# XJTU-Power-AI/charginghub-env

Hardware: AMD Instinct MI355X
Metric: env-steps/sec at 65 536 parallel envs (higher is better)
Workload: dtype f64; 1 GPU; 65536 envs x hub [20 fast, 25 slow] (BASELINE.json configs[3]), fcev_permeate 0.01, random policy resident in HBM, reset every 96 steps, Philox streams; envs_per_gpu=65536, obs_dim=13, act_dim=47, work_order=XCD-aware (tiles, tail and level workgroups in contiguous eighths per XCD), graph=on, collective=none

## Files before the change

### charginghub-env_amd/_lib.py

```python
import ctypes as C
import os

os.environ.setdefault("HIP_FORCE_DEV_KERNARG", "1")

_HERE = os.path.dirname(os.path.abspath(__file__))
DATA_DIR = os.path.join(_HERE, "data")

CHUB_FAST, CHUB_SLOW = 0, 1
RNG_COMPAT, RNG_PHILOX, RNG_PHILOX_CURVES = 0, 1, 2
RNG_MODES = {"compat": RNG_COMPAT, "philox": RNG_PHILOX, "philox_curves": RNG_PHILOX_CURVES}
T_COUNT = 38
TELEMETRY_NAMES = ["hy_act", "hy_flow_speed", "all_power_second", "Store_SOC", "capacity", "total_mass_need", "hy_use",
                   "not_meet", "fc_power", "hy_to_use", "re_used_renew", "re_ev_power_0", "re_ev_power_1",
                   "re_hydrogen_power", "income", "reward", "re_pv_power", "re_wd_power", "price_next",
                   "fcev_arrive_number", "fcev_line", "fcev_queue_len", "pv_day", "wd_day",
                   "ev_power_0_net", "ev_power_1_net", "ev_power_sum_net", "price_now",
                   "min_power_0", "charge_power_0", "max_power_0", "line_0", "flow_in_0",
                   "min_power_1", "charge_power_1", "max_power_1", "line_1", "flow_in_1"]
T = {name: i for i, name in enumerate(TELEMETRY_NAMES)}
EPISODE_NAMES = ["return", "income", "draw_ele", "length", "deviation", "test_penalty", "end_soc"]
EP_COUNT = len(EPISODE_NAMES)
EP = {name: i for i, name in enumerate(EPISODE_NAMES)}
PILE_NAMES = ("car", "charge", "emergency", "power", "soc", "init_soc", "target_soc", "stay_time", "already_stay_time")
PILE_COUNT = len(PILE_NAMES)
# ... 305 lines not shown
                ("price_fluctuate", C.c_double), ("hydro_loss", C.c_double)]


ENV_PARAM_FIELDS = ("hydro_prod_rate", "hydro_store_vlt", "init_soc", "fc_max_power", "fcev_permeate", "renew_fluctuate", "price_fluctuate",
                    "hydro_loss")


class ChubEnvParams(C.Structure):
    _fields_ = [(name, C.c_double) for name in ENV_PARAM_FIELDS]


def lib_path():
    return os.environ.get("CHUB_LIB") or os.path.join(_HERE, "libchub.so")


def source_hash():
    import hashlib

    h = hashlib.sha256()
    csrc = os.path.join(_HERE, "csrc")
    for name in ("chub_kernels.hip", "chub_policy.hip", "chub_critic.hip", "chub_runtime.cpp", "chub_comm.cpp", "chub_device.h", "chub_curves.h", "chub_plan.h",
                 "chub_policy.h", "chub_critic.h"):
        h.update(open(os.path.join(csrc, name), "rb").read())
    h.update(open(os.path.join(os.path.dirname(_HERE), "include", "chub.h"), "rb").read())
    return h.hexdigest()[:16]


_lib = None


def load_library():
    global _lib
    if _lib is not None:
        return _lib
    path = lib_path()
    if not os.path.exists(path):
        raise ChubError("libchub.so is not built (%s): run `python -c 'import __graft_entry__ as g; g.build()'` "
                        "or `make -C charginghub-env_amd/csrc`; there is no CPU fallback" % path)
    lib = C.CDLL(path)
    if not os.environ.get("CHUB_LIB"):
        lib.chub_build_id.restype = C.c_char_p
        have, want = lib.chub_build_id().decode(), source_hash()
        if have != want:
            raise ChubError("libchub.so (build id %s) is older than its sources (%s): rebuild with "
                            "`make -C charginghub-env_amd/csrc`" % (have, want))
    P, I, L = C.c_void_p, C.c_int, C.c_int64
    sig = {
        "chub_create": (I, [C.POINTER(ChubConfig), C.c_char_p, L, L, I, C.c_uint64, I, C.POINTER(P)]),
        "chub_create_ex": (I, [C.POINTER(ChubConfig), C.c_char_p, L, L, I, C.c_uint64, I, C.POINTER(ChubOptions), C.POINTER(P)]),
        "chub_destroy": (I, [P]),
        "chub_obs_dim": (I, [P]), "chub_act_dim": (I, [P]), "chub_num_envs": (L, [P]), "chub_clock": (I, [P]), "chub_uses_packed_kernel": (I, [P]), "chub_uses_fused_step": (I, [P]), "chub_uses_xcd_order": (I, [P]),
        "chub_launch_plan": (I, [C.POINTER(ChubConfig), L, I, C.POINTER(ChubOptions), P]),
        "chub_launch_plan_params": (I, [C.POINTER(ChubConfig), L, I, C.POINTER(ChubOptions), P]),
        "chub_create_params": (I, [C.POINTER(ChubConfig), C.c_char_p, L, L, I, C.c_uint64, I, C.POINTER(ChubOptions), P, C.POINTER(P)]),
        "chub_set_env_params": (I, [P, P, P]), "chub_get_env_params": (I, [P, P]), "chub_has_env_params": (I, [P]),
        "chub_reset": (I, [P, P, P, P]),
        "chub_step": (I, [P, P, P, P, P, P]), "chub_host_actions": (I, [P, C.POINTER(P)]),
        "chub_step_bits": (I, [P, P, P, P, P, P, P]), "chub_host_bits": (I, [P, C.POINTER(P), C.POINTER(P)]),
        "chub_step_bits_device": (I, [P, P, P, P, P, P, P, P]), "chub_step_bits_device_packed": (I, [P, P, P, P, P, P]),
        "chub_reset_device": (I, [P, P, P, P, P]),
        "chub_step_device": (I, [P, P, P, P, P, P, P]),
        "chub_step_device_packed": (I, [P, P, P, P, P]),
        "chub_reset_envs": (I, [P, P, P, P, P]), "chub_step_envs": (I, [P, P, P, P, P, P, P]), "chub_reset_envs_device": (I, [P, P, P, P, P, P]),
        "chub_step_envs_device": (I, [P, P, P, P, P, P, P, P]), "chub_env_clocks": (I, [P, P, P]), "chub_clock_groups": (I, [P]),
        "chub_dmask_reset_envs_device": (I, [P, P, P, P, P, P]), "chub_dmask_step_envs_device": (I, [P, P, P, P, P, P, P, P]),
        "chub_autoreset_step_device": (I, [P, P, P, P, P, P, P, P]),
        "chub_call_plan": (I, [C.POINTER(ChubConfig), L, I, C.POINTER(ChubOptions), I, C.c_uint32, P]),
        "chub_step_load": (I, [P, P, P, P, P, P]), "chub_step_load_device": (I, [P, P, P, P, P, P, P]),
        "chub_step_load_envs": (I, [P, P, P, P, P, P, P]), "chub_step_load_envs_device": (I, [P, P, P, P, P, P, P, P]),
        "chub_random_actions_device": (I, [P, C.c_uint64, C.c_uint32, P, P]),
        "chub_sync": (I, [P]),
        "chub_profile_begin": (I, [P, I, I]), "chub_profile_end": (I, [P, P, P, P]),
        "chub_get_slots": (I, [P, P]), "chub_get_station_scalars": (I, [P, P]), "chub_get_telemetry": (I, [P, P]),
        "chub_get_obs_f64": (I, [P, P]), "chub_get_reward_f64": (I, [P, P]), "chub_set_telemetry": (I, [P, I]), "chub_fcev_stuck_count": (I, [P, P]),
        "chub_telemetry_host": (I, [P, C.POINTER(P), C.POINTER(P), C.POINTER(P)]),
        "chub_set_episode_stats": (I, [P, I]), "chub_has_episode_stats": (I, [P]), "chub_get_episode_stats": (I, [P, I, P]),
        "chub_get_episode_counts": (I, [P, P]), "chub_episode_stats_device": (I, [P, I, P, P, P]),
        "chub_episode_summary_device": (I, [P, P, I, P]), "chub_episode_summary": (I, [P, P, I]),
        "chub_pile_obs_columns": (I, [C.c_uint32]), "chub_pile_obs_device": (I, [P, C.c_uint32, P, P, P]),
        "chub_station_profile_size": (I, [C.c_uint32, C.c_int32]), "chub_station_profile_device": (I, [P, C.c_uint32, C.c_int32, P, P, P]),
        "chub_load_dispatch_device": (I, [P, I, P, P, P, P, P, P]), "chub_load_dispatch": (I, [P, I, P, P, P, P]),
        "chub_forecast_size": (I, [C.c_uint32, C.c_int32]), "chub_forecast_device": (I, [P, C.c_uint32, C.c_int32, P, P, P]),
        "chub_forecast": (I, [P, C.c_uint32, C.c_int32, P]),
        "chub_get_step_terms_size": (I, [C.c_uint32]), "chub_get_step_terms_device": (I, [P, C.c_uint32, P, P, P]),
        "chub_get_step_terms": (I, [P, C.c_uint32, P]), "chub_set_step_terms": (I, [P, C.c_uint32, P]), "chub_get_step_terms_attached": (I, [P]),
        "chub_set_rng_compat_seeds": (I, [P, P]), "chub_set_rng_compat_state": (I, [P, P]),
        "chub_get_rng_compat_state": (I, [P, P]), "chub_compat_replay_constructor": (I, [P]), "chub_set_ou_state": (I, [P, P]),
        "chub_copy_envs": (I, [P, P, P, P, L]), "chub_copy_envs_device": (I, [P, P, P, P, L, P]),
        "chub_state_size": (L, [P]), "chub_get_state": (I, [P, P, L]), "chub_set_state": (I, [P, P, L]),
        "chub_get_hy_table": (I, [P, P]), "chub_get_hy_table_env": (I, [P, L, P]), "chub_set_hy_table": (I, [P, P]),
        "chub_last_error": (C.c_char_p, []), "chub_device_count": (I, []), "chub_build_id": (C.c_char_p, []),
        "chub_comm_unique_id": (I, [P]), "chub_comm_create": (I, [P, I, I, I, C.POINTER(P)]), "chub_comm_destroy": (I, [P]),
        "chub_comm_world": (I, [P]), "chub_comm_rank": (I, [P]), "chub_comm_gather": (I, [P, P, P, L, P]),
        "chub_comm_gather_timed": (I, [P, P, P, L, P, I, C.POINTER(C.c_double)]),
        "chub_comm_max_f64": (I, [P, C.POINTER(C.c_double), P]), "chub_comm_barrier": (I, [P, P]),
        "chub_comm_ranks_seen": (I, [P, C.POINTER(C.c_int), P]),
        "chub_comm_set_overlap": (I, [P, I]), "chub_comm_gather_begin": (I, [P, P, P]), "chub_comm_join": (I, [P, P]), "chub_device_info": (I, [I, P]),
        "chub_step_gather": (I, [P, P, P, P, P, P]), "chub_run_steps": (I, [P, P, P, I, P, P, P, L, L, P]),
        "chub_tape_register_soc": (I, [P, P, C.c_int32, P]), "chub_set_slots": (I, [P, P]), "chub_set_station_queue": (I, [P, P]),
        "chub_step_tape": (I, [P, P, P, P, P, P, P]), "chub_reset_tape": (I, [P, P, P, P]), "chub_tape_clear_soc": (I, [P]),
        "chub_step_tape_env": (I, [P, P, P, P, P, P, C.c_int32, P, P, P]), "chub_reset_tape_env": (I, [P, P, P, P, P, P]),
        "chub_graph_begin": (I, [P, P]), "chub_graph_end": (I, [P, P, C.POINTER(P)]), "chub_graph_launch": (I, [P, P]),
        "chub_graph_destroy": (I, [P]),
        "chub_malloc_device": (I, [I, L, C.POINTER(P)]), "chub_free_device": (I, [I, P]), "chub_copy_to_host": (I, [I, P, P, L, P]),
        "chub_copy_to_device": (I, [I, P, P, L, P]), "chub_alloc_host": (I, [I, L, C.POINTER(P)]), "chub_free_host": (I, [I, P]), "chub_stream_create": (I, [I, C.POINTER(P)]), "chub_stream_destroy": (I, [I, P]),
        "chub_stream_sync": (I, [I, P]),
# ... 2 lines not shown
        "chub_policy_set_weights": (I, [P, C.c_int32, P, P]), "chub_policy_set_weights_device": (I, [P, C.c_int32, P, P, P]),
        "chub_policy_act_device": (I, [P, P, P, L, P, P, P, P, P]), "chub_policy_act": (I, [P, P, P, P]),
        "chub_policy_run_steps": (I, [P, P, I, P, P, P, L, L, P]),
        "chub_next_tick": (I, [P, C.POINTER(C.c_uint32)]), "chub_policy_set_exploration": (I, [P, C.c_uint64, P]),
        "chub_policy_set_log_std_device": (I, [P, P, P]),
        "chub_policy_sample_device": (I, [P, P, P, L, P, C.POINTER(ChubPolicySampleOut), P]),
        "chub_policy_collect": (I, [P, P, I, C.POINTER(ChubRollout), P, L, P]),
        "chub_pile_set_device": (I, [P, I, P, P, P]),
        "chub_policy_sample_set_device": (I, [P, P, P, L, P, I, P, C.POINTER(ChubPolicySampleOut), P]),
        "chub_policy_collect_set": (I, [P, P, I, I, C.POINTER(ChubRollout), P, P, L, P]),
        "chub_rollout_gae_device": (I, [P, C.POINTER(ChubGae), P]),
        "chub_moments_create": (I, [P, C.c_int32, C.POINTER(P)]), "chub_moments_destroy": (I, [P]),
        "chub_moments_update_device": (I, [P, P, L, L, P, P]), "chub_moments_reset_device": (I, [P, P]),
        "chub_moments_get": (I, [P, C.POINTER(C.c_double), P, P]), "chub_moments_set": (I, [P, C.c_double, P, P]),
        "chub_moments_state_device": (I, [P, C.POINTER(P)]),
        "chub_policy_set_normalizer": (I, [P, P, P]), "chub_policy_set_normalizer_device": (I, [P, P, P, P]),
        "chub_policy_get_normalizer_device": (I, [P, P, P, P]), "chub_policy_normalizer_from_moments_device": (I, [P, P, C.c_double, P]),
        "chub_population_param_count": (I, [C.POINTER(ChubConfig), C.POINTER(ChubPolicySpec), C.POINTER(L)]),
        "chub_population_create": (I, [P, C.c_int32, C.c_uint64, C.POINTER(P)]), "chub_population_destroy": (I, [P]),
        "chub_population_perturb_device": (I, [P, P, P, C.c_float, C.c_uint32, P]),
        "chub_population_set_member_device": (I, [P, C.c_int32, C.c_int32, P, P, P]),
        "chub_population_get_member_device": (I, [P, C.c_int32, C.c_int32, P, P, P]),
        "chub_population_set_member": (I, [P, C.c_int32, C.c_int32, P, P]), "chub_population_get_member": (I, [P, C.c_int32, C.c_int32, P, P]),
        "chub_population_copy_members_device": (I, [P, P, P, C.c_int32, P]),
        "chub_population_act_device": (I, [P, P, P, L, P, P, P, P, P]), "chub_population_run_steps": (I, [P, P, I, P, P, P, L, L, P]),
        "chub_population_es_gradient_device": (I, [P, P, C.c_uint32, P, P, P]),
        "chub_policy_grad_plan": (I, [C.POINTER(ChubConfig), C.POINTER(ChubPolicySpec), L, C.POINTER(ChubPolicyGradPlanOut)]),
        "chub_policy_grad_create": (I, [P, L, C.POINTER(P)]), "chub_policy_grad_destroy": (I, [P]),
        "chub_policy_grad_device": (I, [P, C.POINTER(ChubPolicyGradIn), C.POINTER(ChubPolicyGradOut), P]),
        "chub_critic_plan": (I, [C.POINTER(ChubCriticSpec), L, C.POINTER(ChubCriticPlanOut)]),
        "chub_critic_create": (I, [P, C.POINTER(ChubCriticSpec), P, P, P, P, L, C.POINTER(P)]), "chub_critic_destroy": (I, [P]),
        "chub_critic_set_weights": (I, [P, C.c_int32, P, P]), "chub_critic_set_weights_device": (I, [P, C.c_int32, P, P, P]),
        "chub_critic_set_normalizer": (I, [P, P, P]), "chub_critic_set_normalizer_device": (I, [P, P, P, P]),
        "chub_critic_normalizer_from_moments_device": (I, [P, P, C.c_double, P]),
        "chub_critic_values_device": (I, [P, P, L, L, P, L, P, P]),
        "chub_critic_grad_device": (I, [P, C.POINTER(ChubCriticGradIn), C.POINTER(ChubCriticGradOut), P]),
    }
    for name, (res, args) in sig.items():
        try:
            fn = getattr(lib, name)
        except AttributeError:
            if os.environ.get("CHUB_LIB"):
                def missing(*_a, _name=name, _path=path):
                    raise ChubError("%s is not exported by the library CHUB_LIB names (%s): an older build" % (_name, _path))
                setattr(lib, name, missing)
                continue
            raise
        fn.restype = res
        fn.argtypes = args
    _lib = lib
    return lib


EXPORTED = ["chub_create", "chub_create_ex", "chub_destroy", "chub_obs_dim", "chub_act_dim", "chub_num_envs", "chub_clock", "chub_uses_packed_kernel", "chub_uses_fused_step", "chub_uses_xcd_order", "chub_launch_plan", "chub_launch_plan_params",
            "chub_create_params", "chub_set_env_params", "chub_get_env_params", "chub_has_env_params", "chub_reset",
            "chub_step", "chub_host_actions", "chub_step_bits", "chub_host_bits", "chub_step_bits_device", "chub_step_bits_device_packed", "chub_reset_device", "chub_step_device", "chub_step_device_packed", "chub_step_load", "chub_step_load_device", "chub_step_load_envs", "chub_step_load_envs_device", "chub_reset_envs", "chub_step_envs", "chub_reset_envs_device", "chub_step_envs_device",
            "chub_env_clocks", "chub_clock_groups", "chub_dmask_reset_envs_device", "chub_dmask_step_envs_device", "chub_autoreset_step_device", "chub_call_plan", "chub_random_actions_device", "chub_sync", "chub_profile_begin", "chub_profile_end",
            "chub_get_slots", "chub_get_station_scalars", "chub_get_telemetry", "chub_get_obs_f64",
            "chub_get_reward_f64", "chub_set_telemetry", "chub_fcev_stuck_count", "chub_set_rng_compat_seeds", "chub_set_rng_compat_state", "chub_get_rng_compat_state", "chub_compat_replay_constructor", "chub_set_ou_state",
            "chub_copy_envs", "chub_copy_envs_device", "chub_state_size", "chub_get_state", "chub_set_state", "chub_get_hy_table", "chub_get_hy_table_env", "chub_set_hy_table", "chub_last_error", "chub_device_count", "chub_build_id",
            "chub_comm_unique_id", "chub_comm_create", "chub_comm_destroy", "chub_comm_world", "chub_comm_rank", "chub_comm_gather", "chub_comm_gather_timed",
            "chub_comm_max_f64", "chub_comm_barrier", "chub_comm_ranks_seen", "chub_comm_set_overlap", "chub_comm_gather_begin", "chub_comm_join", "chub_device_info", "chub_step_gather", "chub_run_steps", "chub_tape_register_soc", "chub_set_slots",
            "chub_set_station_queue", "chub_step_tape", "chub_reset_tape", "chub_tape_clear_soc", "chub_step_tape_env", "chub_reset_tape_env", "chub_telemetry_host", "chub_graph_begin", "chub_graph_end", "chub_graph_launch", "chub_graph_destroy",
            "chub_malloc_device", "chub_free_device", "chub_copy_to_host", "chub_copy_to_device", "chub_alloc_host", "chub_free_host", "chub_stream_create",
            "chub_stream_destroy", "chub_stream_sync",
            "chub_set_episode_stats", "chub_has_episode_stats", "chub_get_episode_stats", "chub_get_episode_counts", "chub_episode_stats_device",
            "chub_episode_summary_device", "chub_episode_summary", "chub_pile_obs_columns", "chub_pile_obs_device",
            "chub_station_profile_size", "chub_station_profile_device", "chub_load_dispatch_device", "chub_load_dispatch",
            "chub_forecast_size", "chub_forecast_device", "chub_forecast",
            "chub_get_step_terms_size", "chub_get_step_terms_device", "chub_get_step_terms", "chub_set_step_terms", "chub_get_step_terms_attached",
            "chub_policy_input_width", "chub_policy_create", "chub_policy_destroy", "chub_policy_set_weights", "chub_policy_set_weights_device",
            "chub_policy_act_device", "chub_policy_act", "chub_policy_run_steps",
            "chub_next_tick", "chub_policy_set_exploration", "chub_policy_set_log_std_device", "chub_policy_sample_device", "chub_policy_collect",
            "chub_pile_set_device", "chub_policy_sample_set_device", "chub_policy_collect_set", "chub_rollout_gae_device",
            "chub_moments_create", "chub_moments_destroy", "chub_moments_update_device", "chub_moments_reset_device", "chub_moments_get", "chub_moments_set",
            "chub_moments_state_device", "chub_policy_set_normalizer", "chub_policy_set_normalizer_device", "chub_policy_get_normalizer_device",
            "chub_policy_normalizer_from_moments_device",
            "chub_population_param_count", "chub_population_create", "chub_population_destroy", "chub_population_perturb_device",
            "chub_population_set_member_device", "chub_population_get_member_device", "chub_population_set_member", "chub_population_get_member",
            "chub_population_copy_members_device", "chub_population_act_device", "chub_population_run_steps", "chub_population_es_gradient_device",
            "chub_policy_grad_plan", "chub_policy_grad_create", "chub_policy_grad_destroy", "chub_policy_grad_device",
            "chub_critic_plan", "chub_critic_create", "chub_critic_destroy", "chub_critic_set_weights", "chub_critic_set_weights_device",
            "chub_critic_set_normalizer", "chub_critic_set_normalizer_device", "chub_critic_normalizer_from_moments_device",
            "chub_critic_values_device", "chub_critic_grad_device"]


def check(rc):
    if rc != 0:
        msg = load_library().chub_last_error()
        raise ChubError("libchub error %d: %s" % (rc, msg.decode() if msg else "?"))
```

### charginghub-env_amd/csrc/chub_device.h

```cpp
#pragma once

#include <stdint.h>

#include "chub_curves.h"

#if defined(__HIP_DEVICE_COMPILE__)
#define CHUB_G(T) T __attribute__((address_space(1))) *
#else
#define CHUB_G(T) T *
#endif

namespace chub {

constexpr int kMaxLine = 10;
constexpr int kLevels = 1000;
constexpr int kBalkTab = 1024;
constexpr int kMaxPiles = 4096;
constexpr int kSocLevels = 2048;
constexpr int kSocLevelShift = 21;
constexpr int kPolarMaxTrials = 32;
#ifndef CHUB_TRACE
#define CHUB_TRACE 0
#endif
#ifndef CHUB_SLOTS_PER_LANE
// ... 175 lines not shown
struct EpisodeArrays {
    int32_t on;
    int32_t pad_;
    CHUB_G(double) live;
    CHUB_G(double) fin;
    CHUB_G(uint32_t) episodes;
    CHUB_G(uint8_t) pending;
};

enum FcField : uint32_t { FC_SLOT = 0, FC_VALID, FC_SIN, FC_COS, FC_PRICE, FC_PV, FC_WIND, FC_ARRIVALS0, FC_ARRIVALS1, FC_FCEV };
constexpr int kFcCount = 10;
constexpr int kFcHist = 301;
struct ForecastTabs {
    const float *mean;
    const uint32_t *hist;
    const uint16_t *hist_len;
};

struct DevCtx {
    HubParams hp;
    SlotArrays sl;
    StationArrays st;
    EnvArrays ev;
    CompatRng cr;
    Tables tb;
    EnvParamArrays ep;
    EpisodeArrays es;
};

struct CopyArgs {
    const DevCtx *src;
    const DevCtx *dst;
    CHUB_G(const int64_t) src_idx;
    CHUB_G(const int64_t) dst_idx;
    int64_t count;
    CHUB_G(const uint16_t) src_clk;
    CHUB_G(uint16_t) dst_clk;
    uint32_t src_clk_value;
    int32_t src_rng, dst_rng;
    CHUB_G(const double) src_rows;
    CHUB_G(double) dst_rows;
};

struct PackedPtrs {
    const EnvArrays *ev;
    const StationArrays *st;
    uint32_t *hot, *rec;
    uint8_t *stay8;
    uint32_t *pk[2];
    const float *cls[2], *ttab[2], *ttab2;
    uint32_t late8[8];
    const Tables *tb;
    const double *sin96;
};

struct StepArgs {
    int32_t t;
    uint32_t tick;
    int32_t draw_price;
    int32_t station_filter;
    double price_last;
    double price_prev;
    const float *actions;
    const uint64_t *act_bits;
    const float *act_tail;
    const double *exo_z;
    const int32_t *exo_days;
    float *obs;
    float *reward;
    uint8_t *done;
    float *done_f32;
    int32_t obs_stride, reward_stride;
    int32_t load_mode;
    const uint64_t *pk_tape;
    const uint32_t *car_tape;
    const uint32_t *hv_tape;
    int32_t hv_w;
    int32_t tail_tape;
    uint16_t *env_clk;
    const uint8_t *env_mask;
    int32_t env_lo, env_hi;
    int32_t fresh;
    int32_t empt_fresh;
    int32_t commit_rng;
    int32_t rng_cur;
    int32_t walked;
    int32_t walk_far, walk_short;
    uint32_t *tick_note;
    uint8_t *done_mask;
    uint32_t *done_count;
    const uint32_t *skip_count;
    float *final_obs;
#if CHUB_TRACE
    unsigned long long *stamps_slot, *stamps_env;
#endif
};

}
```

### charginghub-env_amd/csrc/chub_kernels.hip

```cpp
#include <hip/hip_runtime.h>
#include <hip/hip_ext.h>
#include <stdint.h>

#include "chub_device.h"
#include "chub_plan.h"

namespace chub {

typedef uint32_t u32x4 __attribute__((ext_vector_type(4)));
typedef uint32_t u32x2 __attribute__((ext_vector_type(2)));

__device__ __forceinline__ bool in_group(const StepArgs &sa, int64_t env) { return !sa.env_mask || sa.env_mask[env] != 0; }
__device__ __forceinline__ uint32_t env_clk(const StepArgs &sa, int64_t n_envs, int64_t env) {
    return sa.env_clk[(int64_t) (sa.tick & 1u) * n_envs + env];
}
__device__ __forceinline__ int64_t range_len(const StepArgs &sa) { return (int64_t) sa.env_hi - sa.env_lo + 1; }
__device__ __forceinline__ bool range_unit(const StepArgs &sa, int64_t i, int segments, int &seg, int64_t &env) {
    const int64_t R = range_len(sa);
    if (i >= (int64_t) segments * R) return false;
    seg = (i >= R ? 1 : 0) + (i >= 2 * R ? 1 : 0);
    env = sa.env_lo + (i - (int64_t) seg * R);
    return true;
}

// ... 218 lines not shown
}

__device__ __forceinline__ float normal_from_word(const float *tz, const float *tl, uint32_t w) {
    const uint32_t cell = w >> 20;
    const bool hi = cell >= 4096u - 16u, lo = cell < 16u;
    const uint32_t m = hi ? ~w : w;
    const bool tail = hi || lo;
    const float *tab = tail ? tl : tz;
    const uint32_t idx = tail ? (m >> 12) : cell;
    const float frac = tail ? (float) (m & 0xFFFu) * (1.0f / 4096.0f) : (float) (w & 0xFFFFFu) * (1.0f / 1048576.0f);
    const float a = tab[idx], b = tab[idx + 1];
    const float z = __fadd_rn(a, __fmul_rn(__fsub_rn(b, a), frac));
    return hi ? -z : z;
}

__device__ __forceinline__ uint32_t dk_make(uint64_t pk, int line, bool fast) {
    line = __popc((uint32_t) pk & ((1u << line) - 1u));
    const int n_in = (int) (pk >> 10) & 15;
    const int flow = fast ? n_in : (int) ((pk >> (14 + 4 * line)) & 15);
    return (uint32_t) (line + flow) | ((uint32_t) flow << 8);
}
__device__ __forceinline__ uint32_t draw_decoded_levels(const HubParams &hp, const Tables &tb, uint32_t tick, int t, int k, int64_t env,
                                                        int line, bool fast) {
    PhiloxCtx px{hp.key[0], hp.key[1], tick, (uint32_t) (hp.env_id0 + env)};
    const U4 a0 = px.block(SITE_ARRIVE, (uint32_t) k, 0);
    const U4 r0 = px.block(SITE_RENEGE, (uint32_t) k, 0);
    int n_in = (int) tb.cnt[k][t * kLevels + (int) (a0.v[0] % 1000u)];
    n_in = n_in > 9 ? 9 : n_in;
    uint32_t rw[10] = {r0.v[0], r0.v[1], r0.v[2], r0.v[3], 0u, 0u, 0u, 0u, 0u, 0u};
    if (__any(line > 4)) {
        const U4 r1 = px.block(SITE_RENEGE, (uint32_t) k, 1), r2 = px.block(SITE_RENEGE, (uint32_t) k, 2);
        rw[4] = r1.v[0]; rw[5] = r1.v[1]; rw[6] = r1.v[2]; rw[7] = r1.v[3]; rw[8] = r2.v[0]; rw[9] = r2.v[1];
    }
    int stay_q = 0;
#pragma unroll
    for (int w = 0; w < kMaxLine; w++) stay_q += (w < line && (int) (rw[w] % 1000u) >= (int) tb.thr_renege[w]) ? 1 : 0;
    int flow = n_in;
    if (!fast && __any(n_in > 0)) {
        uint32_t bw[9] = {a0.v[1], a0.v[2], a0.v[3], 0u, 0u, 0u, 0u, 0u, 0u};
        if (__any(n_in > 3)) {
            const U4 a1 = px.block(SITE_ARRIVE, (uint32_t) k, 1), a2 = px.block(SITE_ARRIVE, (uint32_t) k, 2);
            bw[3] = a1.v[0]; bw[4] = a1.v[1]; bw[5] = a1.v[2]; bw[6] = a1.v[3]; bw[7] = a2.v[0]; bw[8] = a2.v[1];
        }
        const int S = hp.S[k];
        flow = 0;
#pragma unroll
        for (int j = 0; j < 9; j++) {
            if (j >= 3 && !__any(n_in > j)) break;
            const int top = (int) tb.inv_balk[bw[j] % 1000u] - j;
            flow += (j < n_in && j <= S && stay_q <= top) ? 1 : 0;
        }
    }
    return (uint32_t) (stay_q + flow) | ((uint32_t) flow << 8);
}
__device__ __forceinline__ int dk_want(uint32_t dk) { return (int) (dk & 255u); }
__device__ __forceinline__ int dk_flow(uint32_t dk) { return (int) ((dk >> 8) & 255u); }


template <int TYPE>
__device__ __forceinline__ void car_step_curves(float tt, bool cp, const CurveConsts &cc, float &soc, float &power) {
    if (cp) {
        soc = time_to_soc<TYPE>(tt, cp, cc);
        power = time_to_power<TYPE>(tt, cp);
        return;
    }
    if (TYPE == 0) {
        const float xf = tt * 15.0f;
        const double x = xf, t = tt;
        const bool p1 = tt >= 0 && t < (28.7 / 15), p2 = tt >= 0 && t < (51.2 / 15);
        const bool s0 = tt <= 0, s1 = t <= 28.7 / 15, s2 = t <= 51.2 / 15;
        float pw = 0.0f, sc = 100.0f;
        if (__any(p1 || (!s0 && s1))) {
            const double e = exp(0.053 * x);
            if (p1) pw = (float) (0.7194 * e + 47.78);
            if (!s0 && s1) sc = (float) ((0.7194 / 0.053) * e + 50.15 * x - (double) cc.fast_aa1_c) * cc.fast_soc_scale;
        }
        if (__any((!p1 && p2) || (!s0 && !s1 && s2))) {
            const double x2 = x * x, x3 = x2 * x, x4 = x2 * x2, x5 = x4 * x;
            if (!p1 && p2) pw = (float) (0.0002253 * x4 - 0.03572 * x3 + 2.016 * x2 - 48.76 * x + 457.7);
            if (!s0 && !s1 && s2)
                sc = (float) ((0.0002253 / 5) * x5 - (0.03572 / 4) * x4 + (2.016 / 3) * x3 - (48.76 / 2) * x2 + 457.7 * x +
                              (double) cc.fast_aa2_c) * cc.fast_soc_scale;
        }
        if (s0) sc = 0.0f;
        soc = sc;
        power = pw;
    } else {
        const float xf = tt / 4.0f;
        const double x = xf, t = tt;
        const bool p1 = t < 2.33 * 4, p2 = t < 3.67 * 4;
        const bool c0 = tt <= 0, c1 = t <= 2.33 * 4, c2 = t <= 3.67 * 4;
        float pw = 0.0f, ch = cc.slow_c2_end;
        if (__any(p1 || (!c0 && c1))) {
            const double x2 = x * x, x3 = x2 * x, x4 = x2 * x2, x5 = x4 * x;
            if (p1) pw = (float) (-0.002056 * x4 + 0.00921 * x3 + 0.03562 * x2 + 0.02379 * x + 6.007);
            if (!c0 && c1)
                ch = (float) (-0.0004112 * x5 + 0.0023025 * x4 + (0.03562 / 3) * x3 + 0.011895 * x2 + 6.007 * x);
        }
        if (__any((!p1 && p2) || (!c0 && !c1 && c2))) {
            if (!p1 && p2) pw = (float) ((-4.041 * x + 21.1) / (x - 0.485));
            if (!c0 && !c1 && c2) ch = (float) (-4.041 * x + 19.140115 * log(fabs(x - 0.485)) + 11.943306312699628);
        }
        if (c0) ch = 0.0f;
        soc = (float) CHUB_DIV_K64((double) (100.0f * ch), 19.285746346634653);
        power = pw;
    }
// ... 1100 lines not shown
            car = tl > 0;
        }
        const bool urgent = car && must_charge(t_target, t_soc, tl);
        const uint64_t bc = __ballot(car);
        if (lane == 0) s_ball[4 + wave] = bc;
        if (MODE == MODE_COMPAT) {
            s_a[tid] = urgent ? power : 0.0f;
            s_b[tid] = charge ? power : 0.0f;
            s_c[tid] = car ? power : 0.0f;
        } else {
            const int q = kw_to_fixed(power);
            s_u[tid] = (uint32_t) (urgent ? q : 0);
            s_v[tid] = (uint32_t) (charge ? q : 0);
            s_w[tid] = (uint32_t) (car ? q : 0);
        }
        __syncthreads();
        cars += __popcll(s_ball[4]) + __popcll(s_ball[5]) + __popcll(s_ball[6]) + __popcll(s_ball[7]);
        if (tid == 0) {
            const int n = S - (c << 8) < 256 ? S - (c << 8) : 256;
            if (MODE == MODE_COMPAT) rf.add(s_a, s_b, s_c, n);
            else ri.add(s_u, s_v, s_w, n);
        }
        base += chunk_empties;
        __syncthreads();
    }
    if (tid == 0) {
        if (MODE == MODE_COMPAT) {
            rs.store(ctx->cr, sa.rng_cur, env);
            rec_store(st.rec, sidx, rf.mn, rf.chg, rf.mx, pkd_make(s_hdr[2], s_hdr[1], cars));
        } else {
            rec_store(st.rec, sidx, fixed64_to_kw(ri.mn), fixed64_to_kw(ri.chg), fixed64_to_kw(ri.mx), pkd_make(s_hdr[2], s_hdr[1], cars));
        }
    }
}

struct PackedArgs {
    uint32_t S[2], type[2];
    uint32_t n_envs, epb, magic, cls_delta;
    CHUB_G(uint32_t) state;
    CHUB_G(uint32_t) rec;
    CHUB_G(const uint32_t) pk;
    CHUB_G(const float) actions;
    CHUB_G(const float) cls0;
    CHUB_G(const float) ttab2;
    CHUB_G(const uint32_t) car_tape;
    uint32_t key[2], gid0, tick;
    const uint32_t *tick_base;
    uint32_t late[8];
    CHUB_G(const uint8_t) env_mask;
    uint32_t blk0;
    uint32_t xcd;
    CHUB_G(float) tail_act;
    CHUB_G(uint8_t) stay8;
};

typedef const uint32_t __attribute__((address_space(4))) *chub_sptr;
__device__ __forceinline__ uint32_t sload_u32(const void *p, int i) { return ((chub_sptr) (uintptr_t) p)[i]; }
__device__ __forceinline__ bool mask_is_empty(const StepArgs &sa) { return sa.skip_count != nullptr && sload_u32(sa.skip_count, 0) == 0u; }

#ifndef CHUB_ACT_NT
#define CHUB_ACT_NT 0
#endif
#if CHUB_ACT_NT
#define CHUB_ACT_LOAD(p) __builtin_nontemporal_load(p)
#else
#define CHUB_ACT_LOAD(p) (*(p))
#endif
#ifndef CHUB_ACC_COPIES
#define CHUB_ACC_COPIES 2
#endif
constexpr int kAccCopies = CHUB_ACC_COPIES;
#ifndef CHUB_TAIL_PRE
#define CHUB_TAIL_PRE 1
#endif
#ifndef CHUB_UNIT_DRAWS
#define CHUB_UNIT_DRAWS 1
#endif
#ifndef CHUB_EPI_ALL
#define CHUB_EPI_ALL 1
#endif
#define CHUB_AT(T_, base, byte_off) (*(CHUB_G(T_)) ((CHUB_G(char)) (base) + (uint32_t) (byte_off)))
template <int BLOCK, int T, bool RESET, bool BIG, bool MASKED, bool FUSED, bool BITS>
__device__ __forceinline__ void packed_records(const PackedArgs &pa, const uint32_t block_local, int *s_acc, const uint32_t *s_unit, u32x4 *s_rec,
                                               const float *tail_pre = nullptr) {
    const int lane = threadIdx.x & 63;
    const int S0 = (int) pa.S[0], S1 = (int) pa.S[1], St = S0 + S1;
    const int epb = (int) pa.epb, N = (int) pa.n_envs;
    const int env_first = (int) block_local * epb;
    const long long *s_acc64 = (const long long *) s_acc;
    __builtin_amdgcn_fence(__ATOMIC_RELEASE, "wavefront");
    __builtin_amdgcn_wave_barrier();
    __builtin_amdgcn_fence(__ATOMIC_ACQUIRE, "wavefront");
    for (int i = lane; i < 2 * epb; i += 64) {
        const int e = i >> 1, k = i & 1;
        const int env = env_first + e;
        if (env >= N) continue;
        if (MASKED && pa.env_mask[env] == 0) continue;
        const uint32_t su = (uint32_t) (k ? N : 0) + (uint32_t) env;
        if (!RESET && !FUSED && !BITS && k == 0) {
            typedef float f32x2_ __attribute__((ext_vector_type(2)));
            const uint32_t ai = ((uint32_t) env * (uint32_t) (St + 2) + (uint32_t) St) << 2;
            f32x2_ tv;
            if (CHUB_TAIL_PRE && i < 64) tv = f32x2_{tail_pre[0], tail_pre[1]};
            else tv = f32x2_{CHUB_AT(const float, pa.actions, ai), CHUB_AT(const float, pa.actions, ai + 4u)};
            CHUB_AT(f32x2_, pa.tail_act, (uint32_t) env << 3) = tv;
        }
        uint32_t lf = s_unit[i];
        if ((k ? S1 : S0) == 0) {
            const uint32_t pk = CHUB_AT(const uint32_t, pa.pk, su << 2);
            const bool fast = (k ? pa.type[1] : pa.type[0]) == 0;
            int want, fl;
            if (RESET) {
                fl = fast ? (int) (int16_t) (pk & 0xFFFFu) : (int) ((pk >> 16) & 0xFFFFu);
                want = fl;
            } else {
                want = dk_want(pk);
                fl = dk_flow(pk);
            }
            const int as = want < 0 ? want : 0;
            int ln = want - as;
            ln = ln < kMaxLine ? ln : kMaxLine;
            lf = pkd_make(ln, fl, 0);
        }
        u32x4 rv;
        if (!BIG) {
            int a0 = 0, a1 = 0, a2 = 0, a3 = 0;
#pragma unroll
            for (int c = 0; c < kAccCopies; c++) {
                const int *acc = s_acc + 4 * i + c * 8 * epb;
                a0 += acc[0]; a1 += acc[1]; a2 += acc[2]; a3 += acc[3];
            }
            rv = u32x4{__float_as_uint(fixed_to_kw(a0)), __float_as_uint(fixed_to_kw(a1)), __float_as_uint(fixed_to_kw(a2)),
                       lf | ((uint32_t) a3 << 16)};
        } else {
            const long long *a64 = s_acc64 + 4 * i;
            rv = u32x4{__float_as_uint((float) a64[0] * (1.0f / 524288.0f)), __float_as_uint((float) a64[1] * (1.0f / 524288.0f)),
                       __float_as_uint((float) a64[2] * (1.0f / 524288.0f)), lf | ((uint32_t) a64[3] << 16)};
        }
        CHUB_AT(u32x4, pa.rec, su << 4) = rv;
        if (FUSED) s_rec[i] = rv;
    }
}
#undef CHUB_AT

struct NoHook {
    __device__ __forceinline__ void prefetch() {}
    __device__ __forceinline__ void park() {}
};
template <int BLOCK, int T, bool TAPE, bool RESET, bool BIG, bool MASKED, bool FUSED, typename Hook, bool BITS = false, bool PIPED = false>
__device__ __forceinline__ int slot_body_packed(const HubParams &hp, const StepArgs &sa, PackedArgs &pa, const Tables &tb,
                                                const uint32_t block_local, uint32_t *q_cnt, uint32_t *q_new,
                                                uint64_t *s_ball, int *s_acc, uint32_t *s_unit, Hook &hook, u32x4 *s_rec, uint32_t *s_uinfo) {
    typedef float f32x4 __attribute__((ext_vector_type(4)));
    typedef float f32x2 __attribute__((ext_vector_type(2)));
    constexpr int WAVES = BLOCK / 64;
    const int tid = threadIdx.x;
    const int lane = tid & 63, wave = tid >> 6;
    const int S0 = (int) pa.S[0], S1 = (int) pa.S[1], St = S0 + S1;
    const int epb = (int) pa.epb, N = (int) pa.n_envs;
    const int env_first = (int) block_local * epb;
    const uint32_t idx0 = (uint32_t) env_first * (uint32_t) St;
    CHUB_STAMP_DECL(16);
    CHUB_STAMP_REAL(12);
    CHUB_STAMP(0);
#define CHUB_AT(T_, base, byte_off) (*(CHUB_G(T_)) ((CHUB_G(char)) (base) + (uint32_t) (byte_off)))

    constexpr bool STATE_FIRST = !RESET && !FUSED && BLOCK <= 256;
    constexpr bool UNIT_DRAWS = CHUB_UNIT_DRAWS && STATE_FIRST && !BIG && T <= 2;
    int e_[T], k_[T], slot[T];
    bool valid[T];
    uint32_t sidx[T];
    uint32_t s2[T];
    float act[T];
    u32x2 actw[T];
    int hs_[T];
    uint32_t pk_in[T];
    uint32_t served[T];
    constexpr bool HOIST_TAIL = CHUB_TAIL_PRE && !RESET && !FUSED && !BITS;
    float tail_pre[2];
#pragma unroll
    for (int j = 0; j < T; j++) {
        const int v = tid + j * BLOCK;
        e_[j] = (int) (__umul24((uint32_t) v, pa.magic) >> 20);
        const int hs = v - (int) __umul24((uint32_t) e_[j], (uint32_t) St);
        k_[j] = hs >= S0 ? 1 : 0;
        hs_[j] = hs;
        slot[j] = hs - (k_[j] ? S0 : 0);
        const int env = env_first + e_[j];
        valid[j] = e_[j] < epb && env < N;
        served[j] = 1u;
        sidx[j] = (uint32_t) (k_[j] ? N : 0) + (uint32_t) env;
        asm volatile("" : "=v"(s2[j]), "=v"(act[j]), "=v"(pk_in[j]), "=v"(actw[j]));
        if (!STATE_FIRST) {
            if (RESET) {
                s2[j] = 0u;
                act[j] = 0.0f;
            }
            if (MASKED && valid[j]) served[j] = pa.env_mask[env];
            if (valid[j]) {
                if (!RESET) {
                    s2[j] = CHUB_AT(uint32_t, pa.state, (idx0 + (uint32_t) v) << 2);
                    if (BITS) actw[j] = CHUB_AT(const u32x2, pa.actions, ((uint32_t) env * (((uint32_t) St + 63u) >> 6) + ((uint32_t) hs >> 6)) << 3);
                    else act[j] = CHUB_ACT_LOAD((CHUB_G(const float)) ((CHUB_G(const char)) pa.actions + (uint32_t) ((idx0 + (uint32_t) v + 2u * (uint32_t) env) << 2)));
                }
                pk_in[j] = CHUB_AT(const uint32_t, pa.pk, sidx[j] << 2);
            }
        }
    }
    if (STATE_FIRST) {
        uint32_t vc[T], envc[T];
#pragma unroll
        for (int j = 0; j < T; j++) {
            vc[j] = valid[j] ? (uint32_t) (tid + j * BLOCK) : 0u;
            envc[j] = valid[j] ? (uint32_t) (env_first + e_[j]) : (uint32_t) env_first;
        }
#pragma unroll
        for (int j = 0; j < T; j++) s2[j] = CHUB_AT(uint32_t, pa.state, (idx0 + vc[j]) << 2);
        asm volatile("" ::: "memory");
        if (MASKED) {
#pragma unroll
            for (int j = 0; j < T; j++) served[j] = CHUB_AT(const uint8_t, pa.env_mask, envc[j]);
            asm volatile("" ::: "memory");
        }
        if (!UNIT_DRAWS) {
#pragma unroll
            for (int j = 0; j < T; j++) pk_in[j] = CHUB_AT(const uint32_t, pa.pk, (valid[j] ? sidx[j] : (uint32_t) env_first) << 2);
            asm volatile("" ::: "memory");
        }
#pragma unroll
        for (int j = 0; j < T; j++) {
            if (BITS) actw[j] = CHUB_AT(const u32x2, pa.actions, (envc[j] * (((uint32_t) St + 63u) >> 6) + (valid[j] ? (uint32_t) hs_[j] >> 6 : 0u)) << 3);
            else act[j] = CHUB_ACT_LOAD((CHUB_G(const float)) ((CHUB_G(const char)) pa.actions + (uint32_t) ((idx0 + vc[j] + 2u * envc[j]) << 2)));
        }
    }
    uint32_t upk = 0u;
    if (UNIT_DRAWS) asm volatile("" : "=v"(upk));
    if (UNIT_DRAWS && (tid & ~63) < 2 * epb) {
        asm volatile("" ::: "memory");
        const int ue = tid >> 1, uenv = env_first + ue;
        upk = CHUB_AT(const uint32_t, pa.pk, (ue < epb && uenv < N ? (uint32_t) ((tid & 1) ? N : 0) + (uint32_t) uenv : (uint32_t) env_first) << 2);
    }
    if (HOIST_TAIL) asm volatile("" : "=v"(tail_pre[0]), "=v"(tail_pre[1]));
    if (HOIST_TAIL && wave == WAVES - 1) {
        asm volatile("" ::: "memory");
        const int te = env_first + (lane >> 1);
        const uint32_t tenv = (uint32_t) ((lane >> 1) < epb && te < N ? te : env_first);
        const uint32_t ai = (tenv * (uint32_t) (St + 2) + (uint32_t) St) << 2;
        tail_pre[0] = CHUB_AT(const float, pa.actions, ai);
        tail_pre[1] = CHUB_AT(const float, pa.actions, ai + 4u);
    }
    if (!TAPE) {
        pa.tick += sload_u32(pa.tick_base, 0);
        asm volatile("" : "+s"(pa.key[0]), "+s"(pa.key[1]), "+s"(pa.gid0), "+s"(pa.tick), "+s"(pa.late[0]), "+s"(pa.late[1]), "+s"(pa.late[2]),
                          "+s"(pa.late[3]), "+s"(pa.late[4]), "+s"(pa.late[5]), "+s"(pa.late[6]), "+s"(pa.late[7]));
    }
    CHUB_STAMP(1);
    if (FUSED) hook.prefetch();
    if (tid == 0) q_cnt[0] = 0;
    for (int i = tid; i < (BIG ? 16 : 8 * kAccCopies) * epb; i += BLOCK) s_acc[i] = 0;
    long long *s_acc64 = (long long *) s_acc;

    uint32_t w0[T];
    int tl[T];
    bool stays[T];
    f32x4 row[T];
    float ttg[T];
    if (!FUSED) {
#pragma unroll
        for (int j = 0; j < T; j++) asm volatile("" : "+v"(s2[j]));
    }
    if (MASKED) {
#pragma unroll
        for (int j = 0; j < T; j++) {
            asm volatile("" : "+v"(served[j]));
            valid[j] = valid[j] && served[j] != 0u;
        }
    }
#pragma unroll
    for (int j = 0; j < T; j++) {
        if (FUSED) asm volatile("" : "+v"(s2[j]));
        w0[j] = valid[j] ? s2[j] : 0u;
        tl[j] = ps_tl(w0[j]);
        stays[j] = tl[j] > 1;
        asm volatile("" : "=v"(row[j]), "=v"(ttg[j]));
        if (stays[j]) {
            row[j] = CHUB_AT(const f32x4, pa.cls0, (k_[j] ? pa.cls_delta : 0u) + (ps_cls(w0[j]) << 8) + (ps_n(w0[j]) << 3));
            ttg[j] = CHUB_AT(const float, pa.ttab2, (k_[j] ? 4096u : 0u) + (ps_lev(w0[j]) << 2));
        }
    }

    CHUB_STAMP(2);
    bool empty[T];
    uint64_t be[T];
#pragma unroll
    for (int j = 0; j < T; j++) {
        empty[j] = valid[j] && !stays[j];
        be[j] = __ballot(empty[j]);
        if (lane == 0) s_ball[wave + j * WAVES] = be[j];
    }
    if (FUSED) hook.park();
    CHUB_STAMP(3);
    __syncthreads();
    CHUB_STAMP(4);
    if (!BIG) {
        for (int u = tid; u < 2 * epb; u += BLOCK) {
            const int e = u >> 1, k = u & 1;
            const int Sk = k ? S1 : S0;
            const int U0 = e * St + (k ? S0 : 0), U1 = U0 + Sk;
            const int wv = U0 >> 6, lo = U0 & 63;
            const int hi0 = (U1 - (wv << 6)) < 64 ? (U1 - (wv << 6)) : 64;
            uint32_t info = (uint32_t) wv << 24;
            int all = 0;
            if (Sk > 0) {
                const uint64_t b0 = s_ball[wv];
                const uint64_t below_lo = lo ? (~0ull >> (64 - lo)) : 0ull, below_hi = ~0ull >> (64 - hi0);
                const int start_e = __popcll(b0 & below_lo), cnt0 = __popcll(b0 & below_hi & ~below_lo);
                const int over = U1 - ((wv + 1) << 6);
                const int cnt1 = over > 0 ? __popcll(s_ball[wv + 1] & (~0ull >> (64 - over))) : 0;
                all = cnt0 + cnt1;
                info |= (uint32_t) start_e | ((uint32_t) cnt0 << 8) | (UNIT_DRAWS ? 0u : (uint32_t) (cnt0 + cnt1) << 16);
            }
            if (UNIT_DRAWS) {
                asm volatile("" : "+v"(upk));
                const int want = dk_want(upk);
                const int assign = want < all ? want : all;
                const int ln = want - assign;
                s_unit[u] = pkd_make(ln < kMaxLine ? ln : kMaxLine, dk_flow(upk), 0);
                info |= (uint32_t) assign << 16;
            }
            s_uinfo[u] = info;
        }
    }

    uint32_t w0n[T];
#pragma unroll
    for (int j = 0; j < T; j++) {
        if (BITS) asm volatile("" : "+v"(row[j]), "+v"(ttg[j]), "+v"(actw[j]));
        else asm volatile("" : "+v"(row[j]), "+v"(ttg[j]), "+v"(act[j]));
        const int u = 2 * e_[j] + k_[j];
        int *acc = s_acc + 4 * u + (BIG ? 0 : (lane & (kAccCopies - 1)) * 8 * epb);
        w0n[j] = 0u;
        if (stays[j]) {
            const float t_target = ttg[j];
            const bool bit_on = BITS && ((((hs_[j] & 32) ? actw[j].y : actw[j].x) >> (hs_[j] & 31)) & 1u) != 0u;
            const bool on = (BITS ? bit_on : act[j] >= kActOnThreshold) || must_charge(t_target, row[j].y, tl[j]);
            const float power = on ? row[j].z : row[j].x, t_soc = on ? row[j].w : row[j].y;
            const int q = kw_to_fixed(power);
            const bool urgent = must_charge(t_target, t_soc, tl[j] - 1);
            w0n[j] = (w0[j] & ~kPsChg) - 1u + (on ? (kPsStep | kPsChg) : 0u);
            if (!BIG) {
                atomicAdd((unsigned long long *) (acc + 2), (unsigned long long) (uint32_t) q | (1ull << 32));
                if (on || urgent)
                    atomicAdd((unsigned long long *) acc,
                              (unsigned long long) (urgent ? (uint32_t) q : 0u) | ((unsigned long long) (on ? (uint32_t) q : 0u) << 32));
            } else {
                unsigned long long *a64 = (unsigned long long *) (s_acc64 + 4 * u);
                atomicAdd(a64 + 2, (unsigned long long) q);
                atomicAdd(a64 + 3, 1ull);
                if (urgent) atomicAdd(a64 + 0, (unsigned long long) q);
                if (on) atomicAdd(a64 + 1, (unsigned long long) q);
            }
        }
    }
    CHUB_STAMP(5);
    if (!BIG) __syncthreads();
    CHUB_STAMP(6);

    int line[T], flow[T];
    bool adm[T];
    uint64_t ba[T];
    uint32_t n_push = 0;
#pragma unroll
    for (int j = 0; j < T; j++) {
        const int vw = wave + j * WAVES;
        int empties, rank;
        if (!BIG) {
// ... 77 lines not shown
            const u32x2 tp = CHUB_AT(const u32x2, pa.car_tape, (idx0 + (uint32_t) src) << 3);
            c = tp.x;
            lev = tp.y & 0xFFFFu;
            late = (int) (tp.y >> 16);
        } else {
            PhiloxCtx p2{pa.key[0], pa.key[1], pa.tick, pa.gid0 + (uint32_t) (env_first + s_e)};
            const U4 o = p2.block(SITE_SOC, (uint32_t) s_hs, 0);
            c = o.v[0] >> kSocLevelShift;
            lev = o.v[1] % 1000u;
            late = 0;
#pragma unroll
            for (int j = 0; j < 8; j++) late += (o.v[2] >= pa.late[j]) ? 1 : 0;
            if (__any(o.v[2] >= pa.late[7])) {
#pragma unroll
                for (int j = 8; j < 16; j++) late += (o.v[2] >= tb.late_thr[j]) ? 1 : 0;
            }
        }
        f32x2 e0 = CHUB_AT(const f32x2, pa.cls0, (s_k ? pa.cls_delta : 0u) + (c << 8));
        float tt_ = CHUB_AT(const float, pa.ttab2, (s_k ? 4096u : 0u) + (lev << 2));
        asm volatile("" : "+v"(e0), "+v"(tt_));
        int st_ = (int) ceilf(__fsub_rn(tt_, e0.y)) + late;
        st_ = st_ > kMaxStay ? kMaxStay : st_;
        CHUB_AT(uint32_t, pa.state, (idx0 + (uint32_t) src) << 2) = st_ > 0 ? ps_make(st_, c, lev) : 0u;
        CHUB_AT(uint8_t, pa.stay8, idx0 + (uint32_t) src) = (uint8_t) st_;
        if (st_ > 0) {
            const int q = kw_to_fixed(e0.x);
            if (!BIG) {
                int *ac = s_acc + 4 * (2 * s_e + s_k) + (lane & (kAccCopies - 1)) * 8 * epb;
                atomicAdd((unsigned long long *) (ac + 2), (unsigned long long) (uint32_t) q | (1ull << 32));
                if (must_charge(tt_, e0.y, st_)) atomicAdd(ac, q);
            } else {
                unsigned long long *a64 = (unsigned long long *) (s_acc64 + 4 * (2 * s_e + s_k));
                atomicAdd(a64 + 2, (unsigned long long) q);
                atomicAdd(a64 + 3, 1ull);
                if (must_charge(tt_, e0.y, st_)) atomicAdd(a64 + 0, (unsigned long long) q);
            }
        }
    }
    CHUB_STAMP(9);
    if (FUSED) return wave == WAVES - 1 ? WAVES : wave + 1;
    if (ALL) {
        __syncthreads();
        CHUB_STAMP(10);
        CHUB_STAMP_REAL(13);
#if CHUB_TRACE
        if (sa.stamps_slot && tid == 0) {
            for (int i = 0; i <= 10; i++) sa.stamps_slot[(size_t) block_local * 16 + i] = stamp_[i];
            sa.stamps_slot[(size_t) block_local * 16 + 12] = stamp_[12];
            sa.stamps_slot[(size_t) block_local * 16 + 13] = stamp_[13];
        }
#endif
        if (wave != WAVES - 1) return 0;
    }
    packed_records<BLOCK, T, RESET, BIG, MASKED, false, BITS>(pa, block_local, s_acc, s_unit, nullptr, tail_pre);
#if CHUB_TRACE
    asm volatile("s_waitcnt vmcnt(0)" ::: "memory");
    CHUB_STAMP(11);
    if (sa.stamps_slot && lane == 0) sa.stamps_slot[(size_t) block_local * 16 + 11] = stamp_[11];
#endif
    return 0;
#undef CHUB_AT
}

template <int BLOCK, int T, bool TAPE, bool RESET, bool BIG, bool MASKED, bool BITS = false>
__global__ __launch_bounds__(BLOCK, (BLOCK <= 256 ? 8 : 2048 / BLOCK)) void k_slot_packed(const DevCtx *__restrict__ ctx, StepArgs sa, PackedArgs pa_in) {
    __shared__ uint32_t q_new[BLOCK * T];
    __shared__ uint32_t q_cnt[2];
    __shared__ uint64_t s_ball[BLOCK * T / 64 + 2];
    __shared__ __attribute__((aligned(16))) int s_acc[2 * BLOCK * T * kAccCopies];
    __shared__ uint32_t s_unit[BLOCK * T / 2];
    __shared__ uint32_t s_uinfo[BLOCK * T / 2];
    if (RESET && MASKED && mask_is_empty(sa)) return;
    PackedArgs pa = pa_in;
    asm volatile("" : "+s"(pa.S[0]), "+s"(pa.S[1]), "+s"(pa.type[0]), "+s"(pa.type[1]), "+s"(pa.n_envs), "+s"(pa.epb), "+s"(pa.magic),
                      "+s"(pa.cls_delta), "+s"(pa.state), "+s"(pa.rec), "+s"(pa.pk), "+s"(pa.actions), "+s"(pa.cls0), "+s"(pa.ttab2));
    NoHook hook;
    (void) slot_body_packed<BLOCK, T, TAPE, RESET, BIG, MASKED, false, NoHook, BITS>(ctx->hp, sa, pa, ctx->tb, xcd_order(blockIdx.x, pa.xcd, MASKED ? 0u : pa.xcd) + (MASKED ? pa.blk0 : 0u), q_cnt, q_new,
                                                                                     s_ball + 1, s_acc, s_unit, hook, nullptr, s_uinfo);
}

struct TailArgs {
    CHUB_G(const double) ou;
    CHUB_G(const double) price_noise;
    CHUB_G(const double) cap;
    CHUB_G(const int16_t) pv_day;
    CHUB_G(const int16_t) wd_day;
    CHUB_G(const uint8_t) q_len;
    CHUB_G(const uint8_t) hv_line;
    CHUB_G(const uint32_t) drw;
    CHUB_G(const uint8_t) drw_cnt;
    CHUB_G(uint32_t) rec;
    CHUB_G(const float) actions;
    uint32_t n_envs, act_dim, s_tot, xcd;
    CHUB_G(const float) tail_act;
    CHUB_G(const double) pv_row;
    CHUB_G(const double) wd_row;
    CHUB_G(const double) pv_row_now;
    CHUB_G(const double) wd_row_now;
    CHUB_G(const double) hy_table;
    const uint32_t *tick_base;
    double sin_t;
    uint32_t key[2], gid0, pad2;
};
inline TailArgs make_tail_args(const EnvArrays &ev, const StationArrays &st, const HubParams &hp, const StepArgs &sa, const PackedPtrs &pp,
                               bool reset) {
    TailArgs ta;
    const int t_next = reset ? 0 : (sa.t + 1) % 96;
    ta.tail_act = (hp.rng_mode == MODE_PHILOX && hp.packed && !sa.load_mode && !reset) ? (CHUB_G(const float)) st.tail_act : nullptr;
    if (sa.act_bits && !reset) ta.tail_act = (CHUB_G(const float)) sa.act_tail;
    ta.pv_row = (CHUB_G(const double)) (pp.tb->pvT + t_next * 100);
    ta.wd_row = (CHUB_G(const double)) (pp.tb->wdT + t_next * 150);
    ta.pv_row_now = (CHUB_G(const double)) (pp.tb->pvT + (reset ? 0 : sa.t) * 100);
    ta.wd_row_now = (CHUB_G(const double)) (pp.tb->wdT + (reset ? 0 : sa.t) * 150);
    ta.hy_table = (CHUB_G(const double)) pp.tb->hy_table;
    ta.tick_base = hp.tick_base;
    ta.sin_t = pp.sin96[t_next];
    ta.key[0] = hp.key[0];
    ta.key[1] = hp.key[1];
    ta.gid0 = (uint32_t) hp.env_id0;
    ta.pad2 = 0;
    ta.ou = (CHUB_G(const double)) ev.ou;
    ta.price_noise = (CHUB_G(const double)) ev.price_noise;
    ta.cap = (CHUB_G(const double)) ev.cap;
    ta.pv_day = (CHUB_G(const int16_t)) ev.pv_day;
    ta.wd_day = (CHUB_G(const int16_t)) ev.wd_day;
    ta.q_len = (CHUB_G(const uint8_t)) ev.q_len;
    ta.hv_line = (CHUB_G(const uint8_t)) ev.hv_line;
    ta.drw = (CHUB_G(const uint32_t)) ev.drw[sa.tick & 1u];
    ta.drw_cnt = (CHUB_G(const uint8_t)) ev.drw_cnt[sa.tick & 1u];
    ta.rec = (CHUB_G(uint32_t)) st.rec;
// ... 491 lines not shown
    double soc = (double) socf;
    if (soc < 0.5) soc = 0.5;
    const double p0 = (soc * 0.01) * 70;
    j2601_time_mass(p0, tn, mn);
}

__device__ __forceinline__ double ou_sample(double &state, double theta, double sigma, double z) {
    const double dx = theta * (0.0 - state) + sigma * z;
    state += dx;
    return state;
}

#define CHUB_TEL(i, v)                                        \
    do {                                                      \
        if (tel_on) ev.telem[(size_t) (i) * (size_t) N + (size_t) env] = (v); \
    } while (0)

constexpr int kEnvBlock = 256;

struct TailIn {
    double ou_pv, ou_wd, ou_price, price_noise, cap;
    float a_el, a_fc;
    int pv_day, wd_day, q_len, hv_line;
    u32x4 drw;
    uint32_t drw_n;
};
__device__ __forceinline__ void tail_prefetch(TailIn &in, const TailArgs &ta, const uint32_t e32, const bool predrawn) {
    const uint32_t n32 = ta.n_envs;
    in.ou_pv = ta.ou[e32];
    in.ou_wd = ta.ou[n32 + e32];
    in.ou_price = ta.ou[2u * n32 + e32];
    in.price_noise = ta.price_noise[e32];
    if (ta.tail_act) {
        typedef float f32x2_ __attribute__((ext_vector_type(2)));
        const f32x2_ tv = ((CHUB_G(const f32x2_)) ta.tail_act)[e32];
        in.a_el = tv.x;
        in.a_fc = tv.y;
    } else {
        const uint32_t ai = e32 * ta.act_dim + ta.s_tot;
        in.a_el = ta.actions[ai];
        in.a_fc = ta.actions[ai + 1u];
    }
    in.cap = ta.cap[e32];
    in.pv_day = ta.pv_day[e32];
    in.wd_day = ta.wd_day[e32];
    in.q_len = ta.q_len[e32];
    in.hv_line = ta.hv_line[e32];
    if (predrawn) {
        in.drw = ((CHUB_G(const u32x4)) ta.drw)[e32];
        in.drw_n = ta.drw_cnt[e32];
    }
}

struct NoMid {
    __device__ __forceinline__ void operator()() {}
    __device__ __forceinline__ void at1() {}
    __device__ __forceinline__ void at2() {}
    __device__ __forceinline__ void at3() {}
};
__device__ __forceinline__ uint32_t hv_count_rate(float rate, uint32_t n) {
    const int c = (int) roundf(rate * (float) n);
    return (uint32_t) (c < 0 ? 0 : (c > 255 ? 255 : c));
}
__device__ __forceinline__ uint32_t hv_count_env(const EnvParamArrays &ep, uint32_t e, int t, uint32_t lev) {
    return hv_count_rate(ep.hv_rate[e], (uint32_t) ep.hv_idx[(uint32_t) t * (uint32_t) kLevels + lev]);
}

template <bool RESET, int MODE, bool MULTI, bool FUSED = false, typename Mid = NoMid, int EB = kEnvBlock, bool TAPE = false, bool EP = false>
__device__ __forceinline__ void env_tail(const DevCtx *__restrict__ ctx, const StepArgs &sa, const int env, const bool live,
                                         const double *s_pv, const double *s_wd, const double *s_pv_now, const double *s_wd_now,
                                         const double *s_hy, const uint8_t *s_hv, float *s_out, const int env_block, const TailArgs &ta,
                                         const u32x4 *s_rec, const int local_env, const int env0_fused, const int rows_fused,
                                         const TailIn &pre, const bool use_pre, Mid &mid) {
    const HubParams &hp = ctx->hp;
    const EnvArrays &ev = ctx->ev;
    const CompatRng &cr = ctx->cr;
    const Tables &tb = ctx->tb;
    const int64_t N = hp.n_envs;
    constexpr bool multi = MULTI;
    const uint32_t my_clk = (multi && env < (int) N) ? env_clk(sa, N, env) : 0u;
    if (multi && env < (int) N)
        sa.env_clk[(int64_t) ((sa.tick + 1u) & 1u) * N + env] = (uint16_t) (!live ? my_clk : (RESET ? 0u : clk_next(my_clk)));
    const int t_now = multi ? clk_t(my_clk) : sa.t;
    const int t_next = RESET ? 0 : (t_now + 1) % 96;
    const bool draw_price = multi ? ((my_clk >> 8) & 3u) == 0u : sa.draw_price != 0;
    const double price_last = multi ? tb.price[RESET ? 95 : t_now] : sa.price_last;
    const double price_prev = multi ? tb.price[(t_now + 95) % 96] : sa.price_prev;
#define TAB_PV(d) (multi ? tb.pvT[t_next * 100 + (d)] : s_pv[d])
#define TAB_WD(d) (multi ? tb.wdT[t_next * 150 + (d)] : s_wd[d])
#define TAB_PV_NOW(d) (multi ? tb.pvT[t_now * 100 + (d)] : s_pv_now[d])
#define TAB_WD_NOW(d) (multi ? tb.wdT[t_now * 150 + (d)] : s_wd_now[d])
#define TAB_HY(i) ((MODE == MODE_COMPAT || EP) ? hy_env[i] : s_hy[i])
#define HP_E(field, own) (EP ? (own) : hp.field)
#define TAB_HV(l) (EP ? hv_count_env(ctx->ep, e32, t_now, (uint32_t) (l)) : multi ? tb.cnt_hv[(uint32_t) t_now * (uint32_t) kLevels + (uint32_t) (l)] : s_hv[l])
    const uint32_t e32 = (uint32_t) env, n32 = ta.n_envs;
    CHUB_STAMP_DECL(16);
    CHUB_STAMP_REAL(8);
    CHUB_STAMP(0);
#if CHUB_TRACE
    {
        uint32_t n_ = n32;
        asm volatile("" : "+s"(n_));
        CHUB_STAMP(1);
    }
#endif
    double st_pv = 0.0, st_wd = 0.0, st_hy = 0.0, st_pv_now = 0.0, st_wd_now = 0.0;
    uint32_t st_hv = 0;
    const double sin_t = multi ? tb.sin96[t_next] : ta.sin_t;
    const int32_t tel_word = hp.telemetry;
    const bool tel_on = (tel_word & 1) != 0;
    const bool ep_on = (tel_word & 2) != 0;
    if (!FUSED) {
        const int i = threadIdx.x;
        if (!multi) {
            if (i < 100) st_pv = ta.pv_row[i];
            if (i < 150) st_wd = ta.wd_row[i];
            if (!RESET) {
                if (i < 100) st_pv_now = ta.pv_row_now[i];
                if (i < 150) st_wd_now = ta.wd_row_now[i];
            }
        }
        if (!RESET) {
            if (!EP && i < 102) st_hy = ta.hy_table[i];
            if (MODE == MODE_COMPAT && !EP && !multi && !sa.hv_tape && i < kLevels / 4) st_hv = ((CHUB_G(const uint32_t)) tb.cnt_hv)[sa.t * (kLevels / 4) + i];
        }
    }
    constexpr bool tick_late = MODE == MODE_PHILOX && !RESET && !TAPE;
    const bool tick_now = MODE == MODE_PHILOX && (!tick_late || sa.fresh != 0);
    PhiloxCtx px{ta.key[0], ta.key[1], tick_now ? sa.tick + sload_u32(ta.tick_base, 0) : sa.tick, ta.gid0 + (uint32_t) env};
    double cap = 0.0, in_price_noise = 0.0;
    double ou_pv = 0.0, ou_wd = 0.0, ou_price = 0.0, z_pv = 0.0, z_wd = 0.0, z_pr = 0.0;
    float a_el_f = 0.0f, a_fc_f = 0.0f, P0f = 0.0f, P1f = 0.0f, mn0 = 0.0f, mx0 = 0.0f, mn1 = 0.0f, mx1 = 0.0f;
    int pv_day = 0, wd_day = 0, q_len = 0, hv_line = 0, F0i = 0, F1i = 0, ln0 = 0, ln1 = 0, hv_lev = 0, hv_arrive = 0;
    u32x4 drw_raw = {0u, 0u, 0u, 0u};
    uint32_t drw_n = 0u, hvw0 = 0u, hvw1 = 0u;
    const bool have_pre = FUSED && use_pre;
    double p_v_h_max = 0.0, p_cells = 0.0, p_rc_cells = 0.0, p_cap_mass = 0.0, p_rc_cap_mass = 0.0, p_init_soc = 0.0, p_hydro_loss = 0.0;
    double p_fc_max_power = 0.0, p_renew_fluct1 = 0.0, p_price_fluct1 = 0.0;
    if (live) {
        if (EP) {
            CHUB_G(const double) pr = ctx->ep.prm;
            p_cap_mass = pr[PRM_CAP_MASS * n32 + e32];
            p_renew_fluct1 = pr[PRM_RENEW_FLUCT1 * n32 + e32];
            p_price_fluct1 = pr[PRM_PRICE_FLUCT1 * n32 + e32];
            if (RESET) {
                p_init_soc = pr[PRM_INIT_SOC * n32 + e32];
            } else {
                p_v_h_max = pr[PRM_V_H_MAX * n32 + e32];
                p_cells = pr[PRM_CELLS * n32 + e32];
                p_rc_cells = pr[PRM_RC_CELLS * n32 + e32];
                p_rc_cap_mass = pr[PRM_RC_CAP_MASS * n32 + e32];
                p_hydro_loss = pr[PRM_HYDRO_LOSS * n32 + e32];
                p_fc_max_power = pr[PRM_FC_MAX_POWER * n32 + e32];
            }
        }
        if (have_pre) {
            ou_pv = pre.ou_pv; ou_wd = pre.ou_wd; ou_price = pre.ou_price; in_price_noise = pre.price_noise;
        } else {
            ou_pv = ta.ou[e32];
            ou_wd = ta.ou[n32 + e32];
            ou_price = ta.ou[2u * n32 + e32];
            in_price_noise = ta.price_noise[e32];
        }
        if (!FUSED) {
            const StationRec r0 = rec_load(ta.rec, e32), r1 = rec_load(ta.rec, n32 + e32);
            mn0 = r0.mn; P0f = r0.chg; mx0 = r0.mx; ln0 = pkd_line(r0.pkd); F0i = pkd_flow(r0.pkd);
            mn1 = r1.mn; P1f = r1.chg; mx1 = r1.mx; ln1 = pkd_line(r1.pkd); F1i = pkd_flow(r1.pkd);
        }
        if (!RESET && have_pre) {
            a_el_f = pre.a_el; a_fc_f = pre.a_fc; cap = pre.cap;
            pv_day = pre.pv_day; wd_day = pre.wd_day; q_len = pre.q_len; hv_line = pre.hv_line;
        } else if (!RESET) {
            if (ta.tail_act) {
                typedef float f32x2_ __attribute__((ext_vector_type(2)));
                const f32x2_ tv = ((CHUB_G(const f32x2_)) ta.tail_act)[e32];
                a_el_f = tv.x;
                a_fc_f = tv.y;
            } else {
                const uint32_t ai = e32 * ta.act_dim + ta.s_tot;
                a_el_f = ta.actions[ai];
                a_fc_f = ta.actions[ai + 1u];
            }
            cap = ta.cap[e32];
            pv_day = ta.pv_day[e32];
            wd_day = ta.wd_day[e32];
            q_len = ta.q_len[e32];
            hv_line = ta.hv_line[e32];
        }
        if (MODE == MODE_COMPAT && !RESET && sa.hv_tape) {
            hvw0 = sa.hv_tape[e32 * (uint32_t) sa.hv_w];
            if (sa.hv_w > 1) hvw1 = sa.hv_tape[e32 * (uint32_t) sa.hv_w + 1u];
        }
        if (TAPE) {
            z_pv = sa.exo_z[e32 * 3u + 0u];
            z_wd = sa.exo_z[e32 * 3u + 1u];
            z_pr = sa.exo_z[e32 * 3u + 2u];
            if (!RESET) hv_arrive = (int) sa.hv_tape[e32 * (uint32_t) sa.hv_w];
        } else if (MODE == MODE_PHILOX && !RESET && !sa.fresh) {
            if (have_pre) {
                drw_raw = pre.drw;
                drw_n = pre.drw_n;
            } else {
                drw_raw = ((CHUB_G(const u32x4)) ta.drw)[e32];
                drw_n = ta.drw_cnt[e32];
            }
        } else if (MODE == MODE_PHILOX) {
            const U4 ow = px.block(SITE_OU, 0, 0);
            z_pv = (double) normal_from_word(tb.normal_icdf, tb.normal_tail, ow.v[0]);
            z_wd = (double) normal_from_word(tb.normal_icdf, tb.normal_tail, ow.v[1]);
            z_pr = (double) normal_from_word(tb.normal_icdf, tb.normal_tail, ow.v[2]);
            if (!RESET) {
                hv_lev = (int) (px.block(SITE_HV, 0, 0).v[0] % 1000u);
                hv_arrive = EP ? (int) hv_count_env(ctx->ep, e32, t_now, (uint32_t) hv_lev)
                               : (int) tb.cnt_hv[(uint32_t) t_now * (uint32_t) kLevels + (uint32_t) hv_lev];
            }
        } else {
            z_pv = sa.exo_z[e32 * 3u + 0u];
            z_wd = sa.exo_z[e32 * 3u + 1u];
            z_pr = sa.exo_z[e32 * 3u + 2u];
        }
    }


    if (tick_late && !tick_now) {
        const uint32_t *tbp = ta.tick_base;
        asm volatile("" : "+s"(tbp) : : "memory");
        px.tick += sload_u32(tbp, 0);
    }
    if (!FUSED) {
        static_assert(EB >= 150, "one table element per lane");
        CHUB_STAMP(2);
        const int i = threadIdx.x;
        if (i < 100) ((double *) s_pv)[i] = st_pv;
        if (i < 150) ((double *) s_wd)[i] = st_wd;
        if (!RESET) {
            if (i < 100) ((double *) s_pv_now)[i] = st_pv_now;
            if (i < 150) ((double *) s_wd_now)[i] = st_wd_now;
            if (!EP && i < 102) ((double *) s_hy)[i] = st_hy;
            if (MODE == MODE_COMPAT && !EP && i < kLevels / 4) ((uint32_t *) s_hv)[i] = st_hv;
        }
        __syncthreads();
    }
    CHUB_STAMP(3);
    if (!TAPE && MODE == MODE_PHILOX && !RESET && !sa.fresh) {
        z_pv = (double) __uint_as_float(drw_raw.x);
        z_wd = (double) __uint_as_float(drw_raw.y);
        z_pr = (double) __uint_as_float(drw_raw.z);
        hv_arrive = (int) drw_n;
    }
    const int row_w = sa.obs_stride;
    auto flush_rows = [&]() {
        if (FUSED) {
            __builtin_amdgcn_fence(__ATOMIC_RELEASE, "wavefront");
            __builtin_amdgcn_wave_barrier();
            __builtin_amdgcn_fence(__ATOMIC_ACQUIRE, "wavefront");
            float *dst = sa.obs + (size_t) env0_fused * (size_t) row_w;
            const int total = rows_fused * row_w;
            if ((((uintptr_t) dst) & 15u) == 0) {
                typedef float f32x4 __attribute__((ext_vector_type(4)));
                const int quads = total >> 2;
                for (int i = (int) (threadIdx.x & 63u); i < quads; i += 64) ((f32x4 *) dst)[i] = ((const f32x4 *) s_out)[i];
                for (int i = (quads << 2) + (int) (threadIdx.x & 63u); i < total; i += 64) dst[i] = s_out[i];
            } else {
                for (int i = (int) (threadIdx.x & 63u); i < total; i += 64) dst[i] = s_out[i];
            }
            __builtin_amdgcn_fence(__ATOMIC_RELEASE, "wavefront");
            __builtin_amdgcn_wave_barrier();
            return;
        }
        __syncthreads();
        const int env0 = env_block * EB;
        const int rows = (int) N - env0 < EB ? (int) N - env0 : EB;
        float *dst = sa.obs + (size_t) env0 * (size_t) row_w;
        const int total = rows * row_w;
        if (MULTI && sa.env_mask && !__syncthreads_and((live || env >= (int) N) ? 1 : 0)) {
            for (int i = threadIdx.x; i < total; i += EB)
                if (in_group(sa, env0 + i / row_w)) dst[i] = s_out[i];
        } else if ((((uintptr_t) dst) & 15u) == 0) {
            typedef float f32x4 __attribute__((ext_vector_type(4)));
            const int quads = total >> 2;
            for (int i = threadIdx.x; i < quads; i += EB) ((f32x4 *) dst)[i] = ((const f32x4 *) s_out)[i];
            for (int i = (quads << 2) + threadIdx.x; i < total; i += EB) dst[i] = s_out[i];
        } else {
            for (int i = threadIdx.x; i < total; i += EB) dst[i] = s_out[i];
        }
    };
    const double *hy_env = (MODE == MODE_COMPAT || EP) ? (const double *) ev.hy_env + (size_t) e32 * 102u : nullptr;
    (void) hy_env;
// ... 88 lines not shown
                }
                if (stuck) {
                    fold_n++;
                } else if (q_len < qcap) {
                    qt[q_len] = tn;
                    qm[q_len] = mn;
                    q_len++;
                }
                total_time += tn;
                total_mass += mn;
            }
            int hv_num = 0;
            if (total_time > 15.0) {
                bool found = false;
                if (!stuck) {
                    for (int i = 1; i <= arrive - 1; i++) {
                        int keep = q_len - i;
                        keep = keep < 0 ? 0 : keep;
                        double part = 0.0;
                        for (int j = 0; j < keep; j++) part += qt[j];
                        if (part <= 15.0) {
                            hv_line = i;
                            hv_num = keep;
                            found = true;
                            break;
                        }
                    }
                }
                if (found) {
                    for (int j = hv_num; j < q_len; j++) {
                        qt[j - hv_num] = qt[j];
                        qm[j - hv_num] = qm[j];
                    }
                    q_len -= hv_num;
                } else {
                    fold_n += (uint32_t) q_len;
                    q_len = 0;
                    stuck = true;
                    ev.q_fold[2u * e32] = total_time;
                    ev.q_fold[2u * e32 + 1u] = total_mass;
                    ev.q_fold_cnt[e32] = fold_n;
                }
            } else {
                hv_line = 0;
                q_len = 0;
            }
            ev.q_len[e32] = (uint8_t) q_len;
            ev.hv_line[e32] = (uint8_t) (hv_line | (stuck ? 128 : 0));
        } else if (hv_line != 0) {
            ev.hv_line[e32] = 0;
            hv_line = 0;
        }
        total_mass_need = total_mass;
    }
    mid.at1();

    {
        double temp = TAB_PV(pv_day);
        if (temp > 0 && (pv_day % 2) == 0) {
            temp += ou_sample(ou_pv, .01, 1., z_pv) * HP_E(renew_fluct1, p_renew_fluct1);
            ev.ou[e32] = ou_pv;
        }
        re_pv = (temp > 0 ? temp : 0.0) * 5;
        temp = TAB_WD(wd_day);
        temp += ou_sample(ou_wd, .01, 1.5, z_wd) * HP_E(renew_fluct1, p_renew_fluct1);
        ev.ou[n32 + e32] = ou_wd;
        re_wd = (temp > 0 ? temp : 0.0) * 1;
        if (draw_price) {
            price_next = ou_sample(ou_price, .1, 0.005, z_pr) * HP_E(price_fluct1, p_price_fluct1);
            ev.ou[2u * n32 + e32] = ou_price;
            ev.price_noise[e32] = price_next;
            price_next += price_last;
        } else {
            price_next = price_last + in_price_noise;
        }
    }
    if (MODE == MODE_COMPAT && !RESET && !hv_walked) rs.store(cr, sa.rng_cur, env);
    } while (0);

    CHUB_STAMP(4);
    mid();
    if (FUSED && live) {
        const u32x4 v0 = s_rec[2 * local_env], v1 = s_rec[2 * local_env + 1];
        mn0 = __uint_as_float(v0.x); P0f = __uint_as_float(v0.y); mx0 = __uint_as_float(v0.z); ln0 = pkd_line(v0.w); F0i = pkd_flow(v0.w);
        mn1 = __uint_as_float(v1.x); P1f = __uint_as_float(v1.y); mx1 = __uint_as_float(v1.z); ln1 = pkd_line(v1.w); F1i = pkd_flow(v1.w);
    }

    do {
    if (!live) break;
    if (!RESET) {
        const double a_el = ((double) a_el_f + 1) / 2;
        const double a_fc = ((double) a_fc_f + 1) / 2;
        const double P0 = (double) P0f, P1 = (double) P1f;
        const double F0 = (double) F0i, F1 = (double) F1i;
        double re_new_power = in_re_wd + in_re_pv;
        const double charging_power = 0.0 + P0 + P1;
        double hy_power_limit = 2000 + re_new_power - charging_power;
        hy_power_limit = hy_power_limit > 0 ? hy_power_limit : 0.0;
        double act_el = a_el;
        int req = (int) ceil(a_el * 100);
        req = req < 0 ? 0 : (req > 101 ? 101 : req);
        if (((MODE == MODE_COMPAT || EP) ? hy_req_pre : TAB_HY(req)) > hy_power_limit) {
            int ind = 0;
            while (ind < 102 && !(TAB_HY(ind) >= hy_power_limit)) ind++;
            act_el = (ind >= 102 || ind == 0) ? 0.01 * 100 : 0.01 * (ind - 1);
        }
        {
        double must_chg = cap_mass * 0.1 - cap;
        must_chg = must_chg > 0 ? must_chg : 0.0;
        double upper_charge = cap_mass - cap;
        upper_charge = upper_charge > 0 ? upper_charge : 0.0;
        const double v_h_max = HP_E(v_h_max, p_v_h_max), cells = HP_E(cells, p_cells);
        double charge_temp = act_el * v_h_max * (15 * 60);
        charge_temp = charge_temp < upper_charge ? charge_temp : upper_charge;
        charge_temp = charge_temp > must_chg ? charge_temp : must_chg;
        double flow = DIV_K(charge_temp, 15 * 60);
        flow = flow < v_h_max ? flow : v_h_max;
        double ele_power = 0.0;
        if (cells != 0.0) {
            const double v_H_mass = div_c(flow, cells, HP_E(rc_cells, p_rc_cells));
            const double v_H_mol = DIV_K(v_H_mass, 2.02);
            const double v_H_L = v_H_mol * hp.v_M;
            const double v_H = v_H_L * 1000 * 60;
            const double temp = div_c(v_H * 2 * 96487, hp.v_M * 1000 * 60, hp.rc_vm60k);
            double power = temp * temp * 0.326 + temp * 1.476;
            ele_power = DIV_K(cells * power, 1000);
        }
// ... 46 lines not shown
        {
            const double sl_ = 0.0 + e0 + e1;
            if (sl_ > 0) {
                const double rate_ = ev_power_sum / sl_;
                e0 = rate_ * e0;
                e1 = rate_ * e1;
            }
        }
        const double hy_loss = -6 / 1000.0 * hy_to_use;
        const double real_price_dollar = in_price_next / 4;
        const double income_evs_fast = 0.42 / 4 * P0 - real_price_dollar * e0;
        const double income_evs_slow = 0.21 / 4 * P1 - real_price_dollar * e1;
        const double income_evs = income_evs_fast + income_evs_slow;
        const double income_evs_serve = 0.8 * (0.0 + F0 + F1);
        const double income_hys = 6 / 1000.0 * hy_use;
        const double not_meet_loss = -10 / 1000.0 * not_meet;
        const double hy_cost = -real_price_dollar * hydrogen_power;
        reward = DIV_K(income_hys + income_evs + income_evs_serve + hy_cost + 1 * hy_loss + not_meet_loss, 50);
        if (tel_on) {
            CHUB_TEL(0, act_el); CHUB_TEL(1, flow); CHUB_TEL(2, all_power_second); CHUB_TEL(4, cap);
            CHUB_TEL(5, total_mass_need); CHUB_TEL(6, hy_use); CHUB_TEL(7, not_meet); CHUB_TEL(8, fc_power);
            CHUB_TEL(9, hy_to_use); CHUB_TEL(10, used_renew); CHUB_TEL(13, hydrogen_power);
            CHUB_TEL(14, income_hys + income_evs + income_evs_serve + hy_cost); CHUB_TEL(15, reward);
            CHUB_TEL(19, (double) arrive); CHUB_TEL(20, (double) hv_line); CHUB_TEL(21, (double) q_len + (double) fold_n);
            CHUB_TEL(24, e0); CHUB_TEL(25, e1); CHUB_TEL(26, ev_power_sum);
            CHUB_TEL(27, in_price_next);
        }
        if (ep_on) {
            CHUB_G(double) lv = ctx->es.live;
            const size_t nn = n32, ee = e32;
            const double init_soc = EP ? ctx->ep.prm[PRM_INIT_SOC * n32 + e32] : hp.init_soc;
            double col[kEpCount];
            col[EPC_RETURN] = lv[EPC_RETURN * nn + ee] + reward;
            col[EPC_INCOME] = lv[EPC_INCOME * nn + ee] + (income_hys + income_evs + income_evs_serve + hy_cost);
            col[EPC_DRAW_ELE] = lv[EPC_DRAW_ELE * nn + ee] + ((e0 + e1) + hydrogen_power);
            col[EPC_LENGTH] = lv[EPC_LENGTH * nn + ee] + 1.0;
            col[EPC_DEVIATION] = fabs(store_soc - init_soc);
            col[EPC_TEST_PENALTY] = fabs(col[EPC_DEVIATION] * cap_mass / 1000 / 0.2);
            col[EPC_END_SOC] = store_soc;
#pragma unroll
            for (int c = 0; c < kEpCount; c++) lv[c * nn + ee] = col[c];
            if ((t_now + 1) >= 96) {
                CHUB_G(double) fin = ctx->es.fin;
#pragma unroll
                for (int c = 0; c < kEpCount; c++) fin[c * nn + ee] = col[c];
                ctx->es.episodes[ee] += 1u;
                ctx->es.pending[ee] = 1;
            }
        }
        }
    }

    ev.cap[e32] = cap;

    float *obs = s_out + (FUSED ? (int) (threadIdx.x & 63u) : (int) threadIdx.x) * row_w;
    double *o64 = tel_on ? (double *) ev.obs64 + (size_t) e32 * hp.obs_dim : nullptr;
    int n = 0;
#define CHUB_OBS(v)                    \
    do {                               \
        const double v_ = (v);         \
        obs[n] = (float) v_;           \
        if (o64) o64[n] = v_;          \
        n++;                           \
    } while (0)
    CHUB_OBS(sin_t);
    CHUB_OBS(div_c(price_next - hp.price_mean, hp.price_std, hp.rc_price_std));
    if (hp.S[0] > 0) {
        const double half_range = (double) hp.transformer_limit[0] / 2, rc_hr = hp.rc_half_range[0];
        CHUB_OBS(div_c((double) mn0 - half_range, half_range, rc_hr));
        CHUB_OBS(div_c((double) P0f - half_range, half_range, rc_hr));
        CHUB_OBS(div_c((double) mx0 - half_range, half_range, rc_hr));
        CHUB_OBS(DIV_K((double) ln0, 5));
    }
    if (hp.S[1] > 0) {
        const double half_range = (double) hp.transformer_limit[1] / 2, rc_hr = hp.rc_half_range[1];
        CHUB_OBS(div_c((double) mn1 - half_range, half_range, rc_hr));
        CHUB_OBS(div_c((double) P1f - half_range, half_range, rc_hr));
        CHUB_OBS(div_c((double) mx1 - half_range, half_range, rc_hr));
        CHUB_OBS(DIV_K((double) ln1, 5));
    }
    CHUB_OBS(store_soc);
    CHUB_OBS(DIV_K(re_pv, 42 * 5));
    CHUB_OBS(DIV_K(re_wd, 92 * 1));
#undef CHUB_OBS
    if (!RESET) {
        const bool dn = (t_now + 1) >= 96;
        if (sa.done_f32) {
            obs[n] = (float) reward;
            obs[n + 1] = dn ? 1.0f : 0.0f;
        } else {
            sa.reward[(size_t) e32 * sa.reward_stride] = (float) reward;
            if (sa.done) sa.done[e32] = (uint8_t) (dn ? 1 : 0);
            if (sa.done_f32) sa.done_f32[(size_t) e32 * sa.reward_stride] = dn ? 1.0f : 0.0f;
        }
    } else if (MULTI && sa.done_f32) {
        obs[n] = sa.reward[(size_t) e32 * sa.reward_stride];
        obs[n + 1] = sa.done_f32[(size_t) e32 * sa.reward_stride];
    }
    if (tel_on) {
        ev.reward64[e32] = reward;
        CHUB_TEL(3, store_soc); CHUB_TEL(16, re_pv); CHUB_TEL(17, re_wd); CHUB_TEL(18, price_next);
        CHUB_TEL(22, (double) pv_day); CHUB_TEL(23, (double) wd_day);
        CHUB_TEL(28, (double) mn0); CHUB_TEL(29, (double) P0f); CHUB_TEL(30, (double) mx0); CHUB_TEL(31, (double) ln0); CHUB_TEL(32, (double) F0i);
        CHUB_TEL(33, (double) mn1); CHUB_TEL(34, (double) P1f); CHUB_TEL(35, (double) mx1); CHUB_TEL(36, (double) ln1); CHUB_TEL(37, (double) F1i);
    }
    } while (0);
// ... 50 lines not shown
        const U4 ow = px.block(SITE_OU, 0, 0);
        const uint32_t hv_lev = px.block(SITE_HV, 0, 0).v[0] % 1000u;
        u32x4 d;
        d.x = __float_as_uint(normal_from_word(tb.normal_icdf, tb.normal_tail, ow.v[0]));
        d.y = __float_as_uint(normal_from_word(tb.normal_icdf, tb.normal_tail, ow.v[1]));
        d.z = __float_as_uint(normal_from_word(tb.normal_icdf, tb.normal_tail, ow.v[2]));
        const uint32_t cnt = EP ? hv_count_env(ctx->ep, e, t_next, hv_lev) : (uint32_t) tb.cnt_hv[(uint32_t) t_next * (uint32_t) kLevels + hv_lev];
        d.w = cnt != 0u ? __float_as_uint(soc_from_word(tb.soc_d_icdf, px.block(SITE_HVSOC, 0, 0).v[0])) : 0u;
        ((CHUB_G(u32x4)) ctx->ev.drw[(sa.tick + 1u) & 1u])[e] = d;
        ctx->ev.drw_cnt[(sa.tick + 1u) & 1u][e] = (uint8_t) cnt;
    }
}

template <bool RESET, int MODE, bool MULTI, bool TAPE = false, bool EP = false>
__global__ __launch_bounds__(kEnvBlock) void k_env(const DevCtx *__restrict__ ctx, StepArgs sa, TailArgs ta, int nb_env) {
    __shared__ double s_pv[100], s_wd[150], s_pv_now[100], s_wd_now[150], s_hy[102];
    __shared__ __attribute__((aligned(16))) uint8_t s_hv[kLevels];
    __shared__ __attribute__((aligned(16))) float s_out[kEnvBlock * 16];
    if (RESET && MULTI && mask_is_empty(sa)) return;
    if (MODE == MODE_PHILOX && (int) blockIdx.x >= nb_env) {
        int seg = 0;
        int64_t env_ = 0;
#if CHUB_TRACE
        CHUB_STAMP_DECL(16);
        CHUB_STAMP_REAL(8);
#endif
        const uint32_t jb = blockIdx.x - (uint32_t) nb_env, n32 = (uint32_t) ctx->hp.n_envs, per = n32 >> 3;
        bool have;
        if (!MULTI && ta.xcd && (n32 & 2047u) == 0u && ((uint32_t) nb_env & 7u) == 0u) {
            const uint32_t x = jb & 7u, i = jb >> 3, wpx = per / kEnvBlock;
            seg = (int) (i / wpx);
            env_ = (int64_t) (x * per + (i - (uint32_t) seg * wpx) * kEnvBlock + threadIdx.x);
            have = seg < 3;
        } else {
            have = range_unit(sa, (int64_t) jb * kEnvBlock + threadIdx.x, 3, seg, env_);
        }
        if (have) level_block<RESET, MULTI, EP>(ctx, sa, (int64_t) seg * ctx->hp.n_envs + env_);
#if CHUB_TRACE
        asm volatile("s_waitcnt vmcnt(0)" ::: "memory");
        CHUB_STAMP_REAL(9);
        if (sa.stamps_env && threadIdx.x == 0) {
            sa.stamps_env[(size_t) blockIdx.x * 16 + 8] = stamp_[8];
            sa.stamps_env[(size_t) blockIdx.x * 16 + 9] = stamp_[9];
        }
#endif
        return;
    }
    const int blk = (int) xcd_order(blockIdx.x, (uint32_t) nb_env, MULTI ? 0u : ta.xcd) + (MULTI ? sa.env_lo / kEnvBlock : 0);
    const int env = blk * kEnvBlock + (int) threadIdx.x;
    TailIn none;
    NoMid nomid;
    env_tail<RESET, MODE, MULTI, false, NoMid, kEnvBlock, TAPE, EP>(ctx, sa, env, env < (int) ta.n_envs && (!MULTI || in_group(sa, env)), s_pv, s_wd, s_pv_now,
                                                                s_wd_now, s_hy, s_hv, s_out, blk, ta, nullptr, 0, 0, 0, none, false, nomid);
}

__global__ __launch_bounds__(256) void k_env_walk(const DevCtx *__restrict__ ctx, StepArgs sa, TailArgs ta, StepArgs sw, int nb_env) {
    __shared__ __attribute__((aligned(16))) uint32_t lds[32 * 256 + 4 * kWalkStageWords];
    if ((int) blockIdx.x >= nb_env) {
        __builtin_amdgcn_s_setprio(3);
        compat_walk_block<false>(ctx, sw, blockIdx.x - (uint32_t) nb_env, lds, lds + 32 * 256);
        return;
    }
    double *s_pv = (double *) lds, *s_wd = s_pv + 100, *s_pv_now = s_wd + 150, *s_wd_now = s_pv_now + 100, *s_hy = s_wd_now + 150;
    uint8_t *s_hv = (uint8_t *) (s_hy + 102 + 2);
    float *s_out = (float *) (s_hv + 1008);
    static_assert((602 + 2) * 8 + 1008 + kEnvBlock * 16 * 4 <= 32 * 256 * 4 && kLevels <= 1008, "the tail's LDS inside the walk's");
    const int env = (int) blockIdx.x * kEnvBlock + (int) threadIdx.x;
    TailIn none;
    NoMid nomid;
    env_tail<false, MODE_COMPAT, false>(ctx, sa, env, env < (int) ta.n_envs, s_pv, s_wd, s_pv_now, s_wd_now, s_hy, s_hv, s_out, (int) blockIdx.x, ta, nullptr, 0, 0,
                                        0, none, false, nomid);
}

static_assert(64 * (1 + kCompatSmallWaves0 + kCompatSmallWaves1) == kCompatSmallBlock, "wave roles of k_compat_small");
struct SmallMid {
    __device__ __forceinline__ void operator()() {
        __builtin_amdgcn_fence(__ATOMIC_RELEASE, "agent");
        __syncthreads();
        __builtin_amdgcn_fence(__ATOMIC_ACQUIRE, "agent");
    }
};
template <bool RESET>
__global__ __launch_bounds__(kCompatSmallBlock) void k_compat_small(const DevCtx *__restrict__ ctx, StepArgs sa, TailArgs ta) {
    constexpr int BLOCK = kCompatSmallBlock;
    __shared__ float lds_f[BLOCK];
    __shared__ uint32_t lds_u[2 * BLOCK];
    __shared__ double s_pv[100], s_wd[150], s_pv_now[100], s_wd_now[150], s_hy[102];
    __shared__ __attribute__((aligned(16))) uint8_t s_hv[kLevels];
    __shared__ __attribute__((aligned(16))) float s_out[kEnvBlock * 16];
    const HubParams &hp = ctx->hp;
    const int wave = (int) (threadIdx.x >> 6);
    const int k = wave <= kCompatSmallWaves0 ? 0 : 1, wave0 = k ? 1 + kCompatSmallWaves0 : 1;
    SmallMid mid;
    if (!RESET && sa.empt_fresh) {
        if (wave >= 1) {
            const int lane = (int) (threadIdx.x & 63u), U = hp.U[k], S = hp.S[k];
            const int upw = 64 / U, uiw = lane / U, slot = lane - uiw * U;
            const int env = (wave - wave0) * upw + uiw;
            const bool unit_ok = uiw < upw && env < (int) hp.n_envs;
            const bool valid = unit_ok && slot < S;
            const uint64_t unit_mask = (U == 64) ? ~0ull : (uiw < upw ? (((1ull << U) - 1ull) << (uiw * U)) : 0ull);
            uint32_t w = 0u;
            if (valid) w = ctx->sl.hot[4 * ((size_t) hp.base[k] + (size_t) env * (size_t) S + (size_t) slot) + 3];
            const uint64_t be = __ballot(valid && hot_tl(w) <= 1) & unit_mask;
            if (unit_ok && slot == 0) ctx->st.empt[(uint32_t) k * (uint32_t) hp.n_envs + (uint32_t) env] = (uint8_t) __popcll(be);
        }
// ... 1391 lines not shown
template void launch_slot<true>(const CallPlan &, const HubParams &, const LaunchPlan &, const DevCtx *, const StepArgs &, hipStream_t, const PackedPtrs &,
                                hipEvent_t, hipEvent_t);
template void launch_slot<false>(const CallPlan &, const HubParams &, const LaunchPlan &, const DevCtx *, const StepArgs &, hipStream_t, const PackedPtrs &,
                                 hipEvent_t, hipEvent_t);

void launch_slot_walk2(const LaunchPlan &lp, const HubParams &hp, const DevCtx *ctx, const StepArgs &sa, const StepArgs &sw, hipStream_t stream,
                       hipEvent_t ev0, hipEvent_t ev1) {
    constexpr int BLOCK = 256;
    ev0 = launch_split_front(hp, ctx, sa, stream, ev0);
    const int64_t sb0 = blocks_for_split2(hp.n_envs, hp.U[0], BLOCK), sb1 = blocks_for_split2(hp.n_envs, hp.U[1], BLOCK);
    switch ((CompatForm) lp.compat) {
    case COMPAT_WALK2_32: {
        const int nwalk = (int) ((hp.n_envs + 31) / 32);
        CHUB_LAUNCH((k_slot_walk2<BLOCK, 32>), dim3((unsigned) (nwalk + sb0 + sb1)), dim3(BLOCK), stream, ev0, ev1, ctx, sa, sw, sb0, nwalk);
        break;
    }
    case COMPAT_WALK2_64: {
        const int nwalk = (int) ((hp.n_envs + 63) / 64);
        CHUB_LAUNCH((k_slot_walk2<BLOCK, 64>), dim3((unsigned) (nwalk + sb0 + sb1)), dim3(BLOCK), stream, ev0, ev1, ctx, sa, sw, sb0, nwalk);
        break;
    }
    default: break;
    }
}

static PackedArgs make_packed_args(const HubParams &hp, const StepArgs &sa, const PackedPtrs &pp) {
    PackedArgs pa;
    for (int k = 0; k < 2; k++) {
        pa.S[k] = (uint32_t) hp.S[k];
        pa.type[k] = (uint32_t) hp.type[k];
    }
    pa.n_envs = (uint32_t) hp.n_envs;
    pa.epb = (uint32_t) hp.epb;
    pa.magic = (1u << 20) / (uint32_t) (hp.S[0] + hp.S[1]) + 1u;
    pa.cls_delta = (uint32_t) ((const char *) pp.cls[1] - (const char *) pp.cls[0]);
    pa.state = (CHUB_G(uint32_t)) pp.hot;
    pa.rec = (CHUB_G(uint32_t)) pp.rec;
    pa.pk = (CHUB_G(const uint32_t)) pp.pk[sa.tick & 1u];
    pa.actions = sa.act_bits ? (CHUB_G(const float)) (const void *) sa.act_bits : (CHUB_G(const float)) sa.actions;
    pa.cls0 = (CHUB_G(const float)) pp.cls[0];
    pa.ttab2 = (CHUB_G(const float)) pp.ttab2;
    pa.car_tape = (CHUB_G(const uint32_t)) sa.car_tape;
    pa.key[0] = hp.key[0];
    pa.key[1] = hp.key[1];
    pa.gid0 = (uint32_t) hp.env_id0;
    pa.tick = sa.tick;
    pa.tick_base = hp.tick_base;
    for (int j = 0; j < 8; j++) pa.late[j] = pp.late8[j];
    pa.env_mask = (CHUB_G(const uint8_t)) sa.env_mask;
    pa.blk0 = sa.env_mask ? (uint32_t) (sa.env_lo / hp.epb) : 0u;
    pa.xcd = hp.xcd ? (uint32_t) ((hp.n_envs + hp.epb - 1) / hp.epb) : 0u;
    pa.tail_act = (CHUB_G(float)) pp.st->tail_act;
    pa.stay8 = (CHUB_G(uint8_t)) pp.stay8;
    return pa;
}

void launch_step_fused(const CallPlan &cp, const HubParams &hp, const DevCtx *ctx, const StepArgs &sa, hipStream_t stream, const PackedPtrs &pp,
                       hipEvent_t ev0, hipEvent_t ev1) {
    launch_levels(cp.levels, ctx, sa, stream);
    const PackedArgs pa = make_packed_args(hp, sa, pp);
    TailArgs ta = make_tail_args(*pp.ev, *pp.st, hp, sa, pp, false);
    ta.tail_act = (cp.one == ONE_FUSED_BITS || cp.one == ONE_TAILWAVE_BITS) ? (CHUB_G(const float)) sa.act_tail : nullptr;
    const uint32_t nb = (uint32_t) ((hp.n_envs + hp.epb - 1) / hp.epb);
    switch (cp.one) {
    case ONE_FUSED: CHUB_LAUNCH((k_step_fused<kPackedBlock, kSlotsPerLane>), dim3(nb), dim3(kPackedBlock), stream, ev0, ev1, ctx, sa, pa, ta); break;
    case ONE_TAILWAVE: CHUB_LAUNCH((k_step_tailwave<kPackedBlock, kSlotsPerLane>), dim3(nb), dim3(kPackedBlock + 64), stream, ev0, ev1, ctx, sa, pa, ta); break;
    case ONE_FUSED_BITS: CHUB_LAUNCH((k_step_fused<kPackedBlock, kSlotsPerLane, true>), dim3(nb), dim3(kPackedBlock), stream, ev0, ev1, ctx, sa, pa, ta); break;
    case ONE_TAILWAVE_BITS:
        CHUB_LAUNCH((k_step_tailwave<kPackedBlock, kSlotsPerLane, true>), dim3(nb), dim3(kPackedBlock + 64), stream, ev0, ev1, ctx, sa, pa, ta);
        break;
    case ONE_FUSED_TAPE:
        CHUB_LAUNCH((k_step_fused<kPackedBlock, kSlotsPerLane, false, true>), dim3(nb), dim3(kPackedBlock), stream, ev0, ev1, ctx, sa, pa, ta);
        break;
    case ONE_NONE: break;
    }
}

void launch_steps_fused(const HubParams &hp, const LaunchPlan &lp, const DevCtx *ctx, const StepArgs &sa, hipStream_t stream, const PackedPtrs &pp,
                        int n_steps, int pc0, int64_t first, const float *const *batches, int n_batches, float *const *packed2) {
    launch_levels(sa.fresh ? LEVELS_DRAW : LEVELS_NONE, ctx, sa, stream);
    const PackedArgs pa = make_packed_args(hp, sa, pp);
    TailArgs ta = make_tail_args(*pp.ev, *pp.st, hp, sa, pp, false);
    ta.tail_act = nullptr;
    SpanArgs sp = {};
    sp.n_steps = n_steps;
    sp.pc0 = pc0;
    sp.first = (uint32_t) (first % (2 * n_batches));
    sp.n_batches = n_batches;
    sp.D = hp.obs_dim;
    for (int j = 0; j < 8; j++) sp.actions[j] = batches[j < n_batches ? j : 0];
    sp.packed[0] = packed2[0];
    sp.packed[1] = packed2[1];
    for (int q = 0; q < 2; q++) {
        sp.pk[q] = (CHUB_G(const uint32_t)) pp.pk[q];
        sp.drw[q] = (CHUB_G(const uint32_t)) pp.ev->drw[q];
        sp.drw_cnt[q] = (CHUB_G(const uint8_t)) pp.ev->drw_cnt[q];
    }
    sp.price = (CHUB_G(const double)) pp.tb->price;
    sp.pvT = (CHUB_G(const double)) pp.tb->pvT;
    sp.wdT = (CHUB_G(const double)) pp.tb->wdT;
    sp.sin96 = (CHUB_G(const double)) pp.tb->sin96;
    const uint32_t nb = (uint32_t) ((hp.n_envs + hp.epb - 1) / hp.epb);
    if (lp.span_piped)
        hipLaunchKernelGGL((k_steps_piped<kPackedBlock, kSlotsPerLane>), dim3(nb), dim3(kPackedBlock + 64), 0, stream, ctx, sa, pa, ta, sp);
    else
        hipLaunchKernelGGL((k_steps_fused<kPackedBlock, kSlotsPerLane>), dim3(nb), dim3(kPackedBlock), 0, stream, ctx, sa, pa, ta, sp);
// ... 1 lines not shown

template <bool RESET>
void launch_compat_small(const HubParams &hp, const DevCtx *ctx, const StepArgs &sa, hipStream_t stream, const PackedPtrs &pp) {
    const TailArgs ta = make_tail_args(*pp.ev, *pp.st, hp, sa, pp, RESET);
    hipLaunchKernelGGL(k_compat_small<RESET>, dim3(1), dim3(kCompatSmallBlock), 0, stream, ctx, sa, ta);
}
template void launch_compat_small<true>(const HubParams &, const DevCtx *, const StepArgs &, hipStream_t, const PackedPtrs &);
template void launch_compat_small<false>(const HubParams &, const DevCtx *, const StepArgs &, hipStream_t, const PackedPtrs &);

template <bool RESET>
void launch_env(EnvForm f, const HubParams &hp, const DevCtx *ctx, const StepArgs &sa, hipStream_t stream, hipEvent_t ev0, hipEvent_t ev1,
                const PackedPtrs &pp) {
    const TailArgs ta = make_tail_args(*pp.ev, *pp.st, hp, sa, pp, RESET);
    const int nb_env = sa.env_clk ? sa.env_hi / kEnvBlock - sa.env_lo / kEnvBlock + 1 : (int) ((hp.n_envs + kEnvBlock - 1) / kEnvBlock);
    if (sa.env_clk && sa.env_mask) {
        const int64_t N = hp.n_envs;
        hipLaunchKernelGGL(k_keep_clocks, dim3((unsigned) ((N + 255) / 256)), dim3(256), 0, stream, sa.env_clk + (int64_t) ((sa.tick + 1u) & 1u) * N,
                           (const uint16_t *) sa.env_clk + (int64_t) (sa.tick & 1u) * N, N);
    }
    const unsigned nb = (unsigned) nb_env + (unsigned) ((3 * ((int64_t) sa.env_hi - sa.env_lo + 1) + kEnvBlock - 1) / kEnvBlock);
    switch (f) {
    case ENV_PHILOX: CHUB_LAUNCH((k_env<RESET, MODE_PHILOX, false>), dim3(nb), dim3(kEnvBlock), stream, ev0, ev1, ctx, sa, ta, nb_env); break;
    case ENV_PHILOX_CLOCKS: CHUB_LAUNCH((k_env<RESET, MODE_PHILOX, true>), dim3(nb), dim3(kEnvBlock), stream, ev0, ev1, ctx, sa, ta, nb_env); break;
    case ENV_PHILOX_TAPE:
        CHUB_LAUNCH((k_env<RESET, MODE_PHILOX, false, true>), dim3(nb), dim3(kEnvBlock), stream, ev0, ev1, ctx, sa, ta, nb_env);
        break;
    case ENV_COMPAT: CHUB_LAUNCH((k_env<RESET, MODE_COMPAT, false>), dim3((unsigned) nb_env), dim3(kEnvBlock), stream, ev0, ev1, ctx, sa, ta, nb_env); break;
    case ENV_COMPAT_CLOCKS: CHUB_LAUNCH((k_env<RESET, MODE_COMPAT, true>), dim3((unsigned) nb_env), dim3(kEnvBlock), stream, ev0, ev1, ctx, sa, ta, nb_env); break;
    case ENV_PHILOX_PARAMS:
        CHUB_LAUNCH((k_env<RESET, MODE_PHILOX, false, false, true>), dim3(nb), dim3(kEnvBlock), stream, ev0, ev1, ctx, sa, ta, nb_env);
        break;
    case ENV_PHILOX_PARAMS_CLOCKS:
        CHUB_LAUNCH((k_env<RESET, MODE_PHILOX, true, false, true>), dim3(nb), dim3(kEnvBlock), stream, ev0, ev1, ctx, sa, ta, nb_env);
        break;
    case ENV_COMPAT_PARAMS:
        CHUB_LAUNCH((k_env<RESET, MODE_COMPAT, false, false, true>), dim3((unsigned) nb_env), dim3(kEnvBlock), stream, ev0, ev1, ctx, sa, ta, nb_env);
        break;
    case ENV_COMPAT_PARAMS_CLOCKS:
        CHUB_LAUNCH((k_env<RESET, MODE_COMPAT, true, false, true>), dim3((unsigned) nb_env), dim3(kEnvBlock), stream, ev0, ev1, ctx, sa, ta, nb_env);
        break;
    }
}
template void launch_env<true>(EnvForm, const HubParams &, const DevCtx *, const StepArgs &, hipStream_t, hipEvent_t, hipEvent_t, const PackedPtrs &);
template void launch_env<false>(EnvForm, const HubParams &, const DevCtx *, const StepArgs &, hipStream_t, hipEvent_t, hipEvent_t, const PackedPtrs &);

void launch_env_walk(const HubParams &hp, const DevCtx *ctx, const StepArgs &sa, const StepArgs &sw, hipStream_t stream, hipEvent_t ev0, hipEvent_t ev1,
                     const PackedPtrs &pp) {
    const TailArgs ta = make_tail_args(*pp.ev, *pp.st, hp, sa, pp, false);
    const int nb_env = (int) ((hp.n_envs + kEnvBlock - 1) / kEnvBlock);
    const unsigned nb = (unsigned) nb_env + (unsigned) ((hp.n_envs + 255) / 256);
    CHUB_LAUNCH(k_env_walk, dim3(nb), dim3(kEnvBlock), stream, ev0, ev1, ctx, sa, ta, sw, nb_env);
}

__global__ void k_tick_advance(uint32_t *tick_base, uint32_t by) { *tick_base += by; }


__global__ void k_expand_bits(int64_t n_envs, int S, int W, const uint64_t *__restrict__ bits, const float *__restrict__ tail,
                              float *__restrict__ actions) {
    const uint32_t A = (uint32_t) S + 2u;
    const uint32_t total = (uint32_t) n_envs * A;
    for (uint32_t i = blockIdx.x * blockDim.x + threadIdx.x; i < total; i += gridDim.x * blockDim.x) {
        const uint32_t env = i / A;
        const uint32_t j = i - env * A;
        float v;
        if (j < (uint32_t) S) v = ((bits[(size_t) env * (size_t) W + (j >> 6)] >> (j & 63u)) & 1ull) ? 1.0f : -1.0f;
        else v = tail[env * 2u + (j - (uint32_t) S)];
        actions[i] = v;
    }
}
void launch_expand_bits(const HubParams &hp, const uint64_t *d_bits, const float *d_tail, float *d_actions, hipStream_t stream) {
    const int S = hp.S[0] + hp.S[1];
    const int64_t total = hp.n_envs * (int64_t) (S + 2);
    int64_t nb = (total + 255) / 256;
    if (nb > 16384) nb = 16384;
    hipLaunchKernelGGL(k_expand_bits, dim3((unsigned) nb), dim3(256), 0, stream, hp.n_envs, S, (S + 63) / 64, d_bits, d_tail, d_actions);
}

__global__ void k_fill_clocks(uint16_t *dst, int64_t n, uint16_t value) {
    const int64_t i = (int64_t) blockIdx.x * blockDim.x + threadIdx.x;
    if (i < n) dst[i] = value;
}
void launch_fill_clocks(uint16_t *dst, int64_t n, uint16_t value, hipStream_t stream) {
    hipLaunchKernelGGL(k_fill_clocks, dim3((unsigned) ((n + 255) / 256)), dim3(256), 0, stream, dst, n, value);
}
void launch_keep_clocks(uint16_t *dst, const uint16_t *src, int64_t n, hipStream_t stream) {
    hipLaunchKernelGGL(k_keep_clocks, dim3((unsigned) ((n + 255) / 256)), dim3(256), 0, stream, dst, src, n);
}
void launch_tick_advance(uint32_t *tick_base, uint32_t by, hipStream_t stream) {
    hipLaunchKernelGGL(k_tick_advance, dim3(1), dim3(1), 0, stream, tick_base, by);
}

__device__ __forceinline__ void copy_span(CHUB_G(uint8_t) d, CHUB_G(const uint8_t) s, uint32_t n, uint32_t lane) {
    const uint32_t al = (uint32_t) (uintptr_t) d | (uint32_t) (uintptr_t) s;
    uint32_t done = 0u;
    if ((al & 15u) == 0u) {
        const uint32_t nv = n >> 4;
        for (uint32_t i = lane; i < nv; i += 64u) ((CHUB_G(u32x4)) d)[i] = ((CHUB_G(const u32x4)) s)[i];
        done = nv << 4;
    }
    if ((al & 3u) == 0u) {
        const uint32_t nw = (n - done) >> 2;
        for (uint32_t i = lane; i < nw; i += 64u) ((CHUB_G(uint32_t)) (d + done))[i] = ((CHUB_G(const uint32_t)) (s + done))[i];
        done += nw << 2;
    }
    for (uint32_t i = done + lane; i < n; i += 64u) d[i] = s[i];
}
// ... 211 lines not shown
```

### charginghub-env_amd/csrc/chub_plan.h

```cpp
#pragma once

#include <stdint.h>

#include <algorithm>

#include "../../include/chub.h"
#include "chub_device.h"

namespace chub {

#ifndef CHUB_XCD_ANY_TILE
#define CHUB_XCD_ANY_TILE 0
#endif
#ifndef CHUB_SPLIT2
#define CHUB_SPLIT2 1
#endif
constexpr int64_t kBigTileSlots = (int64_t) 10 << 20;
constexpr int64_t kXcdOrderSlots = (int64_t) 6 << 20;
constexpr int kPipedMaxBlocks = 256;
constexpr int kFusedMaxBlocksTailWave = 768;
constexpr int kSpanMaxBlocks = 384;
constexpr int kFusedMaxBlocks = 384;
constexpr int64_t kWalk2HalfMaxEnvs = 40000;

enum PackedForm : int32_t {
    PACKED_NONE = 0, PACKED_SMALL = 1, PACKED_SMALL_WIDE = 2, PACKED_LARGE = 3, PACKED_LARGE_WIDE = 4
};
enum OneLaunch : int32_t {
    ONE_NONE = 0, ONE_FUSED = 1, ONE_TAILWAVE = 2, ONE_FUSED_BITS = 3, ONE_TAILWAVE_BITS = 4, ONE_FUSED_TAPE = 5
};
enum CompatForm : int32_t {
    COMPAT_NONE = 0,
    COMPAT_STATIONS = 1,
    COMPAT_SPLIT = 2,
    COMPAT_WALK2_32 = 3,
    COMPAT_WALK2_64 = 4
};
enum StationKernel : int32_t {
    STATION_WAVE = 0,
    STATION_UNIT = 1,
    STATION_UNIT_ANY = 2,
    STATION_CURVES = 3
};

struct LaunchPlan {
    int32_t packed;
    int32_t big_tile;
    int32_t pblock, pslots;
    int32_t epb;
    int32_t xcd;
    int32_t one_launch;
    int32_t span_size_ok;
    int32_t span_piped;
    int32_t span_steps;
    int32_t compat_small;
    int32_t compat;
    int32_t split2;
    int32_t walk_ahead;
    int32_t station[2];
};
static_assert(sizeof(LaunchPlan) == CHUB_PLAN_COUNT * sizeof(int32_t), "LaunchPlan mirrors the CHUB_PLAN_* list");

inline int plan_handle(const chub_config *cfg, int64_t n_envs, int rng_mode, const chub_options &opt, LaunchPlan &p, const char **msg) {
    auto refuse = [&](int code, const char *m) {
        *msg = m;
        return code;
    };
    if (opt.slot_kernel < 0 || opt.slot_kernel > 2) return refuse(CHUB_ERR_ARG, "chub_options.slot_kernel must be 0, 1 or 2");
    if (opt.fused_step < 0 || opt.fused_step > 2) return refuse(CHUB_ERR_ARG, "chub_options.fused_step must be 0, 1 or 2");
    if (opt.tile < 0 || opt.tile > 2) return refuse(CHUB_ERR_ARG, "chub_options.tile must be 0, 1 or 2");
    if (opt.walk_ahead < 0 || opt.walk_ahead > 1) return refuse(CHUB_ERR_ARG, "chub_options.walk_ahead must be 0 or 1");
    if (opt.work_order < 0 || opt.work_order > 1) return refuse(CHUB_ERR_ARG, "chub_options.work_order must be 0 or 1");
    if (opt.span_steps < 0 || opt.span_steps > 96) return refuse(CHUB_ERR_ARG, "chub_options.span_steps must be 0 .. 96");
    if (opt.span_tails < 0 || opt.span_tails > 2)
        return refuse(CHUB_ERR_ARG, "chub_options.span_tails must be 0 (by size), 1 (on the last slot wave) or 2 (on a wave of their own)");
// ... 26 lines not shown
    const int pb = p.pblock * p.pslots;
    p.epb = pb / St > 0 ? pb / St : 1;
    if (p.epb > pb / 4) p.epb = pb / 4;
    bool magic_ok = true;
    for (int l = 0; l < pb && magic_ok; l++)
        if ((((uint32_t) l * ((1u << 20) / (uint32_t) St + 1u)) >> 20) != (uint32_t) (l / St)) magic_ok = false;
    const bool packed = rng_mode == CHUB_RNG_PHILOX && St <= pb && magic_ok &&
                        (uint64_t) n_envs * (uint64_t) (St + 2) * 16u < ((uint64_t) 1 << 32) &&
                        opt.slot_kernel != 1;
    const bool large = p.pblock == kBigBlock;
    p.packed = !packed ? PACKED_NONE : large ? (small_units ? PACKED_LARGE : PACKED_LARGE_WIDE) : (small_units ? PACKED_SMALL : PACKED_SMALL_WIDE);

    const int64_t nb = (n_envs + p.epb - 1) / p.epb;
    const bool can = packed && small_units && p.pblock == kPackedBlock;
    const bool fused = can && (opt.fused_step == 2 || (opt.fused_step == 0 && nb <= (p.epb <= 64 ? kFusedMaxBlocksTailWave : kFusedMaxBlocks)));
    p.one_launch = !fused ? ONE_NONE : p.epb <= 64 ? ONE_TAILWAVE : ONE_FUSED;
    p.span_size_ok = (nb <= kSpanMaxBlocks || opt.fused_step == 2) ? 1 : 0;
    const bool can_pipe = p.one_launch == ONE_TAILWAVE;
    p.span_piped = (can_pipe && (opt.span_tails == 2 || (opt.span_tails == 0 && nb <= kPipedMaxBlocks))) ? 1 : 0;
    p.span_steps = opt.span_steps;

    const int U0 = S0 > 0 ? (S0 < 64 ? S0 : 64) : 1, U1 = S1 > 0 ? (S1 < 64 ? S1 : 64) : 1;
    const int64_t fit = std::min<int64_t>(64, std::min<int64_t>(kCompatSmallWaves0 * (64 / U0), kCompatSmallWaves1 * (64 / U1)));
    p.compat_small = (compat && opt.fused_step != 1 && small_units && n_envs <= fit) ? 1 : 0;
    const bool split = compat && small_units && opt.slot_kernel != 1;
    p.split2 = (split && CHUB_SPLIT2 && U0 >= 8 && U1 >= 8) ? 1 : 0;
    p.walk_ahead = (split && opt.walk_ahead == 0) ? 1 : 0;
    const bool walk2 = p.walk_ahead && p.split2 && !p.compat_small;
    p.compat = !compat ? COMPAT_NONE : !split ? COMPAT_STATIONS : !walk2 ? COMPAT_SPLIT : n_envs <= kWalk2HalfMaxEnvs ? COMPAT_WALK2_32 : COMPAT_WALK2_64;

    if (opt.fused_step == 2 && !can)
        return refuse(CHUB_ERR_UNSUPPORTED, "fused_step = 2: the single-launch step covers PHILOX handles on the packed slot kernel with "
                                            "stations of at most 64 piles");
    if (opt.span_tails == 2 && !can_pipe)
        return refuse(CHUB_ERR_UNSUPPORTED, "span_tails = 2: the tail wave of a span covers handles on the one-launch step (fused_step) with at most 64 envs "
                                            "per workgroup (hubs of 8 piles and more)");
    return CHUB_OK;
}

inline int plan_params(LaunchPlan &p, int rng_mode, const char **msg) {
    (void) msg;
    if (rng_mode == CHUB_RNG_COMPAT) {
        p.compat = COMPAT_STATIONS;
        p.compat_small = 0;
        p.split2 = 0;
        p.walk_ahead = 0;
    }
    p.one_launch = ONE_NONE;
    p.span_size_ok = 0;
    p.span_piped = 0;
    return CHUB_OK;
}

enum CallForm : int32_t {
    CALL_COMPAT_SMALL,
    CALL_ONE_LAUNCH,
    CALL_SLOT_WALK2,
    CALL_SLOT_ENV_WALK,
    CALL_SLOT_ENV
};
enum SlotForm : int32_t {
    SLOT_PACKED, SLOT_PACKED_MASKED, SLOT_PACKED_TAPE, SLOT_PACKED_BITS,
    SLOT_CURVES,
    SLOT_WAVE,
    SLOT_STATIONS,
    SLOT_SPLIT,
    SLOT_SPLIT2,
    SLOT_COMPAT_STATIONS
};
enum LevelsForm : int32_t { LEVELS_NONE, LEVELS_DRAW, LEVELS_RESET };
enum EnvForm : int32_t { ENV_PHILOX, ENV_PHILOX_CLOCKS, ENV_PHILOX_TAPE, ENV_COMPAT, ENV_COMPAT_CLOCKS,
                         ENV_PHILOX_PARAMS, ENV_PHILOX_PARAMS_CLOCKS, ENV_COMPAT_PARAMS, ENV_COMPAT_PARAMS_CLOCKS };

struct CallState {
    bool reset, load_mode;
    bool per_env;
    bool all_served;
    bool capturing;
    bool car_tape, pk_tape, tail_tape;
    bool bits;
    bool fresh;
    bool env_params;
    bool dev_mask;
};
struct CallPlan {
    CallForm call;
    OneLaunch one;
    SlotForm slot;
    LevelsForm levels;
    EnvForm env;
};

inline bool slot_form_split(SlotForm f) { return f == SLOT_SPLIT || f == SLOT_SPLIT2; }

inline SlotForm slot_form(const LaunchPlan &p, const CallState &c) {
    if (p.station[0] == STATION_CURVES) return SLOT_CURVES;
    if (p.packed != PACKED_NONE && !c.load_mode)
        return c.car_tape ? SLOT_PACKED_TAPE : c.bits && !c.reset ? SLOT_PACKED_BITS : !c.all_served ? SLOT_PACKED_MASKED : SLOT_PACKED;
    switch ((CompatForm) p.compat) {
    case COMPAT_NONE: return (p.station[0] == STATION_WAVE && p.station[1] == STATION_WAVE) ? SLOT_WAVE : SLOT_STATIONS;
    case COMPAT_STATIONS: return SLOT_COMPAT_STATIONS;
    default: return (p.split2 && !c.reset && !c.load_mode) ? SLOT_SPLIT2 : SLOT_SPLIT;
    }
}

inline CallPlan plan_call(const LaunchPlan &p, const CallState &c_in) {
// ... 37 lines not shown
```

### charginghub-env_amd/csrc/chub_runtime.cpp

```cpp
#include <hip/hip_runtime.h>
#include <math.h>
#include <stdint.h>
#include <stdio.h>
#include <string.h>
#include <stdlib.h>

#include <algorithm>
#include <map>
#include <string>
#include <vector>

#include "../../include/chub.h"
#include "chub_device.h"
#include "chub_plan.h"
#include "chub_policy.h"
#include "chub_critic.h"

namespace chub {
template <bool RESET>
void launch_slot(const CallPlan &cp, const HubParams &hp, const LaunchPlan &lp, const DevCtx *ctx, const StepArgs &sa, hipStream_t stream,
                 const PackedPtrs &pp, hipEvent_t ev0, hipEvent_t ev1);
void launch_check_ttab(const DevCtx *ctx, uint32_t *d_mismatch, hipStream_t stream);
void launch_build_cls_soc(const DevCtx *ctx, float *d_out, hipStream_t stream);
void launch_pile_obs(const HubParams &hp, const DevCtx *ctx, uint32_t fields, const uint8_t *d_mask, const float *d_cls_soc, float *d_out,
                     hipStream_t stream);
void launch_pile_set(const HubParams &hp, const DevCtx *ctx, int which, const uint8_t *d_mask, uint64_t *d_bits, hipStream_t stream);
void launch_station_profile(const HubParams &hp, const DevCtx *ctx, uint32_t fields, int buckets, const uint8_t *d_mask, const float *d_cls_soc,
                            float *d_out, hipStream_t stream);
void launch_load_dispatch(const HubParams &hp, const DevCtx *ctx, int units, const uint8_t *d_mask, const float *d_cls_soc, const float *d_loads,
                          const float *d_tail, float *d_actions, uint64_t *d_bits, hipStream_t stream);
void launch_forecast(const HubParams &hp, const DevCtx *ctx, const ForecastTabs &ft, uint32_t fields, int horizon, int t, const uint16_t *d_clk,
                     const uint8_t *d_mask, float *d_out, hipStream_t stream);
template <typename OUT>
void launch_step_terms(const HubParams &hp, const DevCtx *ctx, uint32_t fields, const uint8_t *d_mask, OUT *d_out, hipStream_t stream);
template <bool RESET>
void launch_env(EnvForm f, const HubParams &hp, const DevCtx *ctx, const StepArgs &sa, hipStream_t stream, hipEvent_t ev0, hipEvent_t ev1,
                const PackedPtrs &pp);
void launch_random_actions(const HubParams &hp, uint64_t key, uint32_t batch, float *d_actions, hipStream_t stream);
void launch_compat_ctor_sweep(const HubParams &hp, const DevCtx *ctx, int rng_cur, hipStream_t stream, bool env_params);
void launch_tick_advance(uint32_t *tick_base, uint32_t by, hipStream_t stream);
void launch_fill_clocks(uint16_t *dst, int64_t n, uint16_t value, hipStream_t stream);
void launch_keep_clocks(uint16_t *dst, const uint16_t *src, int64_t n, hipStream_t stream);
void launch_expand_bits(const HubParams &hp, const uint64_t *d_bits, const float *d_tail, float *d_actions, hipStream_t stream);
void launch_copy_envs(int layout, const CopyArgs &a, hipStream_t stream);
void launch_episode_summary(const HubParams &hp, const DevCtx *ctx, double *d_partials, double *d_out, int drain, hipStream_t stream);
void launch_step_fused(const CallPlan &cp, const HubParams &hp, const DevCtx *ctx, const StepArgs &sa, hipStream_t stream, const PackedPtrs &pp,
                       hipEvent_t ev0, hipEvent_t ev1);
template <bool RESET>
void launch_compat_small(const HubParams &hp, const DevCtx *ctx, const StepArgs &sa, hipStream_t stream, const PackedPtrs &pp);
void launch_steps_fused(const HubParams &hp, const LaunchPlan &lp, const DevCtx *ctx, const StepArgs &sa, hipStream_t stream, const PackedPtrs &pp,
                        int n_steps, int pc0, int64_t first, const float *const *batches, int n_batches, float *const *packed2);
void launch_slot_walk2(const LaunchPlan &lp, const HubParams &hp, const DevCtx *ctx, const StepArgs &sa, const StepArgs &sw, hipStream_t stream,
                       hipEvent_t ev0, hipEvent_t ev1);
void launch_env_walk(const HubParams &hp, const DevCtx *ctx, const StepArgs &sa, const StepArgs &sw, hipStream_t stream, hipEvent_t ev0, hipEvent_t ev1,
                     const PackedPtrs &pp);
}

using namespace chub;

static thread_local std::string g_err;

static int fail(int code, const std::string &msg) {
    g_err = msg;
    return code;
}
static int refuse_params(const char *what) {
    return fail(CHUB_ERR_UNSUPPORTED, std::string(what) + " is not supported on a handle with per-env hub parameters (chub_create_params)");
}
extern "C" __attribute__((visibility("hidden"))) int chub_set_last_error_(int code, const char *msg) { return fail(code, msg); }

#define HIP_TRY(expr)                                                                                   \
    do {                                                                                                \
        hipError_t e_ = (expr);                                                                         \
        if (e_ != hipSuccess)                                                                           \
            return fail(CHUB_ERR_HIP, std::string(#expr) + ": " + hipGetErrorString(e_));               \
    } while (0)

struct chub_env {
    chub_config cfg;
    HubParams hp;
    SlotArrays sl;
    StationArrays st;
    EnvArrays ev;
    CompatRng cr;
    Tables tb;
    int device;
    LaunchPlan plan;
    int rng_cur = 0;
    uint32_t walked_tick = 0;
    uint32_t e2_tick = ~0u;
    bool empt_valid;
    DevCtx *d_ctx;
    bool ctx_dirty;
    int t;
    int price_count;
    uint32_t tick;
    bool per_env;
    uint16_t *d_env_clk;
    uint8_t *d_mask;
    uint8_t *h_mask;
    hipEvent_t mask_done[2];
    uint32_t mask_seq;
    uint32_t *d_tick_note = nullptr;
    uint8_t *d_done_mask = nullptr;
    uint32_t *d_done_count = nullptr;
    uint32_t done_seq = 0;
    std::vector<void *> cap_masks;
    std::vector<uint32_t> cap_rel;
    uint32_t cap_full_rel;
    bool graph_per_env0;
    uint32_t graph_full_tick0;
    std::vector<uint32_t> graph_h_tick0;
    std::vector<uint32_t> h_tick;
    uint32_t full_tick;
    bool predrawn;
    double price[96];
    double hy_table[102];
    std::vector<void *> allocs;
    char *arena;
    size_t arena_size, arena_used;
    float *d_actions, *d_obs, *d_reward;
    uint8_t *d_done;
    double *d_exo_z;
    int32_t *d_exo_days;
    hipStream_t stream;
    hipStream_t host_stream;
    hipStream_t upload_stream;
    float *h_actions, *h_packed;
    uint64_t *h_bits, *d_bits;
    float *h_tail, *d_tail;
    float *d_packed;
    double *h_telem;
    double *d_telem = nullptr;
    int tape_classes;
    bool tape_stale = false;
    bool env_params = false;
    chub_env_params *d_rows = nullptr;
    int hv_max_arrive = 0;
    int hv_top[96];
    EnvParamArrays ep = {nullptr, nullptr, nullptr};
// ... 296 lines not shown
static int write_env_params(chub_env *e, const uint8_t *mask, const chub_env_params *rows);
static int create_impl(const chub_config *cfg_in, const char *data_dir, int64_t n_envs, int64_t env_id0, int device, uint64_t seed, int rng_mode,
                       const chub_options *opt_in, const chub_env_params *rows, chub_env **out);

int chub_create(const chub_config *cfg, const char *data_dir, int64_t n_envs, int64_t env_id0, int device,
                uint64_t seed, int rng_mode, chub_env **out) {
    return chub_create_ex(cfg, data_dir, n_envs, env_id0, device, seed, rng_mode, nullptr, out);
}
int chub_create_ex(const chub_config *cfg, const char *data_dir, int64_t n_envs, int64_t env_id0, int device,
                   uint64_t seed, int rng_mode, const chub_options *opt, chub_env **out) {
    return create_impl(cfg, data_dir, n_envs, env_id0, device, seed, rng_mode, opt, nullptr, out);
}
int chub_create_params(const chub_config *cfg, const char *data_dir, int64_t n_envs, int64_t env_id0, int device, uint64_t seed, int rng_mode,
                       const chub_options *opt, const chub_env_params *rows, chub_env **out) {
    if (!rows) return fail(CHUB_ERR_ARG, "null argument");
    return create_impl(cfg, data_dir, n_envs, env_id0, device, seed, rng_mode, opt, rows, out);
}


static int create_impl(const chub_config *cfg_in, const char *data_dir, int64_t n_envs, int64_t env_id0, int device, uint64_t seed, int rng_mode,
                       const chub_options *opt_in, const chub_env_params *rows, chub_env **out) {
    if (!cfg_in || !data_dir || !out) return fail(CHUB_ERR_ARG, "null argument");
    chub_options opt;
    memset(&opt, 0, sizeof opt);
    if (opt_in) opt = *opt_in;
    *out = nullptr;
    LaunchPlan plan;
    const char *msg = nullptr;
    if (const int rc = plan_handle(cfg_in, n_envs, rng_mode, opt, plan, &msg)) return fail(rc, msg);
    if (rows)
        if (const int rc = plan_params(plan, rng_mode, &msg)) return fail(rc, msg);
    const bool soc_curves = rng_mode == CHUB_RNG_PHILOX_CURVES;
    const int public_mode = rng_mode;
    if (soc_curves) rng_mode = CHUB_RNG_PHILOX;
    chub_config cfg_eff = *cfg_in;
    if (rows) {
        for (int64_t i = 0; i < n_envs; i++) {
            const chub_env_params &r = rows[i];
            if (const int rc = check_scalars(r.init_soc, r.hydro_prod_rate, r.hydro_store_vlt, r.fc_max_power, " (env " + std::to_string(i) + ")")) return rc;
        }
        const chub_env_params &r = rows[0];
        cfg_eff.hydro_prod_rate = r.hydro_prod_rate; cfg_eff.hydro_store_vlt = r.hydro_store_vlt; cfg_eff.init_soc = r.init_soc;
        cfg_eff.fc_max_power = r.fc_max_power; cfg_eff.fcev_permeate = r.fcev_permeate; cfg_eff.renew_fluctuate = r.renew_fluctuate;
        cfg_eff.price_fluctuate = r.price_fluctuate; cfg_eff.hydro_loss = r.hydro_loss;
    } else if (const int rc = check_scalars(cfg_in->init_soc, cfg_in->hydro_prod_rate, cfg_in->hydro_store_vlt, cfg_in->fc_max_power, "")) {
        return rc;
    }
    const chub_config *cfg = &cfg_eff;

    chub_env *e = new chub_env();
    e->cfg = *cfg_in;
    e->env_params = rows != nullptr;
    e->plan = plan;
    e->public_mode = public_mode;
    e->device = device;
    e->t = 0;
    e->price_count = 0;
    e->tick = 0;
    e->per_env = false;
    e->d_env_clk = nullptr;
    e->d_mask = nullptr;
    e->h_mask = nullptr;
    e->mask_done[0] = e->mask_done[1] = nullptr;
    e->mask_seq = 0;
    e->cap_full_rel = 0;
    e->graph_per_env0 = false;
    e->graph_full_tick0 = 0;
    e->full_tick = 0;
    e->predrawn = false;
    e->stream = nullptr;
    e->host_stream = nullptr;
    e->upload_stream = nullptr;
    e->h_actions = e->h_packed = e->d_packed = nullptr;
    e->h_bits = e->d_bits = nullptr;
    e->h_tail = e->d_tail = nullptr;
    e->h_telem = nullptr;
    e->empt_valid = false;
    e->prof_used = e->prof_cap = 0;
    e->prof_on = false;
    e->arena = nullptr;
    e->arena_size = e->arena_used = 0;
    auto bail = [&](int rc) {
        chub_destroy(e);
        return rc;
    };

    std::string dir(data_dir);
    std::vector<float> cdf;
    int rc;
    if ((rc = load_cdf(dir + "/car_flow_possibility_list_save.csv", cdf))) return bail(rc);
    std::vector<double> pv(100 * 96), wd(150 * 96);
    if ((rc = load_f64(dir + "/price_96.f64", e->price, 96))) return bail(rc);
    if ((rc = load_f64(dir + "/pv_100x96.f64", pv.data(), pv.size()))) return bail(rc);
    if ((rc = load_f64(dir + "/wd_150x96.f64", wd.data(), wd.size()))) return bail(rc);

    {
        int ndev = 0;
        if (hipGetDeviceCount(&ndev) != hipSuccess || ndev <= 0)
            return bail(fail(CHUB_ERR_HIP, "no HIP device available: libchub has no CPU path"));
        if (device < 0 || device >= ndev) return bail(fail(CHUB_ERR_ARG, "device ordinal out of range"));
        hipError_t he = hipSetDevice(device);
        if (he != hipSuccess) return bail(fail(CHUB_ERR_HIP, std::string("hipSetDevice: ") + hipGetErrorString(he)));
    }

    int hv_max_arrive = 0;
    {
// ... 380 lines not shown
        rc = chub_set_rng_compat_seeds(e, seeds.data());
        if (rc) {
            *out = nullptr;
            return bail(rc);
        }
        uint32_t *d_bad = nullptr, bad = 0u;
        if ((rc = sync_ctx(e, nullptr))) {
            *out = nullptr;
            return bail(rc);
        }
        if (hipMalloc((void **) &d_bad, sizeof(uint32_t)) != hipSuccess || hipMemset(d_bad, 0, sizeof(uint32_t)) != hipSuccess) {
            if (d_bad) (void) hipFree(d_bad);
            *out = nullptr;
            return bail(fail(CHUB_ERR_HIP, "hipMalloc failed"));
        }
        launch_check_ttab(e->d_ctx, d_bad, nullptr);
        const hipError_t he = hipMemcpy(&bad, d_bad, sizeof(uint32_t), hipMemcpyDeviceToHost);
        (void) hipFree(d_bad);
        if (he != hipSuccess || bad != 0u) {
            *out = nullptr;
            return bail(fail(he != hipSuccess ? CHUB_ERR_HIP : CHUB_ERR_UNSUPPORTED,
                             he != hipSuccess ? "the target-time table could not be checked on the device"
                                              : "the device's soc_to_time differs from the host-built table of target times"));
        }
    }
    {
        const size_t b_mean = fc_mean.size() * sizeof(float), b_hist = fc_hist.size() * sizeof(uint32_t), b_len = fc_hist_len.size() * sizeof(uint16_t);
        char *d = nullptr;
        if (hipMalloc((void **) &d, b_mean + b_hist + b_len) != hipSuccess) return bail(fail(CHUB_ERR_HIP, "hipMalloc failed"));
        e->fc.mean = (const float *) d;
        if (b_hist) {
            e->fc.hist = (const uint32_t *) (d + b_mean);
            e->fc.hist_len = (const uint16_t *) (d + b_mean + b_hist);
        }
        if (hipMemcpy(d, fc_mean.data(), b_mean, hipMemcpyHostToDevice) != hipSuccess ||
            (b_hist && (hipMemcpy(d + b_mean, fc_hist.data(), b_hist, hipMemcpyHostToDevice) != hipSuccess ||
                        hipMemcpy(d + b_mean + b_hist, fc_hist_len.data(), b_len, hipMemcpyHostToDevice) != hipSuccess)))
            return bail(fail(CHUB_ERR_HIP, "the look-ahead tables could not be uploaded"));
    }
    if (rng_mode == CHUB_RNG_PHILOX && !soc_curves) {
        if (hipMalloc((void **) &e->d_cls_soc, (size_t) 2 * kSocLevels * kClsRow * sizeof(float)) != hipSuccess) {
            e->d_cls_soc = nullptr;
            return bail(fail(CHUB_ERR_HIP, "hipMalloc failed"));
        }
        if ((rc = sync_ctx(e, nullptr))) return bail(rc);
        launch_build_cls_soc(e->d_ctx, e->d_cls_soc, nullptr);
        if (hipGetLastError() != hipSuccess || hipStreamSynchronize(nullptr) != hipSuccess)
            return bail(fail(CHUB_ERR_HIP, "the SoC table of the arrival classes could not be built on the device"));
    }
    if (hipMalloc((void **) &e->d_gae_part, (size_t) ((n_envs + kGaeLanes - 1) / kGaeLanes) * 3 * sizeof(double)) != hipSuccess) {
        e->d_gae_part = nullptr;
        return bail(fail(CHUB_ERR_HIP, "hipMalloc failed"));
    }
    *out = e;
    return CHUB_OK;
}

static void policy_free(chub_policy *pol);
static void moments_free(chub_moments *m);
static void critic_free(chub_critic *c);

int chub_destroy(chub_env *e) {
    if (!e) return CHUB_OK;
    while (!e->moments.empty()) moments_free(e->moments.back());
    while (!e->policies.empty()) policy_free(e->policies.back());
    while (!e->critics.empty()) critic_free(e->critics.back());
    if (!e->allocs.empty() || !e->prof_events.empty()) {
        (void) hipSetDevice(e->device);
        (void) hipDeviceSynchronize();
        for (void *p : e->allocs) (void) hipFree(p);
        for (hipEvent_t ev : e->prof_events) (void) hipEventDestroy(ev);
        if (e->h_actions) (void) hipHostFree(e->h_actions);
        if (e->h_mask) (void) hipHostFree(e->h_mask);
        for (hipEvent_t ev : e->mask_done)
            if (ev) (void) hipEventDestroy(ev);
        if (e->h_packed) (void) hipHostFree(e->h_packed);
        if (e->h_telem) (void) hipHostFree(e->h_telem);
        if (e->d_telem) (void) hipFree(e->d_telem);
        if (e->d_ledger) (void) hipFree(e->d_ledger);
        if (e->d_cls_soc) (void) hipFree(e->d_cls_soc);
        if (e->fc.mean) (void) hipFree((void *) e->fc.mean);
        if (e->d_ep_sum) (void) hipFree(e->d_ep_sum);
        if (e->d_gae_part) (void) hipFree(e->d_gae_part);
        if (e->h_bits) (void) hipHostFree(e->h_bits);
        if (e->d_bits) (void) hipFree(e->d_bits);
        if (e->d_packed) (void) hipFree(e->d_packed);
        if (e->host_stream) (void) hipStreamDestroy(e->host_stream);
        if (e->upload_stream) (void) hipStreamDestroy(e->upload_stream);
    }
    (void) hipGetLastError();
    delete e;
    return CHUB_OK;
}

int chub_obs_dim(const chub_env *e) { return e ? e->hp.obs_dim : CHUB_ERR_ARG; }
int chub_act_dim(const chub_env *e) { return e ? e->hp.act_dim : CHUB_ERR_ARG; }
int64_t chub_num_envs(const chub_env *e) { return e ? e->hp.n_envs : CHUB_ERR_ARG; }
int chub_clock(const chub_env *e) {
    if (!e) return CHUB_ERR_ARG;
    if (!e->per_env) return e->t;
    uint16_t c = 0;
    if (hipSetDevice(e->device) != hipSuccess || hipDeviceSynchronize() != hipSuccess ||
        hipMemcpy(&c, e->d_env_clk + (size_t) ((e->tick + 1u - e->graph_base) & 1u) * (size_t) e->hp.n_envs, sizeof c, hipMemcpyDeviceToHost) != hipSuccess)
        return CHUB_ERR_HIP;
    return (int) (c & 127u);
}
int chub_uses_packed_kernel(const chub_env *e) { return e ? e->hp.packed : CHUB_ERR_ARG; }
int chub_uses_xcd_order(const chub_env *e) {
    return e ? ((e->hp.packed && e->hp.xcd && e->plan.one_launch == ONE_NONE) ? 1 : 0) : CHUB_ERR_ARG;
}
int chub_uses_fused_step(const chub_env *e) { return e ? ((e->plan.one_launch != ONE_NONE || e->plan.compat_small) ? 1 : 0) : CHUB_ERR_ARG; }

int chub_launch_plan(const chub_config *cfg, int64_t n_envs, int rng_mode, const chub_options *opt_in, int32_t *out) {
    if (!cfg || !out) return fail(CHUB_ERR_ARG, "null argument");
    chub_options opt;
    memset(&opt, 0, sizeof opt);
    if (opt_in) opt = *opt_in;
    LaunchPlan p;
    const char *msg = nullptr;
    if (const int rc = plan_handle(cfg, n_envs, rng_mode, opt, p, &msg)) return fail(rc, msg);
    memcpy(out, &p, sizeof p);
    return CHUB_OK;
}

int chub_launch_plan_params(const chub_config *cfg, int64_t n_envs, int rng_mode, const chub_options *opt_in, int32_t *out) {
    if (!cfg || !out) return fail(CHUB_ERR_ARG, "null argument");
    chub_options opt;
    memset(&opt, 0, sizeof opt);
    if (opt_in) opt = *opt_in;
    LaunchPlan p;
    const char *msg = nullptr;
    if (const int rc = plan_handle(cfg, n_envs, rng_mode, opt, p, &msg)) return fail(rc, msg);
    if (const int rc = plan_params(p, rng_mode, &msg)) return fail(rc, msg);
    memcpy(out, &p, sizeof p);
    return CHUB_OK;
}

int chub_sync(chub_env *e) {
    if (!e) return fail(CHUB_ERR_ARG, "null handle");
    HIP_TRY(hipSetDevice(e->device));
    HIP_TRY(hipDeviceSynchronize());
    return CHUB_OK;
}


struct OutSink {
    float *obs, *reward;
    int obs_stride, reward_stride;
    uint8_t *done;
    float *done_f32;
};
static OutSink dense_out(const chub_env *e, float *obs, float *reward, uint8_t *done) { return {obs, reward, e->hp.obs_dim, 1, done, nullptr}; }
static OutSink packed_out(const chub_env *e, float *packed) {
    const int D = e->hp.obs_dim;
    return {packed, packed + D, D + 2, D + 2, nullptr, packed + D + 1};
}

struct StepCall {
    bool reset;
    int load_mode;
    const uint8_t *mask;
    const uint8_t *dmask;
    uint8_t *done_mask;
    uint32_t *done_count;
// ... 463 lines not shown
    c.bits = (flags & CHUB_CALL_BITS) != 0;
    c.load_mode = (flags & CHUB_CALL_LOAD) != 0;
    c.capturing = (flags & CHUB_CALL_CAPTURING) != 0;
    c.env_params = env_params != 0;
    const CallPlan r = plan_call(p, c);
    out[CHUB_CALLPLAN_CALL] = r.call;
    out[CHUB_CALLPLAN_ONE] = r.one;
    out[CHUB_CALLPLAN_SLOT] = r.slot;
    out[CHUB_CALLPLAN_LEVELS] = r.levels;
    out[CHUB_CALLPLAN_ENV] = r.env;
    return CHUB_OK;
}

int chub_step_load_envs_device(chub_env *e, const uint8_t *mask, const float *d_actions, const double *d_exo_z, float *d_obs, float *d_reward,
                               uint8_t *d_done, void *stream) {
    if (!e || !mask || !d_actions || !d_obs || !d_reward || !d_done) return fail(CHUB_ERR_ARG, "null argument");
    return run_call(e, step_call(mask, d_actions, d_exo_z, dense_out(e, d_obs, d_reward, d_done), 1), (hipStream_t) stream);
}

int chub_step_gather(chub_env *e, chub_comm *comm, const float *d_actions, float *d_packed, float *d_gathered, void *stream) {
    if (!e || !comm || !d_actions) return fail(CHUB_ERR_ARG, "null argument");
    const bool root = chub_comm_rank(comm) == 0;
    if (root && !d_gathered) return fail(CHUB_ERR_ARG, "rank 0 needs the gathered buffer");
    if (!root && !d_packed) return fail(CHUB_ERR_ARG, "null argument");
    float *out = root ? d_gathered : d_packed;
    int rc = chub_comm_gather_begin(comm, out, stream);
    if (rc) return rc;
    if (e->capturing) e->cap_comm = comm;
    rc = chub_step_device_packed(e, d_actions, nullptr, out, stream);
    if (rc) return rc;
    return chub_comm_gather(comm, out, d_gathered, e->hp.n_envs * (int64_t) (e->hp.obs_dim + 2) * (int64_t) sizeof(float), stream);
}

static bool span_ok(const chub_env *e, int n_batches) {
    return e->plan.one_launch != ONE_NONE && e->plan.span_size_ok && e->plan.span_steps != 1 && !e->per_env && !e->prof_on && !e->tape_only &&
           n_batches <= 8 && e->tick != 0 && !e->hp.telemetry && !e->es.on;
}

static int run_span(chub_env *e, const float *const *batches, int n_batches, float *const *packed2, int64_t first, int k, hipStream_t s) {
    HIP_TRY(hipSetDevice(e->device));
    (void) hipGetLastError();
    if (e->t + k > 96) return fail(CHUB_ERR_ARG, "a span of steps ends at the day's end at the latest");
    const StepCall c = step_call(nullptr, batches[first % n_batches], nullptr, packed_out(e, packed2[first & 1]), 0);
    const MaskView all = {nullptr, 0, e->hp.n_envs - 1};
    StepArgs sa;
    if (const int rc = fill_args(e, c, 2, all, e->tick + 1u, s, sa)) return rc;
    launch_steps_fused(e->hp, e->plan, e->d_ctx, sa, s, packed_ptrs(e), k, e->price_count, first, batches, n_batches, packed2);
    HIP_TRY(hipGetLastError());
    e->tick += (uint32_t) k;
    advance_clocks(e, c, 2, k);
    return note_served(e, nullptr, 2, s);
}

int chub_run_steps(chub_env *e, chub_comm *comm, const float *const *d_action_batches, int n_batches, float *const *d_packed2,
                   float *const *d_gathered2, float *d_reset_obs, int64_t first_step, int64_t n_steps, void *stream) {
    if (!e || !d_action_batches || n_batches <= 0 || !d_packed2 || !d_packed2[0] || !d_packed2[1] || !d_reset_obs || first_step < 0 ||
        n_steps < 0)
        return fail(CHUB_ERR_ARG, "bad argument");
    for (int64_t i = first_step; i < first_step + n_steps; i++) {
        int rc;
        if (i % 96 == 0 && (rc = chub_reset_device(e, nullptr, nullptr, d_reset_obs, stream))) return rc;
        if (!comm) {
            int64_t k = first_step + n_steps - i;
            k = k < 96 - i % 96 ? k : 96 - i % 96;
            k = k < 96 - e->t ? k : 96 - e->t;
            if (e->plan.span_steps > 1 && k > e->plan.span_steps) k = e->plan.span_steps;
            if (k >= 2 && span_ok(e, n_batches)) {
                if ((rc = run_span(e, d_action_batches, n_batches, d_packed2, i, (int) k, (hipStream_t) stream))) return rc;
                i += k - 1;
                continue;
            }
        }
        const float *act = d_action_batches[i % n_batches];
        float *packed = d_packed2[i & 1];
        if (comm) rc = chub_step_gather(e, comm, act, packed, d_gathered2 ? d_gathered2[i & 1] : nullptr, stream);
        else rc = chub_step_device_packed(e, act, nullptr, packed, stream);
        if (rc) return rc;
    }
    return CHUB_OK;
}

static int fetch_clocks(chub_env *e, std::vector<uint16_t> &c) {
    const size_t N = (size_t) e->hp.n_envs;
    c.assign(N, (uint16_t) ((uint32_t) e->t | (((uint32_t) e->price_count & 3u) << 8)));
    if (!e->per_env) return CHUB_OK;
    HIP_TRY(hipSetDevice(e->device));
    HIP_TRY(hipDeviceSynchronize());
    HIP_TRY(hipMemcpy(c.data(), e->d_env_clk + (size_t) ((e->tick + 1u - e->graph_base) & 1u) * N, N * sizeof(uint16_t), hipMemcpyDeviceToHost));
    return CHUB_OK;
}

int chub_env_clocks(chub_env *e, int32_t *t_out, uint32_t *tick_out) {
    if (!e || !t_out) return fail(CHUB_ERR_ARG, "null argument");
    const size_t N = (size_t) e->hp.n_envs;
    std::vector<uint16_t> c;
    int rc = fetch_clocks(e, c);
    if (rc) return rc;
    if (e->per_env && tick_out) {
        std::vector<uint32_t> note(N);
        HIP_TRY(hipMemcpy(note.data(), e->d_tick_note, N * sizeof(uint32_t), hipMemcpyDeviceToHost));
        if (e->h_tick.size() != N) e->h_tick.assign(N, 0u);
        for (size_t i = 0; i < N; i++)
            if (note[i] > e->h_tick[i]) e->h_tick[i] = note[i];
    }
    for (size_t i = 0; i < N; i++) {
        t_out[i] = (int32_t) (c[i] & 127u);
        if (tick_out) tick_out[i] = (e->h_tick.size() == N && e->h_tick[i] > e->full_tick) ? e->h_tick[i] : e->full_tick;
    }
    return CHUB_OK;
}

int chub_clock_groups(chub_env *e) {
    if (!e) return CHUB_ERR_ARG;
    std::vector<uint16_t> c;
// ... 3188 lines not shown
```

### charginghub-env_amd/vec_env.py

```python
import ctypes as C

import numpy as np

from . import _lib
from ._lib import ChubConfig, ChubError, ChubOptions, check, load_library


def make_config(station_list, station_type_list, constant_charging=False, hydro_prod_rate=None, hydro_store_vlt=None,
                init_soc=0.5, fc_max_power=None, fcev_permeate=0.01, renew_fluctuate=0, price_fluctuate=0,
                hydro_loss=0):
    if not (len(station_list) == len(station_type_list) == 2):
        raise AssertionError("station_list and station_type_list must both have 2 entries")
    cfg = ChubConfig()
    for k in range(2):
        cfg.station_list[k] = int(station_list[k])
        if station_type_list[k] == "fast":
            cfg.station_type_list[k] = _lib.CHUB_FAST
        elif station_type_list[k] == "slow":
            cfg.station_type_list[k] = _lib.CHUB_SLOW
        else:
            raise ValueError("EVS type must be fast or slow")
    cfg.constant_charging = int(bool(constant_charging))
    cfg.hydro_prod_rate = 430.0 if hydro_prod_rate is None else float(hydro_prod_rate)
    cfg.hydro_store_vlt = 5000.0 if hydro_store_vlt is None else float(hydro_store_vlt)
# ... 902 lines not shown
    def step_bits_device(self, d_pile_bits, d_tail, d_obs, d_reward, d_done, d_exo_z=0, stream=0):
        check(self._lib.chub_step_bits_device(self._h, d_pile_bits, d_tail, d_exo_z or None, d_obs, d_reward, d_done, stream or None))

    def step_bits_device_packed(self, d_pile_bits, d_tail, d_packed, d_exo_z=0, stream=0):
        check(self._lib.chub_step_bits_device_packed(self._h, d_pile_bits, d_tail, d_exo_z or None, d_packed, stream or None))

    def reset_envs_dmask_device(self, d_mask, d_obs, d_exo_days=0, d_exo_z=0, stream=0):
        check(self._lib.chub_dmask_reset_envs_device(self._h, d_mask, d_exo_days or None, d_exo_z or None, d_obs, stream or None))

    def step_envs_dmask_device(self, d_mask, d_actions, d_obs, d_reward, d_done, d_exo_z=0, stream=0):
        check(self._lib.chub_dmask_step_envs_device(self._h, d_mask, d_actions, d_exo_z or None, d_obs, d_reward, d_done, stream or None))

    def step_autoreset_device(self, d_actions, d_packed, d_final_obs=0, d_exo_z=0, d_reset_exo_days=0, d_reset_exo_z=0, stream=0):
        check(self._lib.chub_autoreset_step_device(self._h, d_actions, d_exo_z or None, d_reset_exo_days or None, d_reset_exo_z or None,
                                                   d_packed, d_final_obs or None, stream or None))

    def random_actions_device(self, d_actions, key, batch, stream=0):
        check(self._lib.chub_random_actions_device(self._h, int(key), int(batch), d_actions, stream or None))

    def graph_begin(self, stream):
        check(self._lib.chub_graph_begin(self._h, stream))

    def graph_end(self, stream):
        g = C.c_void_p()
        check(self._lib.chub_graph_end(self._h, stream, C.byref(g)))
        return g

    def graph_launch(self, graph, stream):
        check(self._lib.chub_graph_launch(graph, stream))

    def graph_destroy(self, graph):
        self._lib.chub_graph_destroy(graph)

    def profile_begin(self, max_steps, every=1):
        check(self._lib.chub_profile_begin(self._h, int(max_steps), int(every)))

    def profile_end(self):
        a, b, n = C.c_double(), C.c_double(), C.c_int()
        check(self._lib.chub_profile_end(self._h, C.byref(a), C.byref(b), C.byref(n)))
        return a.value, b.value, n.value

    def sync(self):
        check(self._lib.chub_sync(self._h))

    @property
    def uses_packed_kernel(self):
        return bool(self._lib.chub_uses_packed_kernel(self._h))

    @property
    def uses_fused_step(self):
        return bool(self._lib.chub_uses_fused_step(self._h))

    @property
    def uses_xcd_order(self):
        return bool(self._lib.chub_uses_xcd_order(self._h))

    @property
    def clock(self):
        return self._lib.chub_clock(self._h)

    def set_telemetry(self, on=True):
        check(self._lib.chub_set_telemetry(self._h, int(bool(on))))
        self._tel_views = None

    def telemetry_views(self):
        if getattr(self, "_tel_views", None) is None:
            pt, po, pr = C.c_void_p(), C.c_void_p(), C.c_void_p()
            check(self._lib.chub_telemetry_host(self._h, C.byref(pt), C.byref(po), C.byref(pr)))
            N, D, T = self.n_envs, self.obs_dim, _lib.T_COUNT
            view = lambda p, n, shape: np.frombuffer((C.c_double * n).from_address(p.value), dtype=np.float64).reshape(shape)
            self._tel_views = (view(pt, T * N, (T, N)), view(po, N * D, (N, D)), view(pr, N, (N,)))
        return self._tel_views

    def slots(self):
        out = np.zeros((self.n_envs, 9 * self.n_slots), dtype=np.float32)
        check(self._lib.chub_get_slots(self._h, _ptr(out)))
        s0 = self.piles[0]
        a = out[:, :9 * s0].reshape(self.n_envs, 9, s0)
        b = out[:, 9 * s0:].reshape(self.n_envs, 9, self.piles[1])
        return [a, b]

    def pile_obs_device(self, d_out, fields=None, d_mask=0, stream=0):
        check(self._lib.chub_pile_obs_device(self._h, _lib.pile_fields_mask(fields), d_mask or None, d_out, stream or None))

    def pile_obs(self, fields=None):
        mask = _lib.pile_fields_mask(fields)
        out = np.zeros((self.n_envs, len(_lib.pile_fields_names(mask)), self.n_slots), dtype=np.float32)
        if out.size == 0:
            return out
        d = C.c_void_p()
        check(self._lib.chub_malloc_device(self._device, out.nbytes, C.byref(d)))
        try:
            check(self._lib.chub_sync(self._h))
            check(self._lib.chub_pile_obs_device(self._h, mask, None, d, None))
            check(self._lib.chub_copy_to_host(self._device, _ptr(out), d, out.nbytes, None))
        finally:
            self._lib.chub_free_device(self._device, d)
        return out

    def pile_set_device(self, d_bits, which="decidable", d_mask=0, stream=0):
        check(self._lib.chub_pile_set_device(self._h, _lib.pile_set(which), d_mask or None, d_bits, stream or None))

    def pile_set(self, which="decidable"):
        words = np.zeros((self.n_envs, self.bit_words), dtype=np.uint64)
        d = C.c_void_p()
        check(self._lib.chub_malloc_device(self._device, words.nbytes, C.byref(d)))
# ... 244 lines not shown
```

### include/chub.h

```cpp
#ifndef CHUB_H
#define CHUB_H

#include <stdint.h>

#ifdef __cplusplus
extern "C" {
#endif

#define CHUB_VERSION 1

enum {
    CHUB_OK = 0,
    CHUB_ERR_ARG = -1,
    CHUB_ERR_DATA = -2,
    CHUB_ERR_HIP = -3,
    CHUB_ERR_UNSUPPORTED = -4,
    CHUB_ERR_COMM = -5
};

enum { CHUB_FAST = 0, CHUB_SLOW = 1 };

enum { CHUB_RNG_COMPAT = 0, CHUB_RNG_PHILOX = 1, CHUB_RNG_PHILOX_CURVES = 2 };

typedef struct chub_config {
// ... 7 lines not shown
    double fc_max_power;
    double fcev_permeate;
    double renew_fluctuate;
    double price_fluctuate;
    double hydro_loss;
} chub_config;

typedef struct chub_env chub_env;

typedef struct chub_options {
    int32_t slot_kernel;
    int32_t no_arena;
    int32_t fused_step;
    int32_t tile;
    int32_t walk_ahead;
    int32_t work_order;
    int32_t span_steps;
    int32_t span_tails;
} chub_options;

enum {
    CHUB_T_HY_ACT = 0, CHUB_T_HY_FLOW_SPEED, CHUB_T_ALL_POWER_SECOND, CHUB_T_STORE_SOC, CHUB_T_CAPACITY,
    CHUB_T_TOTAL_MASS_NEED, CHUB_T_HY_USE, CHUB_T_NOT_MEET, CHUB_T_FC_POWER, CHUB_T_HY_TO_USE,
    CHUB_T_USED_RENEW, CHUB_T_EV0, CHUB_T_EV1, CHUB_T_HYDROGEN_POWER, CHUB_T_INCOME, CHUB_T_REWARD,
    CHUB_T_RE_PV, CHUB_T_RE_WD, CHUB_T_PRICE_NEXT, CHUB_T_HV_ARRIVE, CHUB_T_HV_LINE, CHUB_T_QUEUE_LEN,
    CHUB_T_PV_DAY, CHUB_T_WD_DAY,
    CHUB_T_EV0_NET, CHUB_T_EV1_NET, CHUB_T_EV_SUM_NET, CHUB_T_PRICE_NOW,
    CHUB_T_MIN0, CHUB_T_CHG0, CHUB_T_MAX0, CHUB_T_LINE0, CHUB_T_FLOW0, CHUB_T_MIN1, CHUB_T_CHG1, CHUB_T_MAX1, CHUB_T_LINE1, CHUB_T_FLOW1,
    CHUB_T_COUNT
};

int chub_create(const chub_config *cfg, const char *data_dir, int64_t n_envs, int64_t env_id0, int device,
                uint64_t seed, int rng_mode, chub_env **out);
int chub_create_ex(const chub_config *cfg, const char *data_dir, int64_t n_envs, int64_t env_id0, int device,
                   uint64_t seed, int rng_mode, const chub_options *opt , chub_env **out);
int chub_destroy(chub_env *env);

typedef struct chub_env_params {
    double hydro_prod_rate;
    double hydro_store_vlt;
    double init_soc;
    double fc_max_power;
    double fcev_permeate;
    double renew_fluctuate;
    double price_fluctuate;
    double hydro_loss;
} chub_env_params;
int chub_create_params(const chub_config *cfg, const char *data_dir, int64_t n_envs, int64_t env_id0, int device, uint64_t seed, int rng_mode,
                       const chub_options *opt , const chub_env_params *rows , chub_env **out);
int chub_set_env_params(chub_env *env, const uint8_t *mask , const chub_env_params *rows );
int chub_get_env_params(chub_env *env, chub_env_params *rows );
int chub_has_env_params(const chub_env *env);
int chub_launch_plan_params(const chub_config *cfg, int64_t n_envs, int rng_mode, const chub_options *opt , int32_t *out);

int chub_obs_dim(const chub_env *env);
int chub_act_dim(const chub_env *env);
int64_t chub_num_envs(const chub_env *env);
int chub_clock(const chub_env *env);
int chub_uses_packed_kernel(const chub_env *env);
int chub_uses_fused_step(const chub_env *env);
int chub_uses_xcd_order(const chub_env *env);

int chub_launch_plan(const chub_config *cfg, int64_t n_envs, int rng_mode, const chub_options *opt , int32_t *out);
enum {
    CHUB_PLAN_PACKED = 0,
    CHUB_PLAN_BIG_TILE,
    CHUB_PLAN_PBLOCK,
    CHUB_PLAN_PSLOTS,
    CHUB_PLAN_EPB,
    CHUB_PLAN_XCD,
    CHUB_PLAN_ONE_LAUNCH,
    CHUB_PLAN_SPAN_SIZE_OK,
    CHUB_PLAN_SPAN_PIPED,
    CHUB_PLAN_SPAN_STEPS,
    CHUB_PLAN_COMPAT_SMALL,
    CHUB_PLAN_COMPAT,
    CHUB_PLAN_SPLIT2,
    CHUB_PLAN_WALK_AHEAD,
    CHUB_PLAN_STATION0,
    CHUB_PLAN_STATION1,
    CHUB_PLAN_COUNT
};

int chub_reset(chub_env *env, const int32_t *exo_days, const double *exo_z, float *obs);
int chub_step(chub_env *env, const float *actions, const double *exo_z, float *obs, float *reward, uint8_t *done);
int chub_host_actions(chub_env *env, float **out);

int chub_step_bits(chub_env *env, const uint64_t *pile_bits, const float *tail, const double *exo_z, float *obs, float *reward,
                   uint8_t *done);
int chub_host_bits(chub_env *env, uint64_t **pile_bits_out, float **tail_out);
int chub_step_bits_device(chub_env *env, const uint64_t *d_pile_bits, const float *d_tail, const double *d_exo_z, float *d_obs,
                          float *d_reward, uint8_t *d_done, void *stream);
int chub_step_bits_device_packed(chub_env *env, const uint64_t *d_pile_bits, const float *d_tail, const double *d_exo_z, float *d_packed,
                                 void *stream);

int chub_reset_device(chub_env *env, const int32_t *d_exo_days, const double *d_exo_z, float *d_obs, void *stream);
int chub_step_device(chub_env *env, const float *d_actions, const double *d_exo_z, float *d_obs, float *d_reward,
                     uint8_t *d_done, void *stream);

int chub_reset_envs(chub_env *env, const uint8_t *mask, const int32_t *exo_days, const double *exo_z, float *obs);
int chub_step_envs(chub_env *env, const uint8_t *mask, const float *actions, const double *exo_z, float *obs, float *reward,
                   uint8_t *done);
int chub_reset_envs_device(chub_env *env, const uint8_t *mask , const int32_t *d_exo_days, const double *d_exo_z, float *d_obs,
                           void *stream);
int chub_step_envs_device(chub_env *env, const uint8_t *mask , const float *d_actions, const double *d_exo_z, float *d_obs,
                          float *d_reward, uint8_t *d_done, void *stream);
// ... 355 lines not shown
```

Baseline: 2.661 billion env-steps/s.

## Run two lock-step Philox steps per launch pair with prefetched tail inputs

After: 2.752 billion env-steps/s (median of 6 runs). 1.03x the previous value.

```diff
diff --git a/charginghub-env_amd/_lib.py b/charginghub-env_amd/_lib.py
--- a/charginghub-env_amd/_lib.py
+++ b/charginghub-env_amd/_lib.py
@@ -381,6 +381,7 @@
         "chub_obs_dim": (I, [P]), "chub_act_dim": (I, [P]), "chub_num_envs": (L, [P]), "chub_clock": (I, [P]), "chub_uses_packed_kernel": (I, [P]), "chub_uses_fused_step": (I, [P]), "chub_uses_xcd_order": (I, [P]),
         "chub_launch_plan": (I, [C.POINTER(ChubConfig), L, I, C.POINTER(ChubOptions), P]),
         "chub_launch_plan_params": (I, [C.POINTER(ChubConfig), L, I, C.POINTER(ChubOptions), P]),
+        "chub_pair_plan": (I, [C.POINTER(ChubConfig), L, I, C.POINTER(ChubOptions), I, C.c_uint32, I, L, P]), "chub_uses_pair_tails": (I, [P]),
         "chub_create_params": (I, [C.POINTER(ChubConfig), C.c_char_p, L, L, I, C.c_uint64, I, C.POINTER(ChubOptions), P, C.POINTER(P)]),
         "chub_set_env_params": (I, [P, P, P]), "chub_get_env_params": (I, [P, P]), "chub_has_env_params": (I, [P]),
         "chub_reset": (I, [P, P, P, P]),
@@ -489,7 +490,7 @@
     return lib
 
 
-EXPORTED = ["chub_create", "chub_create_ex", "chub_destroy", "chub_obs_dim", "chub_act_dim", "chub_num_envs", "chub_clock", "chub_uses_packed_kernel", "chub_uses_fused_step", "chub_uses_xcd_order", "chub_launch_plan", "chub_launch_plan_params",
+EXPORTED = ["chub_create", "chub_create_ex", "chub_destroy", "chub_obs_dim", "chub_act_dim", "chub_num_envs", "chub_clock", "chub_uses_packed_kernel", "chub_uses_fused_step", "chub_uses_xcd_order", "chub_launch_plan", "chub_launch_plan_params", "chub_pair_plan", "chub_uses_pair_tails",
             "chub_create_params", "chub_set_env_params", "chub_get_env_params", "chub_has_env_params", "chub_reset",
             "chub_step", "chub_host_actions", "chub_step_bits", "chub_host_bits", "chub_step_bits_device", "chub_step_bits_device_packed", "chub_reset_device", "chub_step_device", "chub_step_device_packed", "chub_step_load", "chub_step_load_device", "chub_step_load_envs", "chub_step_load_envs_device", "chub_reset_envs", "chub_step_envs", "chub_reset_envs_device", "chub_step_envs_device",
             "chub_env_clocks", "chub_clock_groups", "chub_dmask_reset_envs_device", "chub_dmask_step_envs_device", "chub_autoreset_step_device", "chub_call_plan", "chub_random_actions_device", "chub_sync", "chub_profile_begin", "chub_profile_end",
diff --git a/charginghub-env_amd/csrc/chub_device.h b/charginghub-env_amd/csrc/chub_device.h
--- a/charginghub-env_amd/csrc/chub_device.h
+++ b/charginghub-env_amd/csrc/chub_device.h
@@ -251,6 +251,14 @@
     uint32_t late8[8];
     const Tables *tb;
     const double *sin96;
+};
+
+struct PairBufs {
+    uint32_t *rec_a;
+    float *tail_act_a;
+    uint64_t *pkraw;
+    uint32_t *drw[2][2];
+    uint8_t *cnt[2][2];
 };
 
 struct StepArgs {
diff --git a/charginghub-env_amd/csrc/chub_kernels.hip b/charginghub-env_amd/csrc/chub_kernels.hip
--- a/charginghub-env_amd/csrc/chub_kernels.hip
+++ b/charginghub-env_amd/csrc/chub_kernels.hip
@@ -294,6 +294,51 @@
         }
     }
     return (uint32_t) (stay_q + flow) | ((uint32_t) flow << 8);
+}
+__device__ __forceinline__ uint64_t draw_raw_levels(const HubParams &hp, const Tables &tb, uint32_t tick, int t, int k, int64_t env, int qmax,
+                                                    bool fast) {
+    PhiloxCtx px{hp.key[0], hp.key[1], tick, (uint32_t) (hp.env_id0 + env)};
+    const U4 a0 = px.block(SITE_ARRIVE, (uint32_t) k, 0);
+    const U4 r0 = px.block(SITE_RENEGE, (uint32_t) k, 0);
+    int n_in = (int) tb.cnt[k][t * kLevels + (int) (a0.v[0] % 1000u)];
+    n_in = n_in > 9 ? 9 : n_in;
+    uint32_t rw[10] = {r0.v[0], r0.v[1], r0.v[2], r0.v[3], 0u, 0u, 0u, 0u, 0u, 0u};
+    if (__any(qmax > 4)) {
+        const U4 r1 = px.block(SITE_RENEGE, (uint32_t) k, 1), r2 = px.block(SITE_RENEGE, (uint32_t) k, 2);
+        rw[4] = r1.v[0]; rw[5] = r1.v[1]; rw[6] = r1.v[2]; rw[7] = r1.v[3]; rw[8] = r2.v[0]; rw[9] = r2.v[1];
+    }
+    uint32_t ren = 0u;
+#pragma unroll
+    for (int w = 0; w < kMaxLine; w++) ren |= ((int) (rw[w] % 1000u) >= (int) tb.thr_renege[w]) ? (1u << w) : 0u;
+    uint64_t pk = (uint64_t) (ren | ((uint32_t) n_in << 10));
+    if (!fast && __any(n_in > 0)) {
+        uint32_t bw[9] = {a0.v[1], a0.v[2], a0.v[3], 0u, 0u, 0u, 0u, 0u, 0u};
+        if (__any(n_in > 3)) {
+            const U4 a1 = px.block(SITE_ARRIVE, (uint32_t) k, 1), a2 = px.block(SITE_ARRIVE, (uint32_t) k, 2);
+            bw[3] = a1.v[0]; bw[4] = a1.v[1]; bw[5] = a1.v[2]; bw[6] = a1.v[3]; bw[7] = a2.v[0]; bw[8] = a2.v[1];
+        }
+        const int S = hp.S[k];
+        int top[9];
+#pragma unroll
+        for (int j = 0; j < 9; j++) top[j] = -1;
+#pragma unroll
+        for (int j = 0; j < 9; j++) {
+            if (j >= 3 && !__any(n_in > j)) break;
+            top[j] = (j < n_in && j <= S) ? (int) tb.inv_balk[bw[j] % 1000u] - j : -1;
+        }
+        const bool more3 = __any(n_in > 3);
+#pragma unroll
+        for (int l = 0; l <= kMaxLine; l++) {
+            if (l > 0 && !__any(qmax >= l)) break;
+            int c = (l <= top[0] ? 1 : 0) + (l <= top[1] ? 1 : 0) + (l <= top[2] ? 1 : 0);
+            if (more3) {
+#pragma unroll
+                for (int j = 3; j < 9; j++) c += l <= top[j] ? 1 : 0;
+            }
+            pk |= (uint64_t) c << (14 + 4 * l);
+        }
+    }
+    return pk;
 }
 __device__ __forceinline__ int dk_want(uint32_t dk) { return (int) (dk & 255u); }
 __device__ __forceinline__ int dk_flow(uint32_t dk) { return (int) ((dk >> 8) & 255u); }
@@ -1500,6 +1545,7 @@
     uint32_t xcd;
     CHUB_G(float) tail_act;
     CHUB_G(uint8_t) stay8;
+    CHUB_G(const uint32_t) rec_prev;
 };
 
 typedef const uint32_t __attribute__((address_space(4))) *chub_sptr;
@@ -1528,7 +1574,7 @@
 #define CHUB_EPI_ALL 1
 #endif
 #define CHUB_AT(T_, base, byte_off) (*(CHUB_G(T_)) ((CHUB_G(char)) (base) + (uint32_t) (byte_off)))
-template <int BLOCK, int T, bool RESET, bool BIG, bool MASKED, bool FUSED, bool BITS>
+template <int BLOCK, int T, bool RESET, bool BIG, bool MASKED, bool FUSED, bool BITS, bool RAW = false>
 __device__ __forceinline__ void packed_records(const PackedArgs &pa, const uint32_t block_local, int *s_acc, const uint32_t *s_unit, u32x4 *s_rec,
                                                const float *tail_pre = nullptr) {
     const int lane = threadIdx.x & 63;
@@ -1554,7 +1600,7 @@
             CHUB_AT(f32x2_, pa.tail_act, (uint32_t) env << 3) = tv;
         }
         uint32_t lf = s_unit[i];
-        if ((k ? S1 : S0) == 0) {
+        if (!RAW && (k ? S1 : S0) == 0) {
             const uint32_t pk = CHUB_AT(const uint32_t, pa.pk, su << 2);
             const bool fast = (k ? pa.type[1] : pa.type[0]) == 0;
             int want, fl;
@@ -1595,7 +1641,7 @@
     __device__ __forceinline__ void prefetch() {}
     __device__ __forceinline__ void park() {}
 };
-template <int BLOCK, int T, bool TAPE, bool RESET, bool BIG, bool MASKED, bool FUSED, typename Hook, bool BITS = false, bool PIPED = false>
+template <int BLOCK, int T, bool TAPE, bool RESET, bool BIG, bool MASKED, bool FUSED, typename Hook, bool BITS = false, bool PIPED = false, bool RAW = false>
 __device__ __forceinline__ int slot_body_packed(const HubParams &hp, const StepArgs &sa, PackedArgs &pa, const Tables &tb,
                                                 const uint32_t block_local, uint32_t *q_cnt, uint32_t *q_new,
                                                 uint64_t *s_ball, int *s_acc, uint32_t *s_unit, Hook &hook, u32x4 *s_rec, uint32_t *s_uinfo) {
@@ -1615,6 +1661,7 @@
 
     constexpr bool STATE_FIRST = !RESET && !FUSED && BLOCK <= 256;
     constexpr bool UNIT_DRAWS = CHUB_UNIT_DRAWS && STATE_FIRST && !BIG && T <= 2;
+    static_assert(!RAW || (UNIT_DRAWS && !MASKED && !BITS && !TAPE), "the raw draws are decoded in the unit pass of the lock-step small tile");
     int e_[T], k_[T], slot[T];
     bool valid[T];
     uint32_t sidx[T];
@@ -1682,11 +1729,20 @@
         }
     }
     uint32_t upk = 0u;
+    u32x2 uraw = {0u, 0u};
+    uint32_t uprev = 0u;
     if (UNIT_DRAWS) asm volatile("" : "=v"(upk));
+    if (RAW) asm volatile("" : "=v"(uraw), "=v"(uprev));
     if (UNIT_DRAWS && (tid & ~63) < 2 * epb) {
         asm volatile("" ::: "memory");
         const int ue = tid >> 1, uenv = env_first + ue;
-        upk = CHUB_AT(const uint32_t, pa.pk, (ue < epb && uenv < N ? (uint32_t) ((tid & 1) ? N : 0) + (uint32_t) uenv : (uint32_t) env_first) << 2);
+        const uint32_t ui = ue < epb && uenv < N ? (uint32_t) ((tid & 1) ? N : 0) + (uint32_t) uenv : (uint32_t) env_first;
+        if (RAW) {
+            uraw = CHUB_AT(const u32x2, pa.pk, ui << 3);
+            uprev = CHUB_AT(const uint32_t, pa.rec_prev, (ui << 4) + 12u);
+        } else {
+            upk = CHUB_AT(const uint32_t, pa.pk, ui << 2);
+        }
     }
     if (HOIST_TAIL) asm volatile("" : "=v"(tail_pre[0]), "=v"(tail_pre[1]));
     if (HOIST_TAIL && wave == WAVES - 1) {
@@ -1769,7 +1825,12 @@
                 info |= (uint32_t) start_e | ((uint32_t) cnt0 << 8) | (UNIT_DRAWS ? 0u : (uint32_t) (cnt0 + cnt1) << 16);
             }
             if (UNIT_DRAWS) {
-                asm volatile("" : "+v"(upk));
+                if (RAW) {
+                    asm volatile("" : "+v"(uraw), "+v"(uprev));
+                    upk = dk_make((uint64_t) uraw.x | ((uint64_t) uraw.y << 32), pkd_line(uprev), (k ? pa.type[1] : pa.type[0]) == 0);
+                } else {
+                    asm volatile("" : "+v"(upk));
+                }
                 const int want = dk_want(upk);
                 const int assign = want < all ? want : all;
                 const int ln = want - assign;
@@ -1953,7 +2014,7 @@
 #endif
         if (wave != WAVES - 1) return 0;
     }
-    packed_records<BLOCK, T, RESET, BIG, MASKED, false, BITS>(pa, block_local, s_acc, s_unit, nullptr, tail_pre);
+    packed_records<BLOCK, T, RESET, BIG, MASKED, false, BITS, RAW>(pa, block_local, s_acc, s_unit, nullptr, tail_pre);
 #if CHUB_TRACE
     asm volatile("s_waitcnt vmcnt(0)" ::: "memory");
     CHUB_STAMP(11);
@@ -1963,7 +2024,7 @@
 #undef CHUB_AT
 }
 
-template <int BLOCK, int T, bool TAPE, bool RESET, bool BIG, bool MASKED, bool BITS = false>
+template <int BLOCK, int T, bool TAPE, bool RESET, bool BIG, bool MASKED, bool BITS = false, bool RAW = false>
 __global__ __launch_bounds__(BLOCK, (BLOCK <= 256 ? 8 : 2048 / BLOCK)) void k_slot_packed(const DevCtx *__restrict__ ctx, StepArgs sa, PackedArgs pa_in) {
     __shared__ uint32_t q_new[BLOCK * T];
     __shared__ uint32_t q_cnt[2];
@@ -1976,7 +2037,7 @@
     asm volatile("" : "+s"(pa.S[0]), "+s"(pa.S[1]), "+s"(pa.type[0]), "+s"(pa.type[1]), "+s"(pa.n_envs), "+s"(pa.epb), "+s"(pa.magic),
                       "+s"(pa.cls_delta), "+s"(pa.state), "+s"(pa.rec), "+s"(pa.pk), "+s"(pa.actions), "+s"(pa.cls0), "+s"(pa.ttab2));
     NoHook hook;
-    (void) slot_body_packed<BLOCK, T, TAPE, RESET, BIG, MASKED, false, NoHook, BITS>(ctx->hp, sa, pa, ctx->tb, xcd_order(blockIdx.x, pa.xcd, MASKED ? 0u : pa.xcd) + (MASKED ? pa.blk0 : 0u), q_cnt, q_new,
+    (void) slot_body_packed<BLOCK, T, TAPE, RESET, BIG, MASKED, false, NoHook, BITS, false, RAW>(ctx->hp, sa, pa, ctx->tb, xcd_order(blockIdx.x, pa.xcd, MASKED ? 0u : pa.xcd) + (MASKED ? pa.blk0 : 0u), q_cnt, q_new,
                                                                                      s_ball + 1, s_acc, s_unit, hook, nullptr, s_uinfo);
 }
 
@@ -2574,6 +2635,12 @@
     }
 }
 
+struct TailNext {
+    TailIn in;
+    u32x4 r0, r1;
+    double st_pv, st_wd;
+};
+
 struct NoMid {
     __device__ __forceinline__ void operator()() {}
     __device__ __forceinline__ void at1() {}
@@ -2588,12 +2655,13 @@
     return hv_count_rate(ep.hv_rate[e], (uint32_t) ep.hv_idx[(uint32_t) t * (uint32_t) kLevels + lev]);
 }
 
-template <bool RESET, int MODE, bool MULTI, bool FUSED = false, typename Mid = NoMid, int EB = kEnvBlock, bool TAPE = false, bool EP = false>
+template <bool RESET, int MODE, bool MULTI, bool FUSED = false, typename Mid = NoMid, int EB = kEnvBlock, bool TAPE = false, bool EP = false, int PAIR = 0>
 __device__ __forceinline__ void env_tail(const DevCtx *__restrict__ ctx, const StepArgs &sa, const int env, const bool live,
                                          const double *s_pv, const double *s_wd, const double *s_pv_now, const double *s_wd_now,
                                          const double *s_hy, const uint8_t *s_hv, float *s_out, const int env_block, const TailArgs &ta,
                                          const u32x4 *s_rec, const int local_env, const int env0_fused, const int rows_fused,
-                                         const TailIn &pre, const bool use_pre, Mid &mid) {
+                                         const TailIn &pre, const bool use_pre, Mid &mid, TailNext *nx = nullptr, const TailArgs *ta2 = nullptr) {
+    static_assert(PAIR == 0 || (!RESET && MODE == MODE_PHILOX && !MULTI && !FUSED && !TAPE && !EP), "pairs: the lock-step PHILOX step of the stand-alone tail");
     const HubParams &hp = ctx->hp;
     const EnvArrays &ev = ctx->ev;
     const CompatRng &cr = ctx->cr;
@@ -2634,15 +2702,23 @@
     const bool ep_on = (tel_word & 2) != 0;
     if (!FUSED) {
         const int i = threadIdx.x;
-        if (!multi) {
+        if (PAIR == 2) {
+            st_pv = nx->st_pv;
+            st_wd = nx->st_wd;
+        } else if (!multi) {
             if (i < 100) st_pv = ta.pv_row[i];
             if (i < 150) st_wd = ta.wd_row[i];
             if (!RESET) {
                 if (i < 100) st_pv_now = ta.pv_row_now[i];
                 if (i < 150) st_wd_now = ta.wd_row_now[i];
             }
-        }
-        if (!RESET) {
+            if (PAIR == 1) {
+                nx->st_pv = nx->st_wd = 0.0;
+                if (i < 100) nx->st_pv = ta2->pv_row[i];
+                if (i < 150) nx->st_wd = ta2->wd_row[i];
+            }
+        }
+        if (!RESET && PAIR != 2) {
             if (!EP && i < 102) st_hy = ta.hy_table[i];
             if (MODE == MODE_COMPAT && !EP && !multi && !sa.hv_tape && i < kLevels / 4) st_hv = ((CHUB_G(const uint32_t)) tb.cnt_hv)[sa.t * (kLevels / 4) + i];
         }
@@ -2656,7 +2732,7 @@
     int pv_day = 0, wd_day = 0, q_len = 0, hv_line = 0, F0i = 0, F1i = 0, ln0 = 0, ln1 = 0, hv_lev = 0, hv_arrive = 0;
     u32x4 drw_raw = {0u, 0u, 0u, 0u};
     uint32_t drw_n = 0u, hvw0 = 0u, hvw1 = 0u;
-    const bool have_pre = FUSED && use_pre;
+    const bool have_pre = (FUSED || PAIR == 2) && use_pre;
     double p_v_h_max = 0.0, p_cells = 0.0, p_rc_cells = 0.0, p_cap_mass = 0.0, p_rc_cap_mass = 0.0, p_init_soc = 0.0, p_hydro_loss = 0.0;
     double p_fc_max_power = 0.0, p_renew_fluct1 = 0.0, p_price_fluct1 = 0.0;
     if (live) {
@@ -2684,7 +2760,11 @@
             ou_price = ta.ou[2u * n32 + e32];
             in_price_noise = ta.price_noise[e32];
         }
-        if (!FUSED) {
+        if (PAIR == 2) {
+            const u32x4 v0 = nx->r0, v1 = nx->r1;
+            mn0 = __uint_as_float(v0.x); P0f = __uint_as_float(v0.y); mx0 = __uint_as_float(v0.z); ln0 = pkd_line(v0.w); F0i = pkd_flow(v0.w);
+            mn1 = __uint_as_float(v1.x); P1f = __uint_as_float(v1.y); mx1 = __uint_as_float(v1.z); ln1 = pkd_line(v1.w); F1i = pkd_flow(v1.w);
+        } else if (!FUSED) {
             const StationRec r0 = rec_load(ta.rec, e32), r1 = rec_load(ta.rec, n32 + e32);
             mn0 = r0.mn; P0f = r0.chg; mx0 = r0.mx; ln0 = pkd_line(r0.pkd); F0i = pkd_flow(r0.pkd);
             mn1 = r1.mn; P1f = r1.chg; mx1 = r1.mx; ln1 = pkd_line(r1.pkd); F1i = pkd_flow(r1.pkd);
@@ -2741,6 +2821,16 @@
             z_wd = sa.exo_z[e32 * 3u + 1u];
             z_pr = sa.exo_z[e32 * 3u + 2u];
         }
+        if (PAIR == 1) {
+            typedef float f32x2_ __attribute__((ext_vector_type(2)));
+            nx->r0 = ((CHUB_G(const u32x4)) ta2->rec)[e32];
+            nx->r1 = ((CHUB_G(const u32x4)) ta2->rec)[n32 + e32];
+            const f32x2_ tv = ((CHUB_G(const f32x2_)) ta2->tail_act)[e32];
+            nx->in.a_el = tv.x;
+            nx->in.a_fc = tv.y;
+            nx->in.drw = ((CHUB_G(const u32x4)) ta2->drw)[e32];
+            nx->in.drw_n = ta2->drw_cnt[e32];
+        }
     }
 
 
@@ -2755,7 +2845,7 @@
         const int i = threadIdx.x;
         if (i < 100) ((double *) s_pv)[i] = st_pv;
         if (i < 150) ((double *) s_wd)[i] = st_wd;
-        if (!RESET) {
+        if (!RESET && PAIR != 2) {
             if (i < 100) ((double *) s_pv_now)[i] = st_pv_now;
             if (i < 150) ((double *) s_wd_now)[i] = st_wd_now;
             if (!EP && i < 102) ((double *) s_hy)[i] = st_hy;
@@ -2950,6 +3040,10 @@
             hv_line = 0;
         }
         total_mass_need = total_mass;
+        if (PAIR == 1) {
+            nx->in.q_len = q_len;
+            nx->in.hv_line = hv_line | (stuck ? 128 : 0);
+        }
     }
     mid.at1();
 
@@ -2968,9 +3062,11 @@
             price_next = ou_sample(ou_price, .1, 0.005, z_pr) * HP_E(price_fluct1, p_price_fluct1);
             ev.ou[2u * n32 + e32] = ou_price;
             ev.price_noise[e32] = price_next;
+            if (PAIR == 1) nx->in.price_noise = price_next;
             price_next += price_last;
         } else {
             price_next = price_last + in_price_noise;
+            if (PAIR == 1) nx->in.price_noise = in_price_noise;
         }
     }
     if (MODE == MODE_COMPAT && !RESET && !hv_walked) rs.store(cr, sa.rng_cur, env);
@@ -3123,6 +3219,14 @@
     }
 
     ev.cap[e32] = cap;
+    if (PAIR == 1) {
+        nx->in.ou_pv = ou_pv;
+        nx->in.ou_wd = ou_wd;
+        nx->in.ou_price = ou_price;
+        nx->in.cap = cap;
+        nx->in.pv_day = pv_day;
+        nx->in.wd_day = wd_day;
+    }
 
     float *obs = s_out + (FUSED ? (int) (threadIdx.x & 63u) : (int) threadIdx.x) * row_w;
     double *o64 = tel_on ? (double *) ev.obs64 + (size_t) e32 * hp.obs_dim : nullptr;
@@ -3279,6 +3383,111 @@
     NoMid nomid;
     env_tail<RESET, MODE, MULTI, false, NoMid, kEnvBlock, TAPE, EP>(ctx, sa, env, env < (int) ta.n_envs && (!MULTI || in_group(sa, env)), s_pv, s_wd, s_pv_now,
                                                                 s_wd_now, s_hy, s_hv, s_out, blk, ta, nullptr, 0, 0, 0, none, false, nomid);
+}
+
+struct PairArgs {
+    CHUB_G(const uint32_t) rec_a;
+    CHUB_G(uint64_t) pkraw;
+    CHUB_G(const uint32_t) drw_in[2];
+    CHUB_G(const uint8_t) cnt_in[2];
+    CHUB_G(uint32_t) drw_out[2];
+    CHUB_G(uint8_t) cnt_out[2];
+};
+
+__device__ __forceinline__ void draw_env_pre(const DevCtx *__restrict__ ctx, const uint32_t tick, const int t, const uint32_t e, CHUB_G(uint32_t) drw,
+                                             CHUB_G(uint8_t) cnt_out) {
+    const HubParams &hp = ctx->hp;
+    const Tables &tb = ctx->tb;
+    PhiloxCtx px{hp.key[0], hp.key[1], tick, (uint32_t) (hp.env_id0 + e)};
+    const U4 ow = px.block(SITE_OU, 0, 0);
+    const uint32_t hv_lev = px.block(SITE_HV, 0, 0).v[0] % 1000u;
+    u32x4 d;
+    d.x = __float_as_uint(normal_from_word(tb.normal_icdf, tb.normal_tail, ow.v[0]));
+    d.y = __float_as_uint(normal_from_word(tb.normal_icdf, tb.normal_tail, ow.v[1]));
+    d.z = __float_as_uint(normal_from_word(tb.normal_icdf, tb.normal_tail, ow.v[2]));
+    const uint32_t cnt = (uint32_t) tb.cnt_hv[(uint32_t) t * (uint32_t) kLevels + hv_lev];
+    d.w = cnt != 0u ? __float_as_uint(soc_from_word(tb.soc_d_icdf, px.block(SITE_HVSOC, 0, 0).v[0])) : 0u;
+    ((CHUB_G(u32x4)) drw)[e] = d;
+    cnt_out[e] = (uint8_t) cnt;
+}
+
+__device__ __forceinline__ bool level_lane(const uint32_t jb, const uint32_t n32, const int nb_env, const uint32_t xcd, int64_t &u) {
+    const uint32_t per = n32 >> 3;
+    if (xcd && (n32 & 2047u) == 0u && ((uint32_t) nb_env & 7u) == 0u) {
+        const uint32_t x = jb & 7u, i = jb >> 3, wpx = per / kEnvBlock;
+        const uint32_t seg = i / wpx;
+        u = (int64_t) seg * n32 + (int64_t) (x * per + (i - seg * wpx) * kEnvBlock + threadIdx.x);
+        return seg < 3u;
+    }
+    u = (int64_t) jb * kEnvBlock + threadIdx.x;
+    return u < 3 * (int64_t) n32;
+}
+
+__global__ __launch_bounds__(kEnvBlock) void k_pair_draws(const DevCtx *__restrict__ ctx, StepArgs sa, PairArgs pr, uint32_t xcd) {
+    const HubParams &hp = ctx->hp;
+    const uint32_t n32 = (uint32_t) hp.n_envs;
+    int64_t u;
+    if (!level_lane(blockIdx.x, n32, 8, xcd, u)) return;
+    const uint32_t tick1 = CHUB_TICK(hp, sa.tick + 1u);
+    if (u < 2 * (int64_t) n32) {
+        const int kk = u >= (int64_t) n32 ? 1 : 0;
+        const int want = dk_want(ctx->st.pk[sa.tick & 1u][u]);
+        pr.pkraw[u] = draw_raw_levels(hp, ctx->tb, tick1, sa.t + 1, kk, u - (int64_t) kk * n32, want, hp.type[kk] == 0);
+    } else {
+        const uint32_t e = (uint32_t) (u - 2 * (int64_t) n32);
+        draw_env_pre(ctx, tick1 - 1u, sa.t, e, pr.drw_out[0], pr.cnt_out[0]);
+        draw_env_pre(ctx, tick1, sa.t + 1, e, pr.drw_out[1], pr.cnt_out[1]);
+    }
+}
+
+template <bool MORE>
+__global__ __launch_bounds__(kEnvBlock) void k_env_pair(const DevCtx *__restrict__ ctx, StepArgs sa, StepArgs sb, TailArgs ta, TailArgs tb2, PairArgs pr,
+                                                        int nb_env) {
+    __shared__ double s_pv[100], s_wd[150], s_pv_now[100], s_wd_now[150], s_hy[102], s_pv2[100], s_wd2[150];
+    __shared__ __attribute__((aligned(16))) float s_out[2][kEnvBlock * 16];
+    if ((int) blockIdx.x >= nb_env) {
+        const HubParams &hp = ctx->hp;
+        const uint32_t n32 = (uint32_t) hp.n_envs;
+        int64_t u;
+        if (!level_lane(blockIdx.x - (uint32_t) nb_env, n32, nb_env, ta.xcd, u)) return;
+        if (!MORE) {
+            level_block<false, false>(ctx, sb, u);
+            if (u < 2 * (int64_t) n32) {
+                const int kk = u >= (int64_t) n32 ? 1 : 0;
+                ctx->st.pk[sb.tick & 1u][u] = dk_make(pr.pkraw[u], pkd_line(pr.rec_a[4u * (uint32_t) u + 3u]), hp.type[kk] == 0);
+            } else {
+                const uint32_t e = (uint32_t) (u - 2 * (int64_t) n32);
+                ((CHUB_G(u32x4)) ctx->ev.drw[sb.tick & 1u])[e] = ((CHUB_G(const u32x4)) pr.drw_in[1])[e];
+                ctx->ev.drw_cnt[sb.tick & 1u][e] = pr.cnt_in[1][e];
+            }
+            return;
+        }
+        const uint32_t tick2 = CHUB_TICK(hp, sb.tick + 1u);
+        if (u < 2 * (int64_t) n32) {
+            const int kk = u >= (int64_t) n32 ? 1 : 0;
+            const bool fast = hp.type[kk] == 0;
+            const int64_t env_ = u - (int64_t) kk * n32;
+            const int line_now = pkd_line(ctx->st.rec[4u * (uint32_t) u + 3u]);
+            const uint32_t dk = draw_decoded_levels(hp, ctx->tb, tick2, sb.t + 1, kk, env_, line_now, fast);
+            ctx->st.pk[(sb.tick + 1u) & 1u][u] = dk;
+            pr.pkraw[u] = draw_raw_levels(hp, ctx->tb, tick2 + 1u, sb.t + 2, kk, env_, dk_want(dk), fast);
+        } else {
+            const uint32_t e = (uint32_t) (u - 2 * (int64_t) n32);
+            draw_env_pre(ctx, tick2, sb.t + 1, e, pr.drw_out[0], pr.cnt_out[0]);
+            draw_env_pre(ctx, tick2 + 1u, sb.t + 2, e, pr.drw_out[1], pr.cnt_out[1]);
+        }
+        return;
+    }
+    const int blk = (int) xcd_order(blockIdx.x, (uint32_t) nb_env, ta.xcd);
+    const int env = blk * kEnvBlock + (int) threadIdx.x;
+    const bool live = env < (int) ta.n_envs;
+    TailIn none;
+    TailNext nx;
+    NoMid nomid;
+    env_tail<false, MODE_PHILOX, false, false, NoMid, kEnvBlock, false, false, 1>(ctx, sa, env, live, s_pv, s_wd, s_pv_now, s_wd_now, s_hy, nullptr, s_out[0], blk, ta,
+                                                                                  nullptr, 0, 0, 0, none, false, nomid, &nx, &tb2);
+    env_tail<false, MODE_PHILOX, false, false, NoMid, kEnvBlock, false, false, 2>(ctx, sb, env, live, s_pv2, s_wd2, s_pv, s_wd, s_hy, nullptr, s_out[1], blk, tb2,
+                                                                                  nullptr, 0, 0, 0, nx.in, true, nomid, &nx, nullptr);
 }
 
 __global__ __launch_bounds__(256) void k_env_walk(const DevCtx *__restrict__ ctx, StepArgs sa, TailArgs ta, StepArgs sw, int nb_env) {
@@ -4776,6 +4985,7 @@
     pa.xcd = hp.xcd ? (uint32_t) ((hp.n_envs + hp.epb - 1) / hp.epb) : 0u;
     pa.tail_act = (CHUB_G(float)) pp.st->tail_act;
     pa.stay8 = (CHUB_G(uint8_t)) pp.stay8;
+    pa.rec_prev = nullptr;
     return pa;
 }
 
@@ -4883,6 +5093,54 @@
     CHUB_LAUNCH(k_env_walk, dim3(nb), dim3(kEnvBlock), stream, ev0, ev1, ctx, sa, ta, sw, nb_env);
 }
 
+void launch_pair(const HubParams &hp, const DevCtx *ctx, const StepArgs &sa_in, const StepArgs &sb_in, hipStream_t stream, const PackedPtrs &pp,
+                 const PairBufs &pb, int sel, bool chain_start, bool more) {
+    StepArgs sa = sa_in, sb = sb_in;
+    const int64_t N = hp.n_envs;
+    const int nb_env = (int) ((N + kEnvBlock - 1) / kEnvBlock);
+    const unsigned nb_lev = (unsigned) ((3 * N + kEnvBlock - 1) / kEnvBlock);
+    PairArgs pr;
+    pr.rec_a = (CHUB_G(const uint32_t)) pb.rec_a;
+    pr.pkraw = (CHUB_G(uint64_t)) pb.pkraw;
+    for (int q = 0; q < 2; q++) {
+        pr.drw_in[q] = (CHUB_G(const uint32_t)) pb.drw[sel][q];
+        pr.cnt_in[q] = (CHUB_G(const uint8_t)) pb.cnt[sel][q];
+        pr.drw_out[q] = (CHUB_G(uint32_t)) pb.drw[sel ^ 1][q];
+        pr.cnt_out[q] = (CHUB_G(uint8_t)) pb.cnt[sel ^ 1][q];
+    }
+    const uint32_t xcd = hp.xcd ? 1u : 0u;
+    if (chain_start) {
+        launch_levels(sa.fresh ? LEVELS_DRAW : LEVELS_NONE, ctx, sa, stream);
+        PairArgs p0 = pr;
+        for (int q = 0; q < 2; q++) {
+            p0.drw_out[q] = (CHUB_G(uint32_t)) pb.drw[sel][q];
+            p0.cnt_out[q] = (CHUB_G(uint8_t)) pb.cnt[sel][q];
+        }
+        hipLaunchKernelGGL(k_pair_draws, dim3(nb_lev), dim3(kEnvBlock), 0, stream, ctx, sa, p0, xcd);
+    }
+    sa.fresh = 0;
+    sb.fresh = 0;
+    const uint32_t nb = (uint32_t) ((N + hp.epb - 1) / hp.epb);
+    PackedArgs pa = make_packed_args(hp, sa, pp);
+    pa.rec = (CHUB_G(uint32_t)) pb.rec_a;
+    pa.tail_act = (CHUB_G(float)) pb.tail_act_a;
+    hipLaunchKernelGGL((k_slot_packed<kPackedBlock, kSlotsPerLane, false, false, false, false>), dim3(nb), dim3(kPackedBlock), 0, stream, ctx, sa, pa);
+    PackedArgs pa2 = make_packed_args(hp, sb, pp);
+    pa2.pk = (CHUB_G(const uint32_t)) (const void *) pb.pkraw;
+    pa2.rec_prev = (CHUB_G(const uint32_t)) pb.rec_a;
+    hipLaunchKernelGGL((k_slot_packed<kPackedBlock, kSlotsPerLane, false, false, false, false, false, true>), dim3(nb), dim3(kPackedBlock), 0, stream, ctx,
+                       sb, pa2);
+    TailArgs ta = make_tail_args(*pp.ev, *pp.st, hp, sa, pp, false), tb2 = make_tail_args(*pp.ev, *pp.st, hp, sb, pp, false);
+    ta.rec = (CHUB_G(uint32_t)) pb.rec_a;
+    ta.tail_act = (CHUB_G(const float)) pb.tail_act_a;
+    ta.drw = pr.drw_in[0];
+    ta.drw_cnt = pr.cnt_in[0];
+    tb2.drw = pr.drw_in[1];
+    tb2.drw_cnt = pr.cnt_in[1];
+    if (more) hipLaunchKernelGGL(k_env_pair<true>, dim3((unsigned) nb_env + nb_lev), dim3(kEnvBlock), 0, stream, ctx, sa, sb, ta, tb2, pr, nb_env);
+    else hipLaunchKernelGGL(k_env_pair<false>, dim3((unsigned) nb_env + nb_lev), dim3(kEnvBlock), 0, stream, ctx, sa, sb, ta, tb2, pr, nb_env);
+}
+
 __global__ void k_tick_advance(uint32_t *tick_base, uint32_t by) { *tick_base += by; }
 
 
diff --git a/charginghub-env_amd/csrc/chub_plan.h b/charginghub-env_amd/csrc/chub_plan.h
--- a/charginghub-env_amd/csrc/chub_plan.h
+++ b/charginghub-env_amd/csrc/chub_plan.h
@@ -14,6 +14,9 @@
 #endif
 #ifndef CHUB_SPLIT2
 #define CHUB_SPLIT2 1
+#endif
+#ifndef CHUB_PAIR_MIN_ENVS
+#define CHUB_PAIR_MIN_ENVS 8192
 #endif
 constexpr int64_t kBigTileSlots = (int64_t) 10 << 20;
 constexpr int64_t kXcdOrderSlots = (int64_t) 6 << 20;
@@ -21,6 +24,7 @@
 constexpr int kFusedMaxBlocksTailWave = 768;
 constexpr int kSpanMaxBlocks = 384;
 constexpr int kFusedMaxBlocks = 384;
+constexpr int64_t kPairMinEnvs = CHUB_PAIR_MIN_ENVS;
 constexpr int64_t kWalk2HalfMaxEnvs = 40000;
 
 enum PackedForm : int32_t {
@@ -153,6 +157,26 @@
     return CHUB_OK;
 }
 
+inline bool plan_pair_handle(const LaunchPlan &p, int64_t n_envs, const chub_options &opt, bool env_params) {
+    if (p.packed != PACKED_SMALL || p.one_launch != ONE_NONE || env_params || opt.span_steps == 1) return false;
+    return opt.span_steps >= 2 || n_envs >= kPairMinEnvs;
+}
+struct PairState {
+    bool comm;
+    bool per_env;
+    bool tape;
+    bool outputs;
+    bool profiling;
+};
+inline bool plan_pair_call(bool handle_pairs, const PairState &c) {
+    return handle_pairs && !c.comm && !c.per_env && !c.tape && !c.outputs && !c.profiling;
+}
+inline int64_t pair_steps(int t, int64_t left) {
+    const int64_t day = 96 - t;
+    const int64_t k = left < day ? left : day;
+    return k > 0 ? k & ~(int64_t) 1 : 0;
+}
+
 enum CallForm : int32_t {
     CALL_COMPAT_SMALL,
     CALL_ONE_LAUNCH,
diff --git a/charginghub-env_amd/csrc/chub_runtime.cpp b/charginghub-env_amd/csrc/chub_runtime.cpp
--- a/charginghub-env_amd/csrc/chub_runtime.cpp
+++ b/charginghub-env_amd/csrc/chub_runtime.cpp
@@ -54,6 +54,8 @@
                        hipEvent_t ev0, hipEvent_t ev1);
 void launch_env_walk(const HubParams &hp, const DevCtx *ctx, const StepArgs &sa, const StepArgs &sw, hipStream_t stream, hipEvent_t ev0, hipEvent_t ev1,
                      const PackedPtrs &pp);
+void launch_pair(const HubParams &hp, const DevCtx *ctx, const StepArgs &sa, const StepArgs &sb, hipStream_t stream, const PackedPtrs &pp,
+                 const PairBufs &pb, int sel, bool chain_start, bool more);
 }
 
 using namespace chub;
@@ -86,6 +88,9 @@
     Tables tb;
     int device;
     LaunchPlan plan;
+    bool pair_tails = false;
+    PairBufs pair = {};
+    char *d_pair = nullptr;
     int rng_cur = 0;
     uint32_t walked_tick = 0;
     uint32_t e2_tick = ~0u;
@@ -488,6 +493,7 @@
     e->cfg = *cfg_in;
     e->env_params = rows != nullptr;
     e->plan = plan;
+    e->pair_tails = plan_pair_handle(plan, n_envs, opt, rows != nullptr);
     e->public_mode = public_mode;
     e->device = device;
     e->t = 0;
@@ -974,6 +980,26 @@
         e->d_gae_part = nullptr;
         return bail(fail(CHUB_ERR_HIP, "hipMalloc failed"));
     }
+    if (e->pair_tails) {
+        const size_t Np = (size_t) n_envs;
+        auto up = [](size_t b) { return (b + 255) & ~(size_t) 255; };
+        const size_t b_rec = up(32 * Np), b_act = up(8 * Np), b_raw = up(16 * Np), b_drw = up(16 * Np), b_cnt = up(Np);
+        const size_t total = b_rec + b_act + b_raw + 4 * (b_drw + b_cnt);
+        if (hipMalloc((void **) &e->d_pair, total) != hipSuccess) {
+            e->d_pair = nullptr;
+            return bail(fail(CHUB_ERR_HIP, "hipMalloc failed"));
+        }
+        if (hipMemset(e->d_pair, 0, total) != hipSuccess) return bail(fail(CHUB_ERR_HIP, "hipMemset failed"));
+        char *q = e->d_pair;
+        e->pair.rec_a = (uint32_t *) q; q += b_rec;
+        e->pair.tail_act_a = (float *) q; q += b_act;
+        e->pair.pkraw = (uint64_t *) q; q += b_raw;
+        for (int a = 0; a < 2; a++)
+            for (int b = 0; b < 2; b++) {
+                e->pair.drw[a][b] = (uint32_t *) q; q += b_drw;
+                e->pair.cnt[a][b] = (uint8_t *) q; q += b_cnt;
+            }
+    }
     *out = e;
     return CHUB_OK;
 }
@@ -1004,6 +1030,7 @@
         if (e->fc.mean) (void) hipFree((void *) e->fc.mean);
         if (e->d_ep_sum) (void) hipFree(e->d_ep_sum);
         if (e->d_gae_part) (void) hipFree(e->d_gae_part);
+        if (e->d_pair) (void) hipFree(e->d_pair);
         if (e->h_bits) (void) hipHostFree(e->h_bits);
         if (e->d_bits) (void) hipFree(e->d_bits);
         if (e->d_packed) (void) hipFree(e->d_packed);
@@ -1032,6 +1059,34 @@
     return e ? ((e->hp.packed && e->hp.xcd && e->plan.one_launch == ONE_NONE) ? 1 : 0) : CHUB_ERR_ARG;
 }
 int chub_uses_fused_step(const chub_env *e) { return e ? ((e->plan.one_launch != ONE_NONE || e->plan.compat_small) ? 1 : 0) : CHUB_ERR_ARG; }
+
+int chub_uses_pair_tails(const chub_env *e) { return e ? (e->pair_tails ? 1 : 0) : CHUB_ERR_ARG; }
+
+int chub_pair_plan(const chub_config *cfg, int64_t n_envs, int rng_mode, const chub_options *opt_in, int env_params, uint32_t flags, int t, int64_t left,
+                   int64_t *out) {
+    if (!cfg || !out) return fail(CHUB_ERR_ARG, "null argument");
+    if (t < 0 || t > 95 || left < 0) return fail(CHUB_ERR_ARG, "t must be 0 .. 95 and left >= 0");
+    chub_options opt;
+    memset(&opt, 0, sizeof opt);
+    if (opt_in) opt = *opt_in;
+    LaunchPlan p;
+    const char *msg = nullptr;
+    if (const int rc = plan_handle(cfg, n_envs, rng_mode, opt, p, &msg)) return fail(rc, msg);
+    if (env_params)
+        if (const int rc = plan_params(p, rng_mode, &msg)) return fail(rc, msg);
+    const bool handle = plan_pair_handle(p, n_envs, opt, env_params != 0);
+    PairState c;
+    c.comm = (flags & CHUB_PAIRF_COMM) != 0;
+    c.per_env = (flags & CHUB_PAIRF_PER_ENV) != 0;
+    c.tape = (flags & CHUB_PAIRF_TAPE) != 0;
+    c.outputs = (flags & CHUB_PAIRF_OUTPUTS) != 0;
+    c.profiling = (flags & CHUB_PAIRF_PROFILING) != 0;
+    const bool call = plan_pair_call(handle, c);
+    out[CHUB_PAIR_HANDLE] = handle ? 1 : 0;
+    out[CHUB_PAIR_CALL] = call ? 1 : 0;
+    out[CHUB_PAIR_STEPS] = call ? pair_steps(t, left) : 0;
+    return CHUB_OK;
+}
 
 int chub_launch_plan(const chub_config *cfg, int64_t n_envs, int rng_mode, const chub_options *opt_in, int32_t *out) {
     if (!cfg || !out) return fail(CHUB_ERR_ARG, "null argument");
@@ -1601,6 +1656,51 @@
     return note_served(e, nullptr, 2, s);
 }
 
+static bool pairs_ok(const chub_env *e, const chub_comm *comm) {
+    PairState c;
+    c.comm = comm != nullptr;
+    c.per_env = e->per_env;
+    c.tape = e->tape_only;
+    c.outputs = e->st_out != nullptr || e->es.on != 0 || e->hp.telemetry != 0;
+    c.profiling = e->prof_on;
+    return plan_pair_call(e->pair_tails, c) && e->tick != 0;
+}
+
+static int run_pairs(chub_env *e, const float *const *batches, int n_batches, float *const *packed2, int64_t first, int64_t n_pairs, hipStream_t s) {
+    HIP_TRY(hipSetDevice(e->device));
+    (void) hipGetLastError();
+    const MaskView all = {nullptr, 0, e->hp.n_envs - 1};
+    int sel = 0;
+    for (int64_t p = 0; p < n_pairs; p++) {
+        const int64_t i = first + 2 * p;
+        const StepCall c1 = step_call(nullptr, batches[i % n_batches], nullptr, packed_out(e, packed2[i & 1]), 0);
+        const StepCall c2 = step_call(nullptr, batches[(i + 1) % n_batches], nullptr, packed_out(e, packed2[(i + 1) & 1]), 0);
+        StepArgs sa, sb;
+        if (const int rc = fill_args(e, c1, 2, all, e->tick + 1u, s, sa)) return rc;
+        {
+            const int t0 = e->t, pc0 = e->price_count;
+            const bool pd0 = e->predrawn;
+            e->t = t0 + 1;
+            e->price_count = pc0 + 1;
+            e->predrawn = true;
+            const int rc = fill_args(e, c2, 2, all, e->tick + 2u, s, sb);
+            e->t = t0;
+            e->price_count = pc0;
+            e->predrawn = pd0;
+            if (rc) return rc;
+        }
+        launch_pair(e->hp, e->d_ctx, sa, sb, s, packed_ptrs(e), e->pair, sel, p == 0, p + 1 < n_pairs);
+        if (hipGetLastError() != hipSuccess) {
+            e->predrawn = false;
+            return fail(CHUB_ERR_HIP, "a pair of steps could not be launched");
+        }
+        e->tick += 2u;
+        advance_clocks(e, c1, 2, 2);
+        sel ^= 1;
+    }
+    return note_served(e, nullptr, 2, s);
+}
+
 int chub_run_steps(chub_env *e, chub_comm *comm, const float *const *d_action_batches, int n_batches, float *const *d_packed2,
                    float *const *d_gathered2, float *d_reset_obs, int64_t first_step, int64_t n_steps, void *stream) {
     if (!e || !d_action_batches || n_batches <= 0 || !d_packed2 || !d_packed2[0] || !d_packed2[1] || !d_reset_obs || first_step < 0 ||
@@ -1609,6 +1709,14 @@
     for (int64_t i = first_step; i < first_step + n_steps; i++) {
         int rc;
         if (i % 96 == 0 && (rc = chub_reset_device(e, nullptr, nullptr, d_reset_obs, stream))) return rc;
+        if (pairs_ok(e, comm)) {
+            const int64_t k2 = pair_steps(e->t, std::min<int64_t>(first_step + n_steps - i, 96 - i % 96));
+            if (k2 >= 2) {
+                if ((rc = run_pairs(e, d_action_batches, n_batches, d_packed2, i, k2 / 2, (hipStream_t) stream))) return rc;
+                i += k2 - 1;
+                continue;
+            }
+        }
         if (!comm) {
             int64_t k = first_step + n_steps - i;
             k = k < 96 - i % 96 ? k : 96 - i % 96;
diff --git a/charginghub-env_amd/vec_env.py b/charginghub-env_amd/vec_env.py
--- a/charginghub-env_amd/vec_env.py
+++ b/charginghub-env_amd/vec_env.py
@@ -978,6 +978,10 @@
         return bool(self._lib.chub_uses_fused_step(self._h))
 
     @property
+    def uses_pair_tails(self):
+        return bool(self._lib.chub_uses_pair_tails(self._h))
+
+    @property
     def uses_xcd_order(self):
         return bool(self._lib.chub_uses_xcd_order(self._h))
 
diff --git a/include/chub.h b/include/chub.h
--- a/include/chub.h
+++ b/include/chub.h
@@ -83,6 +83,11 @@
 int chub_get_env_params(chub_env *env, chub_env_params *rows );
 int chub_has_env_params(const chub_env *env);
 int chub_launch_plan_params(const chub_config *cfg, int64_t n_envs, int rng_mode, const chub_options *opt , int32_t *out);
+enum { CHUB_PAIR_HANDLE = 0, CHUB_PAIR_CALL, CHUB_PAIR_STEPS, CHUB_PAIR_COUNT };
+enum { CHUB_PAIRF_COMM = 1, CHUB_PAIRF_PER_ENV = 2, CHUB_PAIRF_TAPE = 4, CHUB_PAIRF_OUTPUTS = 8, CHUB_PAIRF_PROFILING = 16 };
+int chub_pair_plan(const chub_config *cfg, int64_t n_envs, int rng_mode, const chub_options *opt , int env_params, uint32_t flags,
+                   int t, int64_t left, int64_t *out);
+int chub_uses_pair_tails(const chub_env *env);
 
 int chub_obs_dim(const chub_env *env);
 int chub_act_dim(const chub_env *env);
```
